# Biomedical-Imaging-Group/MolecularDiffusion_MiViT

Measured on AMD Instinct MI355X. Metric: training image-sequences/sec, higher is better.
Workload: dtype bf16; 1 GPU; PSFNoise 32-frame 64x64 sequences, MiViT depth=4 dim=128 heads=4 hidden=256, linear frame embedding + regression token; train step = fwd + MSE + bwd + AdamW; per_gpu_batch=16384, global_batch=16384, frames=32, frame=64x64, parallelism=dp1, input_dtype=f32 frames resident in HBM

## Files before the change

### include/mivit_hip.h

```cpp
#ifndef MIVIT_HIP_H
#define MIVIT_HIP_H

#include <stddef.h>
#include <stdint.h>

#ifdef __cplusplus
extern "C" {
#endif

#define MIVIT_ABI_VERSION 1

enum { MIVIT_F32 = 0, MIVIT_BF16 = 1, MIVIT_F16 = 2, MIVIT_F64 = 3 };
enum { MIVIT_ACT_NONE = 0, MIVIT_ACT_RELU = 1, MIVIT_ACT_LEAKY_RELU = 2, MIVIT_ACT_GELU = 3 };
enum { MIVIT_EMBED_LINEAR = 0, MIVIT_EMBED_CNN = 1, MIVIT_EMBED_EXTERNAL = 2 };
enum { MIVIT_FUSION_NONE = 0, MIVIT_FUSION_EARLY = 1, MIVIT_FUSION_LATE = 2 };

int mivit_abi_version(void);
const char *mivit_last_error(void);
int mivit_device_count(void);


int mivit_linear_fwd(int dtype, const void *x, int x_is_f32, int64_t ldx, const float *W, const float *bias,
                     int M, int N, int K, int act, const void *resid, int64_t ldr,
                     void *y, int64_t ldy, void *y_preact, void *stream);

int mivit_linear_dgrad(int dtype, const void *dy, int64_t lddy, const float *W, int M, int N, int K,
                       int act, const void *saved, int64_t lds, const void *dres, int64_t lddr,
                       void *dx, int64_t lddx, void *stream);

size_t mivit_linear_wgrad_workspace_bytes(int M, int N, int K);
int mivit_linear_wgrad(int dtype, const void *dy, int64_t lddy, const void *x, int x_is_f32, int64_t ldx,
                       int M, int N, int K, float *dW, float *db, int accumulate,
                       void *workspace, size_t workspace_bytes, void *stream);

int mivit_embed_fwd_bf16(const float *x, const void *W_bf16, const float *bias, int M, int K, int E, void *y_bf16,
                         void *stream);
int mivit_embed_set_variant(int variant);
size_t mivit_embed_wgrad_bf16_workspace_bytes(int M, int K, int E);
int mivit_embed_wgrad_bf16(const void *dy_bf16, const float *x, int M, int K, int E, float *dW, void *workspace,
                           size_t workspace_bytes, void *stream);

int mivit_embed_small_supported(int M, int K, int E);
int mivit_embed_small_fwd(const float *x, const void *W_bf16, const float *bias, int M, int K, int E, void *y_bf16, void *stream);
size_t mivit_embed_small_wgrad_workspace_bytes(int M, int K, int E);
int mivit_embed_small_wgrad(const void *dy_bf16, const float *x, int M, int K, int E, float *dW, float *db, void *workspace,
                            size_t workspace_bytes, void *stream);

int mivit_rowstream_fwd(const void *x, int64_t ldx, const void *W_bf16, const float *bias, int M, int N, int K, int act,
                        const void *resid, int64_t ldr, void *y, int64_t ldy, void *y_preact, const float *ln_gamma,
                        const float *ln_beta, void *ln_out, float *mean, float *rstd, void *stream);
int mivit_rowstream_dgrad(const void *dy, int64_t lddy, const void *W_bf16, int M, int N, int K, int act,
                          const void *saved, int64_t lds, const void *dres, int64_t lddr, void *dx, int64_t lddx,
                          void *stream);
int mivit_wavestream_fwd(const void *x, int64_t ldx, const void *W_bf16, const float *bias, int M, int N, int K, int act,
                         const void *resid, int64_t ldr, void *y, int64_t ldy, void *y_preact, const float *ln_gamma,
                         const float *ln_beta, void *ln_out, float *mean, float *rstd, void *stream);
int mivit_wavestream_dgrad(const void *dy, int64_t lddy, const void *W_bf16, int M, int N, int K, int act,
                           const void *saved, int64_t lds, const void *dres, int64_t lddr, void *dx, int64_t lddx,
                           void *stream);
int mivit_rowstream_set_wavestream(int mode);
int mivit_rowstream_set_wavestream_mask(int mask);

int mivit_gemm_dma_supported(int M, int N, int K, int dgrad);
int mivit_gemm_dma_set_variant(int variant);
int mivit_gemm_dma_fwd(const void *x, int64_t ldx, const void *W_bf16, const float *bias, int M, int N, int K, int act,
                       const void *resid, int64_t ldr, void *y, int64_t ldy, void *y_preact, void *stream);
int mivit_gemm_dma_dgrad(const void *dy, int64_t lddy, const void *W_bf16, int M, int N, int K, int act,
                         const void *saved, int64_t lds, const void *dres, int64_t lddr, void *dx, int64_t lddx,
                         void *stream);
size_t mivit_wgrad_bf16_workspace_bytes(int M, int N, int K);
int mivit_wgrad_bf16(const void *dy, int64_t lddy, const void *x, int64_t ldx, int M, int N, int K, float *dW, float *db,
                     void *workspace, size_t workspace_bytes, void *stream);
int mivit_wgrad_bf16_set_config(int cfg);

int mivit_rowstream_fwd_f16(const void *x, int64_t ldx, const void *W_f16, const float *bias, int M, int N, int K, int act,
                            const void *resid, int64_t ldr, void *y, int64_t ldy, void *y_preact, const float *ln_gamma,
                            const float *ln_beta, void *ln_out, float *mean, float *rstd, void *stream);
int mivit_rowstream_dgrad_f16(const void *dy, int64_t lddy, const void *W_f16, int M, int N, int K, int act,
                              const void *saved, int64_t lds, const void *dres, int64_t lddr, void *dx, int64_t lddx,
                              void *stream);
int mivit_wavestream_fwd_f16(const void *x, int64_t ldx, const void *W_f16, const float *bias, int M, int N, int K, int act,
                             const void *resid, int64_t ldr, void *y, int64_t ldy, void *y_preact, const float *ln_gamma,
                             const float *ln_beta, void *ln_out, float *mean, float *rstd, void *stream);
int mivit_wavestream_dgrad_f16(const void *dy, int64_t lddy, const void *W_f16, int M, int N, int K, int act,
                               const void *saved, int64_t lds, const void *dres, int64_t lddr, void *dx, int64_t lddx,
                               void *stream);
int mivit_rowstream_set_wavestream_f16(int mode);
int mivit_rowstream_set_wavestream_mask_f16(int mask);
size_t mivit_wgrad_bf16_workspace_bytes_f16(int M, int N, int K);
int mivit_wgrad_bf16_f16(const void *dy, int64_t lddy, const void *x, int64_t ldx, int M, int N, int K, float *dW, float *db,
                         void *workspace, size_t workspace_bytes, void *stream);
int mivit_wgrad_bf16_set_config_f16(int cfg);
size_t mivit_wgrad_small_workspace_bytes_f16(int M, int N, int K);
int mivit_wgrad_small_f16(const void *dy, int64_t lddy, const void *x, int64_t ldx, int M, int N, int K, float *dW,
                          float *db, void *workspace, size_t workspace_bytes, void *stream);
int mivit_embed_small_supported_f16(int M, int K, int E);
int mivit_embed_small_fwd_f16(const float *x, const void *W_f16, const float *bias, int M, int K, int E, void *y_f16, void *stream);
size_t mivit_embed_small_wgrad_workspace_bytes_f16(int M, int K, int E);
int mivit_embed_small_wgrad_f16(const void *dy_f16, const float *x, int M, int K, int E, float *dW, float *db, void *workspace,
                                size_t workspace_bytes, void *stream);
int mivit_embed_fwd_bf16_f16(const float *x, const void *W_f16, const float *bias, int M, int K, int E, void *y_f16,
                             void *stream);
int mivit_embed_set_variant_f16(int variant);
size_t mivit_embed_wgrad_bf16_workspace_bytes_f16(int M, int K, int E);
int mivit_embed_wgrad_bf16_f16(const void *dy_f16, const float *x, int M, int K, int E, float *dW, void *workspace,
                               size_t workspace_bytes, void *stream);

int mivit_fused_layer_supported(int dtype, int embed_dim, int hidden_dim, int num_heads, int tokens);
int mivit_attn_block_fwd(const void *n_in, const float *gamma_in, const float *beta_in, const void *Wqkv_bf16,
                         const float *bqkv, const void *Wo_bf16, const float *bo, const float *gamma_out,
                         const float *beta_out, int B, int S, void *ctx, void *n_out, float *rstd, void *x_out,
                         void *z_out, float *mean, void *qkv_out, void *stream);
int mivit_mlp_block_fwd(const void *n_in, const float *gamma_in, const float *beta_in, const void *W1_bf16,
                        const float *b1, const void *W2_bf16, const float *b2, const float *gamma_out,
                        const float *beta_out, int M, int act, void *n_out, float *rstd, void *x_out, void *z_out,
                        float *mean, void *h_out, void *u_out, void *stream);

size_t mivit_mlp_block_bwd_workspace_bytes(int M);
int mivit_mlp_block_bwd_set_waves(int waves);
int mivit_mlp_block_bwd(const void *dy, const void *n2, const float *rstd2, const float *gamma2, const void *n1,
                        const float *gamma1, const float *beta1, const void *W1_bf16, const float *b1, const void *W2_bf16,
                        int M, int act, void *dx1, float *dW1, float *db1, float *dW2, float *db2, float *dgamma2,
                        float *dbeta2, void *workspace, size_t workspace_bytes, void *stream);

int mivit_render_frames(const float *traj_px, int N, int T, int npos, const float *sigmas, int nsig, int P, int up,
                        const float *amp, int center, float *out, void *stream);

int mivit_render_movie(const float *pos, const float *amp, const int *first, const int *last, int Np, int F, int npos,
                       float sigma_hr, int up, int radius, int H, int W, float *movie, void *stream);

size_t mivit_trajectory_features_workspace_bytes(int N, int T, int npos);
int mivit_trajectory_features(const void *traj, int dtype, int N, int T, int npos, double dt, double *feats, void *avg,
                              void *workspace, size_t workspace_bytes, void *stream);

int mivit_rl_tv_deconvolve(const float *frames, int B, int S, int H, int W, const double *psf, int K, const int *snapshots,
                           int n_snap, float tv_weight, float *out, void *stream);

int mivit_gaussian_filter_frames(const float *in, int N, int H, int W, double sigma, double truncate, float *out,
                                 void *stream);

size_t mivit_dog_peaks_workspace_bytes(int F, int H, int W, int cap, int store_dog);
int mivit_dog_peaks(const float *movie, int F, int H, int W, const double *w1, int r1, const double *w2, int r2,
                    float threshold_percentage, int min_distance, int cap, int *count, int *n_candidates, int *coords,
                    float *values, float *dog, void *workspace, size_t workspace_bytes, void *stream);

int mivit_refine_gaussian(const float *patches, int N, int P, double xtol, double *params, float *peak, int *status,
                          void *stream);

int mivit_link_frames(const int *coords, const int *count, const unsigned char *movie_start, int F, int cap,
                      double max_distance, int *link, void *stream);

int mivit_chain_tracks(const int *link, const int *count, const unsigned char *movie_start, int F, int cap, int *ids,
                       int *lengths, int *n_tracks, void *stream);

int mivit_close_gaps(const int *coords, const int *count, const int *link, const unsigned char *movie_start, int F, int cap,
                     int max_gap, double max_distance, int *gap_partner, int *gap_frames, unsigned char *workspace,
                     size_t workspace_bytes, void *stream);

int mivit_chain_tracks_gaps(const int *link, const int *gap_partner, const int *gap_frames, const int *count,
                            const unsigned char *movie_start, int F, int cap, int max_gap, int *ids, int *lengths,
                            int *n_tracks, void *stream);

int mivit_track_msd(const double *pos, int N, const int *offsets, int n_tracks, double dt, int max_lag, int Lmax, double *msd,
                    double *d_lstsq, double *d_weighted, void *stream);

int mivit_track_sequences(const float *movie, int F, int H, int W, const int *frame, const int *y, const int *x, int N,
                          const int *seq_row, int n_seq, int T, int P, float lo, float denom, int normalize, float *seq,
                          void *stream);

int mivit_fgn(const double *z, const double *gamma, const int *gamma_row, int N, int T, int C, int U, double *out, void *stream);

int mivit_map_displacements(const double *disp, const double *s0, const int *geom_of, const double *verts, const double *lengths,
                            const int *vert_offsets, const double *totals, int N, int T, int G, int V, int mode, double *pos,
                            double *arc, int *edge, void *stream);

int mivit_segment_tracks(const double *pos, int N, const int *offsets, int n_tracks, int max_len, int min_len, double penalty,
                         double min_var, int *seg_start, double *cost, void *stream);
int mivit_segment_stats(const double *pos, int N, const int *seg_offsets, const int *seg_track_end, int n_seg, double dt,
                        double R, double *d_cve, double *d_mle, double *sigma2, int *n_increments, void *stream);
int mivit_markov_states(const double *u, const double *p0, const double *M, int N, int T, int K, int *state, void *stream);

size_t mivit_attn_out_bwd_workspace_bytes(int M);
int mivit_attn_out_bwd(const void *dy, const void *n1, const float *rstd1, const float *gamma1, const void *ctx,
                       const void *Wo_bf16, int M, void *dz1, void *dctx, float *dWo, float *dbo, float *dgamma1,
                       float *dbeta1, void *workspace, size_t workspace_bytes, void *stream);

size_t mivit_qkv_bwd_workspace_bytes(int M);
int mivit_qkv_bwd(const void *dqkv, const void *x, const void *Wqkv_bf16, const void *res, int M, void *dx, float *dW, float *db,
                  void *workspace, size_t workspace_bytes, void *stream);
int mivit_qkv_bwd_affine(const void *dqkv, const void *x, const void *Wqkv_bf16, const void *res, int M, void *dx, float *dW,
                         float *db, const float *fix_gamma, const float *fix_beta, void *workspace, size_t workspace_bytes,
                         void *stream);
size_t mivit_qkv_bwd_workspace_bytes_w64(int M);
int mivit_qkv_bwd_w64(const void *dqkv, const void *x, const void *Wqkv_bf16, const void *res, int M, void *dx, float *dW, float *db,
                      void *workspace, size_t workspace_bytes, void *stream);
int mivit_qkv_bwd_affine_w64(const void *dqkv, const void *x, const void *Wqkv_bf16, const void *res, int M, void *dx, float *dW,
                             float *db, const float *fix_gamma, const float *fix_beta, void *workspace, size_t workspace_bytes,
                             void *stream);

int mivit_fused_layer_supported_w64(int dtype, int embed_dim, int hidden_dim, int num_heads, int tokens);
int mivit_attn_block_fwd_w64(const void *n_in, const float *gamma_in, const float *beta_in, const void *Wqkv_bf16,
                             const float *bqkv, const void *Wo_bf16, const float *bo, const float *gamma_out,
                             const float *beta_out, int B, int S, void *ctx, void *n_out, float *rstd, void *x_out,
                             void *z_out, float *mean, void *qkv_out, void *stream);
int mivit_mlp_block_fwd_w64(const void *n_in, const float *gamma_in, const float *beta_in, const void *W1_bf16,
                            const float *b1, const void *W2_bf16, const float *b2, const float *gamma_out,
                            const float *beta_out, int M, int act, void *n_out, float *rstd, void *x_out, void *z_out,
                            float *mean, void *h_out, void *u_out, void *stream);
size_t mivit_mlp_block_bwd_workspace_bytes_w64(int M);
int mivit_mlp_block_bwd_w64(const void *dy, const void *n2, const float *rstd2, const float *gamma2, const void *n1,
                            const float *gamma1, const float *beta1, const void *W1_bf16, const float *b1, const void *W2_bf16,
                            int M, int act, void *dx1, float *dW1, float *db1, float *dW2, float *db2, float *dgamma2,
                            float *dbeta2, void *workspace, size_t workspace_bytes, void *stream);
size_t mivit_attn_out_bwd_workspace_bytes_w64(int M);
int mivit_attn_out_bwd_w64(const void *dy, const void *n1, const float *rstd1, const float *gamma1, const void *ctx,
                           const void *Wo_bf16, int M, void *dz1, void *dctx, float *dWo, float *dbo, float *dgamma1,
                           float *dbeta1, void *workspace, size_t workspace_bytes, void *stream);

int mivit_fused_layer_supported_f16(int dtype, int embed_dim, int hidden_dim, int num_heads, int tokens);
int mivit_attn_block_fwd_f16(const void *n_in, const float *gamma_in, const float *beta_in, const void *Wqkv,
                             const float *bqkv, const void *Wo, const float *bo, const float *gamma_out,
                             const float *beta_out, int B, int S, void *ctx, void *n_out, float *rstd, void *x_out,
                             void *z_out, float *mean, void *qkv_out, void *stream);
int mivit_mlp_block_fwd_f16(const void *n_in, const float *gamma_in, const float *beta_in, const void *W1,
                            const float *b1, const void *W2, const float *b2, const float *gamma_out,
                            const float *beta_out, int M, int act, void *n_out, float *rstd, void *x_out, void *z_out,
                            float *mean, void *h_out, void *u_out, void *stream);
size_t mivit_mlp_block_bwd_workspace_bytes_f16(int M);
int mivit_mlp_block_bwd_f16(const void *dy, const void *n2, const float *rstd2, const float *gamma2, const void *n1,
                            const float *gamma1, const float *beta1, const void *W1, const float *b1, const void *W2,
                            int M, int act, void *dx1, float *dW1, float *db1, float *dW2, float *db2, float *dgamma2,
                            float *dbeta2, void *workspace, size_t workspace_bytes, void *stream);
size_t mivit_attn_out_bwd_workspace_bytes_f16(int M);
int mivit_attn_out_bwd_f16(const void *dy, const void *n1, const float *rstd1, const float *gamma1, const void *ctx,
                           const void *Wo, int M, void *dz1, void *dctx, float *dWo, float *dbo, float *dgamma1,
                           float *dbeta1, void *workspace, size_t workspace_bytes, void *stream);
size_t mivit_qkv_bwd_workspace_bytes_f16(int M);
int mivit_qkv_bwd_f16(const void *dqkv, const void *x, const void *Wqkv, const void *res, int M, void *dx, float *dW, float *db,
                      void *workspace, size_t workspace_bytes, void *stream);
int mivit_qkv_bwd_affine_f16(const void *dqkv, const void *x, const void *Wqkv, const void *res, int M, void *dx, float *dW,
                             float *db, const float *fix_gamma, const float *fix_beta, void *workspace, size_t workspace_bytes,
                             void *stream);
int mivit_mlp_block_bwd_set_waves_f16(int waves);
int mivit_fused_layer_supported_w64_f16(int dtype, int embed_dim, int hidden_dim, int num_heads, int tokens);
int mivit_attn_block_fwd_w64_f16(const void *n_in, const float *gamma_in, const float *beta_in, const void *Wqkv,
                                 const float *bqkv, const void *Wo, const float *bo, const float *gamma_out,
                                 const float *beta_out, int B, int S, void *ctx, void *n_out, float *rstd, void *x_out,
                                 void *z_out, float *mean, void *qkv_out, void *stream);
int mivit_mlp_block_fwd_w64_f16(const void *n_in, const float *gamma_in, const float *beta_in, const void *W1,
                                const float *b1, const void *W2, const float *b2, const float *gamma_out,
                                const float *beta_out, int M, int act, void *n_out, float *rstd, void *x_out, void *z_out,
                                float *mean, void *h_out, void *u_out, void *stream);
size_t mivit_mlp_block_bwd_workspace_bytes_w64_f16(int M);
int mivit_mlp_block_bwd_w64_f16(const void *dy, const void *n2, const float *rstd2, const float *gamma2, const void *n1,
                                const float *gamma1, const float *beta1, const void *W1, const float *b1, const void *W2,
                                int M, int act, void *dx1, float *dW1, float *db1, float *dW2, float *db2, float *dgamma2,
                                float *dbeta2, void *workspace, size_t workspace_bytes, void *stream);
size_t mivit_attn_out_bwd_workspace_bytes_w64_f16(int M);
int mivit_attn_out_bwd_w64_f16(const void *dy, const void *n1, const float *rstd1, const float *gamma1, const void *ctx,
                               const void *Wo, int M, void *dz1, void *dctx, float *dWo, float *dbo, float *dgamma1,
                               float *dbeta1, void *workspace, size_t workspace_bytes, void *stream);
size_t mivit_qkv_bwd_workspace_bytes_w64_f16(int M);
int mivit_qkv_bwd_w64_f16(const void *dqkv, const void *x, const void *Wqkv, const void *res, int M, void *dx, float *dW, float *db,
                          void *workspace, size_t workspace_bytes, void *stream);
int mivit_qkv_bwd_affine_w64_f16(const void *dqkv, const void *x, const void *Wqkv, const void *res, int M, void *dx, float *dW,
                                 float *db, const float *fix_gamma, const float *fix_beta, void *workspace, size_t workspace_bytes,
                                 void *stream);

int mivit_deepresnet_eval_supported(int dtype, int patch_size);
int mivit_deepresnet_eval_fwd(int dtype, const float *x, int N, int P, int E, const float *w0, const float *b0,
                              const void *w11, const void *w12, const void *w1s, const void *w21, const void *w22,
                              const void *w2s, const float *b11, const float *b12, const float *b21, const float *b22,
                              const float *wfc, const float *bfc, float *tokens, void *stream);

typedef struct { const float *weight, *gamma, *beta; float *running_mean, *running_var; } mivit_conv_bn;
typedef struct { mivit_conv_bn conv[7]; const float *fc_weight, *fc_bias; } mivit_deepresnet_params;
typedef struct { float *weight, *gamma, *beta; } mivit_conv_bn_grad;
typedef struct { mivit_conv_bn_grad conv[7]; float *fc_weight, *fc_bias; } mivit_deepresnet_grads;
int mivit_deepresnet_train_supported(int dtype, int patch_size);
size_t mivit_deepresnet_train_workspace_bytes(int dtype, int N, int P, int E);
int mivit_deepresnet_train_fwd(int dtype, const mivit_deepresnet_params *params, const float *x, int N, int P, int E,
                               float momentum, float eps, float *tokens, void *workspace, size_t workspace_bytes,
                               void *stream);
int mivit_deepresnet_infer(int dtype, const mivit_deepresnet_params *params, const float *x, int N, int P, int E,
                           float eps, float *tokens, void *workspace, size_t workspace_bytes, void *stream);
int mivit_deepresnet_train_bwd(int dtype, const mivit_deepresnet_params *params, const float *x, const float *dtokens,
                               int N, int P, int E, float eps, const mivit_deepresnet_grads *grads, void *workspace,
                               size_t workspace_bytes, void *stream);

int mivit_deepresnet_train_workspace_layout(int dtype, int N, int P, int E, size_t *offsets );

#define MIVIT_DEEPRESNET_STAGES 6
#define MIVIT_DEEPRESNET_STATS_DOUBLES (2 * 3 * 128)
int mivit_deepresnet_train_fwd_stage(int dtype, const mivit_deepresnet_params *params, const float *x, int N, int P, int E,
                                     float momentum, float eps, float *tokens, void *workspace, size_t workspace_bytes,
                                     int stage, const double *global_count, double *stats, void *stream);
int mivit_deepresnet_train_bwd_stage(int dtype, const mivit_deepresnet_params *params, const float *x, const float *dtokens,
                                     int N, int P, int E, float eps, const mivit_deepresnet_grads *grads, void *workspace,
                                     size_t workspace_bytes, int stage, const double *global_count, double *stats, void *stream);

size_t mivit_wgrad_small_workspace_bytes(int M, int N, int K);
int mivit_wgrad_small(const void *dy, int64_t lddy, const void *x, int64_t ldx, int M, int N, int K, float *dW,
                      float *db , void *workspace, size_t workspace_bytes, void *stream);

int mivit_layernorm_fwd(int dtype, const void *z, int64_t ldz, const float *gamma, const float *beta,
                        int M, int E, void *y, int64_t ldy, int rows_per_seq, int out_seq_stride, int out_row_off,
                        const float *pos, float *mean, float *rstd, void *stream);

size_t mivit_layernorm_bwd_workspace_bytes(int M, int E);
int mivit_layernorm_bwd(int dtype, const void *dy, int64_t lddy, const void *z, int64_t ldz,
                        const float *gamma, const float *mean, const float *rstd, int M, int E,
                        int rows_per_seq, int in_seq_stride, int in_row_off,
                        void *dz, int64_t lddz, float *dgamma, float *dbeta, int accumulate,
                        void *workspace, size_t workspace_bytes, void *stream);

int mivit_attention_max_seq(int dtype, int Dh);
int mivit_attention_fwd(int dtype, const void *qkv, int B, int S, int H, int Dh, void *ctx, void *stream);
int mivit_attention_bwd(int dtype, const void *qkv, const void *dctx, int B, int S, int H, int Dh,
                        void *dqkv, void *stream);

typedef struct mivit_config {
    int abi_version;
    int dtype;
    int embedding;
    int patch_size;
    int embed_dim;
    int num_heads;
    int hidden_dim;
    int num_layers;
    int activation;
    int use_pos_encoding;
    int use_regression_token;
    int fusion;
    int global_feature_dim;
    int head_hidden;
    int output_dim;
} mivit_config;

typedef struct mivit_plan mivit_plan;

mivit_plan *mivit_plan_create(const mivit_config *cfg);
void mivit_plan_destroy(mivit_plan *plan);

int mivit_plan_num_params(const mivit_plan *plan);
const char *mivit_plan_param_name(const mivit_plan *plan, int i);
int64_t mivit_plan_param_offset(const mivit_plan *plan, int i);
int64_t mivit_plan_param_numel(const mivit_plan *plan, int i);
int64_t mivit_plan_arena_numel(const mivit_plan *plan);
int mivit_plan_num_stages(const mivit_plan *plan);
int mivit_plan_stage_range(const mivit_plan *plan, int stage, int64_t *begin, int64_t *end);

size_t mivit_plan_workspace_bytes(const mivit_plan *plan, int B, int T, int need_backward);

int mivit_forward(const mivit_plan *plan, const float *params, const float *x, const float *features,
                  int B, int T, void *workspace, size_t workspace_bytes, int need_backward,
                  float *out, void *stream);

int mivit_backward(const mivit_plan *plan, const float *params, const float *x, const float *features,
                   int B, int T, void *workspace, size_t workspace_bytes, const float *dout,
                   float *grads, float *dfeatures, float *dx_tokens,
                   int stage_begin, int stage_end, void *stream);

void mivit_graph_stats(uint64_t *replays, uint64_t *captures, int *failures);

enum {
    MIVIT_PROF_EMBED_FWD = 0,
    MIVIT_PROF_EMBED_WGRAD = 1,
    MIVIT_PROF_LINEAR_FWD = 2,
    MIVIT_PROF_LINEAR_DGRAD = 3,
    MIVIT_PROF_LINEAR_WGRAD = 4,
    MIVIT_PROF_ATTN_FWD = 5,
    MIVIT_PROF_ATTN_BWD = 6,
    MIVIT_PROF_LN_FWD = 7,
    MIVIT_PROF_LN_BWD = 8,
    MIVIT_PROF_OP = 9,
    MIVIT_PROF_ATTN_BLOCK_FWD = 10,
    MIVIT_PROF_MLP_BLOCK_FWD = 11,
    MIVIT_PROF_MLP_BLOCK_BWD = 12,
    MIVIT_PROF_ATTN_OUT_BWD = 13,
    MIVIT_PROF_ATTN_CORE_BWD = 14,
    MIVIT_PROF_QKV_WGRAD = 15,
    MIVIT_PROF_QKV_DGRAD = 16,
    MIVIT_PROF_QKV_BWD = 17,
    MIVIT_PROF_NUM_TAGS = 18
};
int mivit_profile_enable(uint64_t tag_mask);
int mivit_profile_collect(int tag, double *total_ms, int *count);
const char *mivit_profile_tag_name(int tag);

#ifdef __cplusplus
}
#endif
#endif
```

### moleculardiffusion_mivit_amd/_native.py

```python
import ctypes
import os
from ctypes import c_char_p, c_float, c_int, c_int64, c_size_t, c_void_p, POINTER, Structure

_PKG = os.path.dirname(os.path.abspath(__file__))
LIB_PATH = os.path.join(_PKG, "libmivit_hip.so")

ABI_VERSION = 1
F32, BF16, F16 = 0, 1, 2
F64 = 3
ACT_NONE, ACT_RELU, ACT_LEAKY_RELU, ACT_GELU = 0, 1, 2, 3
EMBED_LINEAR, EMBED_CNN, EMBED_EXTERNAL = 0, 1, 2
FUSION_NONE, FUSION_EARLY, FUSION_LATE = 0, 1, 2


class MivitConfig(Structure):
    _fields_ = [(n, c_int) for n in (
        "abi_version", "dtype", "embedding", "patch_size", "embed_dim", "num_heads", "hidden_dim", "num_layers",
        "activation", "use_pos_encoding", "use_regression_token", "fusion", "global_feature_dim", "head_hidden",
        "output_dim")]


class ConvBn(Structure):
    _fields_ = [(n, c_void_p) for n in ("weight", "gamma", "beta", "running_mean", "running_var")]


class DeepResNetParams(Structure):
    _fields_ = [("conv", ConvBn * 7), ("fc_weight", c_void_p), ("fc_bias", c_void_p)]


class ConvBnGrad(Structure):
    _fields_ = [(n, c_void_p) for n in ("weight", "gamma", "beta")]


class DeepResNetGrads(Structure):
    _fields_ = [("conv", ConvBnGrad * 7), ("fc_weight", c_void_p), ("fc_bias", c_void_p)]


SYMBOLS = {
    "mivit_abi_version": (c_int, []),
    "mivit_last_error": (c_char_p, []),
    "mivit_device_count": (c_int, []),
    "mivit_linear_fwd": (c_int, [c_int, c_void_p, c_int, c_int64, c_void_p, c_void_p, c_int, c_int, c_int, c_int,
                                 c_void_p, c_int64, c_void_p, c_int64, c_void_p, c_void_p]),
    "mivit_linear_dgrad": (c_int, [c_int, c_void_p, c_int64, c_void_p, c_int, c_int, c_int, c_int, c_void_p, c_int64,
                                   c_void_p, c_int64, c_void_p, c_int64, c_void_p]),
    "mivit_linear_wgrad_workspace_bytes": (c_size_t, [c_int, c_int, c_int]),
    "mivit_linear_wgrad": (c_int, [c_int, c_void_p, c_int64, c_void_p, c_int, c_int64, c_int, c_int, c_int, c_void_p,
                                   c_void_p, c_int, c_void_p, c_size_t, c_void_p]),
    "mivit_embed_fwd_bf16": (c_int, [c_void_p, c_void_p, c_void_p, c_int, c_int, c_int, c_void_p, c_void_p]),
    "mivit_embed_set_variant": (c_int, [c_int]),
    "mivit_embed_wgrad_bf16_workspace_bytes": (c_size_t, [c_int, c_int, c_int]),
    "mivit_embed_wgrad_bf16": (c_int, [c_void_p, c_void_p, c_int, c_int, c_int, c_void_p, c_void_p, c_size_t, c_void_p]),
    "mivit_rowstream_fwd": (c_int, [c_void_p, c_int64, c_void_p, c_void_p, c_int, c_int, c_int, c_int, c_void_p, c_int64,
                                    c_void_p, c_int64, c_void_p, c_void_p, c_void_p, c_void_p, c_void_p, c_void_p, c_void_p]),
    "mivit_rowstream_dgrad": (c_int, [c_void_p, c_int64, c_void_p, c_int, c_int, c_int, c_int, c_void_p, c_int64, c_void_p,
                                      c_int64, c_void_p, c_int64, c_void_p]),
    "mivit_wavestream_fwd": (c_int, [c_void_p, c_int64, c_void_p, c_void_p, c_int, c_int, c_int, c_int, c_void_p, c_int64,
                                     c_void_p, c_int64, c_void_p, c_void_p, c_void_p, c_void_p, c_void_p, c_void_p, c_void_p]),
    "mivit_wavestream_dgrad": (c_int, [c_void_p, c_int64, c_void_p, c_int, c_int, c_int, c_int, c_void_p, c_int64, c_void_p,
                                       c_int64, c_void_p, c_int64, c_void_p]),
    "mivit_gemm_dma_supported": (c_int, [c_int, c_int, c_int, c_int]),
    "mivit_gemm_dma_set_variant": (c_int, [c_int]),
    "mivit_gemm_dma_fwd": (c_int, [c_void_p, c_int64, c_void_p, c_void_p, c_int, c_int, c_int, c_int, c_void_p, c_int64,
                                   c_void_p, c_int64, c_void_p, c_void_p]),
    "mivit_gemm_dma_dgrad": (c_int, [c_void_p, c_int64, c_void_p, c_int, c_int, c_int, c_int, c_void_p, c_int64, c_void_p,
                                     c_int64, c_void_p, c_int64, c_void_p]),
    "mivit_wgrad_bf16_workspace_bytes": (c_size_t, [c_int, c_int, c_int]),
    "mivit_wgrad_bf16": (c_int, [c_void_p, c_int64, c_void_p, c_int64, c_int, c_int, c_int, c_void_p, c_void_p, c_void_p,
                                 c_size_t, c_void_p]),
    "mivit_deepresnet_eval_supported": (c_int, [c_int, c_int]),
    "mivit_deepresnet_eval_fwd": (c_int, [c_int, c_void_p, c_int, c_int, c_int] + [c_void_p] * 16),
    "mivit_deepresnet_train_supported": (c_int, [c_int, c_int]),
    "mivit_deepresnet_train_workspace_bytes": (c_size_t, [c_int, c_int, c_int, c_int]),
    "mivit_deepresnet_train_fwd": (c_int, [c_int, c_void_p, c_void_p, c_int, c_int, c_int, c_float, c_float, c_void_p,
                                           c_void_p, c_size_t, c_void_p]),
    "mivit_deepresnet_infer": (c_int, [c_int, c_void_p, c_void_p, c_int, c_int, c_int, c_float, c_void_p, c_void_p, c_size_t,
                                       c_void_p]),
    "mivit_deepresnet_train_bwd": (c_int, [c_int, c_void_p, c_void_p, c_void_p, c_int, c_int, c_int, c_float, c_void_p,
                                           c_void_p, c_size_t, c_void_p]),
    "mivit_deepresnet_train_workspace_layout": (c_int, [c_int, c_int, c_int, c_int, c_void_p]),
    "mivit_deepresnet_train_fwd_stage": (c_int, [c_int, c_void_p, c_void_p, c_int, c_int, c_int, c_float, c_float, c_void_p,
                                                 c_void_p, c_size_t, c_int, c_void_p, c_void_p, c_void_p]),
    "mivit_deepresnet_train_bwd_stage": (c_int, [c_int, c_void_p, c_void_p, c_void_p, c_int, c_int, c_int, c_float, c_void_p,
                                                 c_void_p, c_size_t, c_int, c_void_p, c_void_p, c_void_p]),
    "mivit_graph_stats": (None, [c_void_p, c_void_p, c_void_p]),
    "mivit_wgrad_small_workspace_bytes": (c_size_t, [c_int, c_int, c_int]),
    "mivit_wgrad_small": (c_int, [c_void_p, c_int64, c_void_p, c_int64, c_int, c_int, c_int, c_void_p, c_void_p, c_void_p,
                                  c_size_t, c_void_p]),
    "mivit_layernorm_fwd": (c_int, [c_int, c_void_p, c_int64, c_void_p, c_void_p, c_int, c_int, c_void_p, c_int64,
                                    c_int, c_int, c_int, c_void_p, c_void_p, c_void_p, c_void_p]),
    "mivit_layernorm_bwd_workspace_bytes": (c_size_t, [c_int, c_int]),
    "mivit_layernorm_bwd": (c_int, [c_int, c_void_p, c_int64, c_void_p, c_int64, c_void_p, c_void_p, c_void_p, c_int,
                                    c_int, c_int, c_int, c_int, c_void_p, c_int64, c_void_p, c_void_p, c_int,
                                    c_void_p, c_size_t, c_void_p]),
    "mivit_attention_max_seq": (c_int, [c_int, c_int]),
    "mivit_attention_fwd": (c_int, [c_int, c_void_p, c_int, c_int, c_int, c_int, c_void_p, c_void_p]),
    "mivit_attention_bwd": (c_int, [c_int, c_void_p, c_void_p, c_int, c_int, c_int, c_int, c_void_p, c_void_p]),
    "mivit_plan_create": (c_void_p, [POINTER(MivitConfig)]),
    "mivit_plan_destroy": (None, [c_void_p]),
    "mivit_plan_num_params": (c_int, [c_void_p]),
    "mivit_plan_param_name": (c_char_p, [c_void_p, c_int]),
    "mivit_plan_param_offset": (c_int64, [c_void_p, c_int]),
    "mivit_plan_param_numel": (c_int64, [c_void_p, c_int]),
    "mivit_plan_arena_numel": (c_int64, [c_void_p]),
    "mivit_plan_num_stages": (c_int, [c_void_p]),
    "mivit_plan_stage_range": (c_int, [c_void_p, c_int, POINTER(c_int64), POINTER(c_int64)]),
    "mivit_plan_workspace_bytes": (c_size_t, [c_void_p, c_int, c_int, c_int]),
    "mivit_forward": (c_int, [c_void_p, c_void_p, c_void_p, c_void_p, c_int, c_int, c_void_p, c_size_t, c_int,
                              c_void_p, c_void_p]),
    "mivit_backward": (c_int, [c_void_p, c_void_p, c_void_p, c_void_p, c_int, c_int, c_void_p, c_size_t, c_void_p,
                               c_void_p, c_void_p, c_void_p, c_int, c_int, c_void_p]),
    "mivit_fused_layer_supported": (c_int, [c_int, c_int, c_int, c_int, c_int]),
    "mivit_attn_block_fwd": (c_int, [c_void_p] * 9 + [c_int, c_int] + [c_void_p] * 8),
    "mivit_mlp_block_fwd": (c_int, [c_void_p] * 9 + [c_int, c_int] + [c_void_p] * 8),
    "mivit_mlp_block_bwd_workspace_bytes": (c_size_t, [c_int]),
    "mivit_mlp_block_bwd_set_waves": (c_int, [c_int]),
    "mivit_mlp_block_bwd": (c_int, [c_void_p] * 10 + [c_int, c_int] + [c_void_p] * 8 + [c_size_t, c_void_p]),
    "mivit_render_frames": (c_int, [c_void_p, c_int, c_int, c_int, c_void_p, c_int, c_int, c_int, c_void_p, c_int, c_void_p, c_void_p]),
    "mivit_render_movie": (c_int, [c_void_p, c_void_p, c_void_p, c_void_p, c_int, c_int, c_int, c_float, c_int, c_int, c_int, c_int,
                                   c_void_p, c_void_p]),
    "mivit_trajectory_features_workspace_bytes": (c_size_t, [c_int, c_int, c_int]),
    "mivit_trajectory_features": (c_int, [c_void_p, c_int, c_int, c_int, c_int, ctypes.c_double, c_void_p, c_void_p, c_void_p,
                                          c_size_t, c_void_p]),
    "mivit_rl_tv_deconvolve": (c_int, [c_void_p, c_int, c_int, c_int, c_int, c_void_p, c_int, c_void_p, c_int, ctypes.c_float,
                                       c_void_p, c_void_p]),
    "mivit_gaussian_filter_frames": (c_int, [c_void_p, c_int, c_int, c_int, ctypes.c_double, ctypes.c_double, c_void_p,
                                             c_void_p]),
    "mivit_dog_peaks_workspace_bytes": (c_size_t, [c_int, c_int, c_int, c_int, c_int]),
    "mivit_dog_peaks": (c_int, [c_void_p, c_int, c_int, c_int, c_void_p, c_int, c_void_p, c_int, c_float, c_int, c_int,
                                c_void_p, c_void_p, c_void_p, c_void_p, c_void_p, c_void_p, c_size_t, c_void_p]),
    "mivit_refine_gaussian": (c_int, [c_void_p, c_int, c_int, ctypes.c_double, c_void_p, c_void_p, c_void_p, c_void_p]),
    "mivit_link_frames": (c_int, [c_void_p, c_void_p, c_void_p, c_int, c_int, ctypes.c_double, c_void_p, c_void_p]),
    "mivit_chain_tracks": (c_int, [c_void_p, c_void_p, c_void_p, c_int, c_int, c_void_p, c_void_p, c_void_p, c_void_p]),
    "mivit_close_gaps": (c_int, [c_void_p, c_void_p, c_void_p, c_void_p, c_int, c_int, c_int, ctypes.c_double, c_void_p, c_void_p,
                                 c_void_p, c_size_t, c_void_p]),
    "mivit_chain_tracks_gaps": (c_int, [c_void_p, c_void_p, c_void_p, c_void_p, c_void_p, c_int, c_int, c_int, c_void_p, c_void_p,
                                        c_void_p, c_void_p]),
    "mivit_track_msd": (c_int, [c_void_p, c_int, c_void_p, c_int, ctypes.c_double, c_int, c_int, c_void_p, c_void_p, c_void_p,
                                c_void_p]),
    "mivit_track_sequences": (c_int, [c_void_p, c_int, c_int, c_int, c_void_p, c_void_p, c_void_p, c_int, c_void_p, c_int, c_int,
                                      c_int, ctypes.c_float, ctypes.c_float, c_int, c_void_p, c_void_p]),
    "mivit_fgn": (c_int, [c_void_p, c_void_p, c_void_p, c_int, c_int, c_int, c_int, c_void_p, c_void_p]),
    "mivit_map_displacements": (c_int, [c_void_p] * 7 + [c_int] * 5 + [c_void_p] * 4),
    "mivit_segment_tracks": (c_int, [c_void_p, c_int, c_void_p, c_int, c_int, c_int, ctypes.c_double, ctypes.c_double, c_void_p,
                                     c_void_p, c_void_p]),
    "mivit_segment_stats": (c_int, [c_void_p, c_int, c_void_p, c_void_p, c_int, ctypes.c_double, ctypes.c_double, c_void_p,
                                    c_void_p, c_void_p, c_void_p, c_void_p]),
    "mivit_markov_states": (c_int, [c_void_p, c_void_p, c_void_p, c_int, c_int, c_int, c_void_p, c_void_p]),
    "mivit_attn_out_bwd_workspace_bytes": (c_size_t, [c_int]),
    "mivit_attn_out_bwd": (c_int, [c_void_p] * 6 + [c_int] + [c_void_p] * 7 + [c_size_t, c_void_p]),
    "mivit_embed_small_supported": (c_int, [c_int, c_int, c_int]),
    "mivit_embed_small_fwd": (c_int, [c_void_p, c_void_p, c_void_p, c_int, c_int, c_int, c_void_p, c_void_p]),
    "mivit_embed_small_wgrad_workspace_bytes": (c_size_t, [c_int, c_int, c_int]),
    "mivit_embed_small_wgrad": (c_int, [c_void_p, c_void_p, c_int, c_int, c_int, c_void_p, c_void_p, c_void_p, c_size_t, c_void_p]),
    "mivit_qkv_bwd_workspace_bytes": (c_size_t, [c_int]),
    "mivit_qkv_bwd": (c_int, [c_void_p] * 4 + [c_int] + [c_void_p] * 4 + [c_size_t, c_void_p]),
    "mivit_qkv_bwd_workspace_bytes_w64": (c_size_t, [c_int]),
    "mivit_qkv_bwd_w64": (c_int, [c_void_p] * 4 + [c_int] + [c_void_p] * 4 + [c_size_t, c_void_p]),
    "mivit_fused_layer_supported_w64": (c_int, [c_int, c_int, c_int, c_int, c_int]),
    "mivit_attn_block_fwd_w64": (c_int, [c_void_p] * 9 + [c_int, c_int] + [c_void_p] * 8),
    "mivit_mlp_block_fwd_w64": (c_int, [c_void_p] * 9 + [c_int, c_int] + [c_void_p] * 8),
    "mivit_mlp_block_bwd_workspace_bytes_w64": (c_size_t, [c_int]),
    "mivit_mlp_block_bwd_w64": (c_int, [c_void_p] * 10 + [c_int, c_int] + [c_void_p] * 8 + [c_size_t, c_void_p]),
    "mivit_attn_out_bwd_workspace_bytes_w64": (c_size_t, [c_int]),
    "mivit_attn_out_bwd_w64": (c_int, [c_void_p] * 6 + [c_int] + [c_void_p] * 7 + [c_size_t, c_void_p]),
    "mivit_qkv_bwd_affine": (c_int, [c_void_p] * 4 + [c_int] + [c_void_p] * 6 + [c_size_t, c_void_p]),
    "mivit_qkv_bwd_affine_w64": (c_int, [c_void_p] * 4 + [c_int] + [c_void_p] * 6 + [c_size_t, c_void_p]),
    "mivit_mlp_block_bwd_set_waves_f16": (c_int, [c_int]),
    "mivit_profile_enable": (c_int, [ctypes.c_uint64]),
    "mivit_profile_collect": (c_int, [c_int, POINTER(ctypes.c_double), POINTER(c_int)]),
    "mivit_profile_tag_name": (c_char_p, [c_int]),
}
for _sfx in ("_f16", "_w64_f16"):
    for _name in ("mivit_fused_layer_supported", "mivit_attn_block_fwd", "mivit_mlp_block_fwd", "mivit_mlp_block_bwd_workspace_bytes",
                  "mivit_mlp_block_bwd", "mivit_attn_out_bwd_workspace_bytes", "mivit_attn_out_bwd", "mivit_qkv_bwd_workspace_bytes",
                  "mivit_qkv_bwd", "mivit_qkv_bwd_affine"):
        SYMBOLS[_name + _sfx] = SYMBOLS[_name]
SYMBOLS["mivit_rowstream_set_wavestream"] = SYMBOLS["mivit_rowstream_set_wavestream_mask"] = (c_int, [c_int])
SYMBOLS["mivit_wgrad_bf16_set_config"] = (c_int, [c_int])
for _name in ("mivit_rowstream_fwd", "mivit_rowstream_dgrad", "mivit_wavestream_fwd", "mivit_wavestream_dgrad",
              "mivit_rowstream_set_wavestream", "mivit_rowstream_set_wavestream_mask", "mivit_wgrad_bf16_workspace_bytes",
              "mivit_wgrad_bf16", "mivit_wgrad_bf16_set_config", "mivit_wgrad_small_workspace_bytes", "mivit_wgrad_small",
              "mivit_embed_small_supported", "mivit_embed_small_fwd", "mivit_embed_small_wgrad_workspace_bytes",
              "mivit_embed_small_wgrad", "mivit_embed_fwd_bf16", "mivit_embed_set_variant",
              "mivit_embed_wgrad_bf16_workspace_bytes", "mivit_embed_wgrad_bf16"):
    SYMBOLS[_name + "_f16"] = SYMBOLS[_name]
PROF_TAGS = ["embed_fwd", "embed_wgrad", "linear_fwd", "linear_dgrad", "linear_wgrad", "attn_fwd", "attn_bwd",
             "ln_fwd", "ln_bwd", "op", "attn_block_fwd", "mlp_block_fwd", "mlp_block_bwd", "attn_out_bwd", "attn_core_bwd",
             "qkv_wgrad", "qkv_dgrad", "qkv_bwd"]


class MivitError(RuntimeError):
    pass


def _load(path=LIB_PATH):
    if not os.path.exists(path):
        raise ImportError(
            f"{path} is missing: the MiViT HIP extension has not been built. Run "
            "`python -m moleculardiffusion_mivit_amd.csrc.build` (needs hipcc, targets gfx950). "
            "There is no CPU / PyTorch fallback for this path.")
    import torch
    lib = ctypes.CDLL(path)
    for name, (res, args) in SYMBOLS.items():
        fn = getattr(lib, name)
        fn.restype = res
        fn.argtypes = args
    if lib.mivit_abi_version() != ABI_VERSION:
        raise ImportError(f"libmivit_hip.so ABI {lib.mivit_abi_version()} != binding ABI {ABI_VERSION}; rebuild")
    return lib


lib = _load()

STRICT_LIB_PATH = os.path.join(_PKG, "libmivit_hip_strict.so")


def load_strict():
    return _load(STRICT_LIB_PATH)


def check(rc, what=""):
    if rc != 0:
        msg = lib.mivit_last_error()
        raise MivitError(f"{what}: {msg.decode() if msg else 'unknown error'}")


def last_error():
    msg = lib.mivit_last_error()
    return msg.decode() if msg else ""
```

### moleculardiffusion_mivit_amd/csrc/attention.hip

```cpp
#include "common.h"

namespace {

template <typename T>
struct Img {
    T *p;
    int rs, ks;
};

template <typename T>
__device__ __forceinline__ f32x4 tile_mma(const Img<T> A, int ar0, const Img<T> B, int br0, int kdim, int lane) {
    f32x4 acc = {0.f, 0.f, 0.f, 0.f};
    for (int kk = 0; kk < kdim; kk += Mma<T>::KS)
        acc = Mma<T>::mma(Mma<T>::load(A.p, A.rs, A.ks, ar0, kk, lane), Mma<T>::load(B.p, B.rs, B.ks, br0, kk, lane), acc);
    return acc;
}

__device__ __forceinline__ void wave_lds_sync() {
    __builtin_amdgcn_fence(__ATOMIC_ACQ_REL, "workgroup");
    __builtin_amdgcn_wave_barrier();
}

__device__ __forceinline__ float group16_max(float v) {
#pragma unroll
    for (int o = 8; o > 0; o >>= 1) v = fmaxf(v, __shfl_xor(v, o, 64));
    return v;
}
__device__ __forceinline__ float group16_sum(float v) {
#pragma unroll
    for (int o = 8; o > 0; o >>= 1) v += __shfl_xor(v, o, 64);
    return v;
}

struct AttnDims {
    int S, Dh, E, H, B;
    int Sp;
    int Skp;
    int Dp;
    int D16;
    int ldq;
    int ldk;
    int per_wave;
    int two_pass;
    int nw;
};

template <typename T>
__host__ __device__ inline int round_up_i(int x, int m) { return (x + m - 1) / m * m; }

template <typename T>
AttnDims make_dims(int B, int S, int H, int Dh, bool backward) {
    constexpr int KS = Mma<T>::KS;
    constexpr bool BF = sizeof(T) == 2;
    AttnDims d;
    d.B = B; d.S = S; d.H = H; d.Dh = Dh; d.E = H * Dh;
    d.Sp = (S + 15) / 16 * 16;
    const int kr = KS > 16 ? KS : 16;
    d.Skp = (S + kr - 1) / kr * kr;
    d.Dp = (Dh + KS - 1) / KS * KS;
    d.D16 = (Dh + 15) / 16 * 16;
    const int rowsq = d.Sp;
    if (BF) {
        d.ldq = d.Dp + 8;
        d.ldk = d.Skp + 8;
    } else {
        d.ldq = (d.Dp > d.D16 ? d.Dp : d.D16) + 1;
        d.ldk = d.Skp + 1;
    }
    const int nat = rowsq * d.ldq;
    const int tr = d.D16 * d.ldk;
    const int ps = (d.Sp > d.Skp ? d.Sp : d.Skp) * d.ldk;
    if (!backward) d.per_wave = 3 * nat + (BF ? tr : 0) + ps;
    else d.per_wave = 4 * nat + (BF ? 3 * tr : 0) + (BF ? 3 : 2) * ps;
    d.two_pass = 0;
    if (backward && !BF && (size_t)d.per_wave * sizeof(T) > (size_t)160 * 1024) { d.two_pass = 1; d.per_wave = 4 * nat + ps; }
    d.per_wave = (d.per_wave + 7) / 8 * 8;
    const size_t bytes = (size_t)d.per_wave * sizeof(T);
    int nw = (int)((size_t)64 * 1024 / bytes);
    d.nw = nw < 1 ? 1 : (nw > 4 ? 4 : nw);
    return d;
}

template <typename T>
__device__ __forceinline__ void stage_head(const T *src, int64_t src_ld, int S, int Dh, T *nat, int ldq, T *tr, int ldk,
                                           int lane) {
    if ((Dh & 3) == 0) {
        const int per_row = Dh >> 2;
        for (int u = lane; u < S * per_row; u += 64) {
            const int r = u / per_row, d = (u % per_row) * 4;
            T v[4];
            if (sizeof(T) == 2) *reinterpret_cast<uint2 *>(v) = *reinterpret_cast<const uint2 *>(src + (int64_t)r * src_ld + d);
            else *reinterpret_cast<float4 *>(v) = *reinterpret_cast<const float4 *>(src + (int64_t)r * src_ld + d);
#pragma unroll
            for (int i = 0; i < 4; ++i) {
                nat[r * ldq + d + i] = v[i];
                if (tr) tr[(d + i) * ldk + r] = v[i];
            }
        }
    } else {
        for (int u = lane; u < S * Dh; u += 64) {
            const int r = u / Dh, d = u % Dh;
            const T v = src[(int64_t)r * src_ld + d];
            nat[r * ldq + d] = v;
            if (tr) tr[d * ldk + r] = v;
        }
    }
}

template <typename T>
__device__ __forceinline__ void zero_lds(T *p, int n, int lane) {
    uint32_t *q = reinterpret_cast<uint32_t *>(p);
    const int words = n * (int)sizeof(T) / 4;
    for (int i = lane; i < words; i += 64) q[i] = 0u;
}

template <typename T, int NT>
__global__ __launch_bounds__(256) void attn_fwd_kernel(const T *qkv, T *ctx, const AttnDims d) {
    extern __shared__ __attribute__((aligned(16))) unsigned char smem_raw[];
    constexpr bool BF = sizeof(T) == 2;
    const int lane = threadIdx.x & 63, wave = threadIdx.x >> 6;
    const int pair = blockIdx.x * d.nw + wave;
    if (pair >= d.B * d.H) return;
    const int b = pair / d.H, h = pair % d.H;
    T *base = reinterpret_cast<T *>(smem_raw) + (size_t)wave * d.per_wave;
    const int nat = d.Sp * d.ldq;
    T *Qn = base, *Kn = Qn + nat, *Vn = Kn + nat;
    T *Vt = BF ? Vn + nat : nullptr;
    T *Ps = (BF ? Vt + d.D16 * d.ldk : Vn + nat);
    zero_lds(base, d.per_wave, lane);
    wave_lds_sync();
    const int64_t ld3 = 3 * (int64_t)d.E;
    const T *src = qkv + (int64_t)b * d.S * ld3 + h * d.Dh;
    stage_head<T>(src, ld3, d.S, d.Dh, Qn, d.ldq, nullptr, 0, lane);
    stage_head<T>(src + d.E, ld3, d.S, d.Dh, Kn, d.ldq, nullptr, 0, lane);
    stage_head<T>(src + 2 * d.E, ld3, d.S, d.Dh, Vn, d.ldq, Vt, d.ldk, lane);
    wave_lds_sync();

    const Img<T> Qi = {Qn, d.ldq, 1}, Ki = {Kn, d.ldq, 1}, Pi = {Ps, d.ldk, 1};
    const Img<T> Vti = BF ? Img<T>{Vt, d.ldk, 1} : Img<T>{Vn, 1, d.ldq};
    const float scale = 1.0f / sqrtf((float)d.Dh);
    const int colq = lane & 15, rowq = (lane >> 4) * 4;

    for (int it = 0; it < NT; ++it) {
        f32x4 sc[NT];
#pragma unroll
        for (int j = 0; j < NT; ++j) sc[j] = tile_mma<T>(Qi, it * 16, Ki, j * 16, d.Dp, lane);
#pragma unroll
        for (int r = 0; r < 4; ++r) {
            float m = -INFINITY;
#pragma unroll
            for (int j = 0; j < NT; ++j) {
                const bool ok = j * 16 + colq < d.S;
                sc[j][r] = ok ? sc[j][r] * scale : -INFINITY;
                m = fmaxf(m, sc[j][r]);
            }
            m = group16_max(m);
            float sum = 0.f;
#pragma unroll
            for (int j = 0; j < NT; ++j) {
                const float e = (j * 16 + colq < d.S) ? __expf(sc[j][r] - m) : 0.f;
                sc[j][r] = e;
                sum += e;
            }
            sum = group16_sum(sum);
            const float inv = 1.f / sum;
#pragma unroll
            for (int j = 0; j < NT; ++j) Ps[(it * 16 + rowq + r) * d.ldk + j * 16 + colq] = from_f32<T>(sc[j][r] * inv);
        }
        wave_lds_sync();
        for (int jd = 0; jd < d.D16 / 16; ++jd) {
            const f32x4 o = tile_mma<T>(Pi, it * 16, Vti, jd * 16, d.Skp, lane);
            const int dcol = jd * 16 + colq;
#pragma unroll
            for (int r = 0; r < 4; ++r) {
                const int row = it * 16 + rowq + r;
                if (row < d.S && dcol < d.Dh)
                    ctx[((int64_t)b * d.S + row) * d.E + h * d.Dh + dcol] = from_f32<T>(o[r]);
            }
        }
    }
}

template <typename T, int NT>
__global__ __launch_bounds__(256) void attn_bwd_kernel(const T *qkv, const T *dctx, T *dqkv, const AttnDims d) {
    extern __shared__ __attribute__((aligned(16))) unsigned char smem_raw[];
    constexpr bool BF = sizeof(T) == 2;
    const int lane = threadIdx.x & 63, wave = threadIdx.x >> 6;
    const int pair = blockIdx.x * d.nw + wave;
    if (pair >= d.B * d.H) return;
    const int b = pair / d.H, h = pair % d.H;
    T *base = reinterpret_cast<T *>(smem_raw) + (size_t)wave * d.per_wave;
    const int nat = d.Sp * d.ldq, tr = d.D16 * d.ldk;
    const int ps = (d.Sp > d.Skp ? d.Sp : d.Skp) * d.ldk;
    T *Qn = base, *Kn = Qn + nat, *Vn = Kn + nat, *On = Vn + nat;
    T *cur = On + nat;
    T *Qt = nullptr, *Kt = nullptr, *Ot = nullptr;
    if (BF) { Qt = cur; Kt = Qt + tr; Ot = Kt + tr; cur = Ot + tr; }
    T *Pa = cur;
    T *dSn = Pa + ps;
    T *dSt = BF ? dSn + ps : nullptr;
    zero_lds(base, d.per_wave, lane);
    wave_lds_sync();
    const int64_t ld3 = 3 * (int64_t)d.E;
    const T *src = qkv + (int64_t)b * d.S * ld3 + h * d.Dh;
    stage_head<T>(src, ld3, d.S, d.Dh, Qn, d.ldq, Qt, d.ldk, lane);
    stage_head<T>(src + d.E, ld3, d.S, d.Dh, Kn, d.ldq, Kt, d.ldk, lane);
    stage_head<T>(src + 2 * d.E, ld3, d.S, d.Dh, Vn, d.ldq, nullptr, 0, lane);
    stage_head<T>(dctx + (int64_t)b * d.S * d.E + h * d.Dh, d.E, d.S, d.Dh, On, d.ldq, Ot, d.ldk, lane);
    wave_lds_sync();

    const Img<T> Qi = {Qn, d.ldq, 1}, Ki = {Kn, d.ldq, 1}, Vi = {Vn, d.ldq, 1}, Oi = {On, d.ldq, 1};
    const float scale = 1.0f / sqrtf((float)d.Dh);
    const int colq = lane & 15, rowq = (lane >> 4) * 4;

    auto score_pass = [&](const int mode) {
        for (int it = 0; it < NT; ++it) {
            f32x4 sc[NT], dp[NT];
#pragma unroll
            for (int j = 0; j < NT; ++j) {
                sc[j] = tile_mma<T>(Qi, it * 16, Ki, j * 16, d.Dp, lane);
                dp[j] = tile_mma<T>(Oi, it * 16, Vi, j * 16, d.Dp, lane);
            }
#pragma unroll
            for (int r = 0; r < 4; ++r) {
                float m = -INFINITY;
#pragma unroll
                for (int j = 0; j < NT; ++j) {
                    const bool ok = j * 16 + colq < d.S;
                    sc[j][r] = ok ? sc[j][r] * scale : -INFINITY;
                    m = fmaxf(m, sc[j][r]);
                }
                m = group16_max(m);
                float sum = 0.f;
#pragma unroll
                for (int j = 0; j < NT; ++j) {
                    const float e = (j * 16 + colq < d.S) ? __expf(sc[j][r] - m) : 0.f;
                    sc[j][r] = e;
                    sum += e;
                }
                sum = group16_sum(sum);
                const float inv = 1.f / sum;
                float delta = 0.f;
#pragma unroll
                for (int j = 0; j < NT; ++j) {
                    sc[j][r] *= inv;
                    delta += sc[j][r] * dp[j][r];
                }
                delta = group16_sum(delta);
                const int row = it * 16 + rowq + r;
#pragma unroll
                for (int j = 0; j < NT; ++j) {
                    const int key = j * 16 + colq;
                    const float p = sc[j][r];
                    const float ds = scale * p * (dp[j][r] - delta);
                    if (mode == 0) {
                        if (BF) {
                            Pa[key * d.ldk + row] = from_f32<T>(p);
                            dSt[key * d.ldk + row] = from_f32<T>(ds);
                        } else {
                            Pa[row * d.ldk + key] = from_f32<T>(p);
                        }
                        dSn[row * d.ldk + key] = from_f32<T>(ds);
                    } else {
                        Pa[row * d.ldk + key] = from_f32<T>(mode == 1 ? p : ds);
                    }
                }
            }
        }
    };
    const bool two_pass = !BF && d.two_pass;
    T *dst = dqkv + (int64_t)b * d.S * ld3 + h * d.Dh;
    if (two_pass) {
        score_pass(1);
        wave_lds_sync();
        const Img<T> PTi1 = {Pa, 1, d.ldk}, Oti1 = {On, 1, d.ldq};
        for (int it = 0; it < NT; ++it)
            for (int jd = 0; jd < d.D16 / 16; ++jd) {
                const f32x4 dv = tile_mma<T>(PTi1, it * 16, Oti1, jd * 16, d.Skp, lane);
                const int dcol = jd * 16 + colq;
#pragma unroll
                for (int r = 0; r < 4; ++r) {
                    const int row = it * 16 + rowq + r;
                    if (row < d.S && dcol < d.Dh) dst[(int64_t)row * ld3 + dcol + 2 * d.E] = from_f32<T>(dv[r]);
                }
            }
        wave_lds_sync();
        score_pass(2);
        wave_lds_sync();
        const Img<T> dSi2 = {Pa, d.ldk, 1}, dSTi2 = {Pa, 1, d.ldk}, Qti2 = {Qn, 1, d.ldq}, Kti2 = {Kn, 1, d.ldq};
        for (int it = 0; it < NT; ++it)
            for (int jd = 0; jd < d.D16 / 16; ++jd) {
                const f32x4 dq = tile_mma<T>(dSi2, it * 16, Kti2, jd * 16, d.Skp, lane);
                const f32x4 dk = tile_mma<T>(dSTi2, it * 16, Qti2, jd * 16, d.Skp, lane);
                const int dcol = jd * 16 + colq;
#pragma unroll
                for (int r = 0; r < 4; ++r) {
                    const int row = it * 16 + rowq + r;
                    if (row < d.S && dcol < d.Dh) {
                        T *o = dst + (int64_t)row * ld3 + dcol;
                        o[0] = from_f32<T>(dq[r]);
                        o[d.E] = from_f32<T>(dk[r]);
                    }
                }
            }
        return;
    }
    score_pass(0);
    wave_lds_sync();

    const Img<T> PTi = BF ? Img<T>{Pa, d.ldk, 1} : Img<T>{Pa, 1, d.ldk};
    const Img<T> dSTi = BF ? Img<T>{dSt, d.ldk, 1} : Img<T>{dSn, 1, d.ldk};
    const Img<T> dSi = {dSn, d.ldk, 1};
    const Img<T> Oti = BF ? Img<T>{Ot, d.ldk, 1} : Img<T>{On, 1, d.ldq};
    const Img<T> Qti = BF ? Img<T>{Qt, d.ldk, 1} : Img<T>{Qn, 1, d.ldq};
    const Img<T> Kti = BF ? Img<T>{Kt, d.ldk, 1} : Img<T>{Kn, 1, d.ldq};
    for (int it = 0; it < NT; ++it) {
        for (int jd = 0; jd < d.D16 / 16; ++jd) {
            const f32x4 dq = tile_mma<T>(dSi, it * 16, Kti, jd * 16, d.Skp, lane);
            const f32x4 dk = tile_mma<T>(dSTi, it * 16, Qti, jd * 16, d.Skp, lane);
            const f32x4 dv = tile_mma<T>(PTi, it * 16, Oti, jd * 16, d.Skp, lane);
            const int dcol = jd * 16 + colq;
#pragma unroll
            for (int r = 0; r < 4; ++r) {
                const int row = it * 16 + rowq + r;
                if (row < d.S && dcol < d.Dh) {
                    T *o = dst + (int64_t)row * ld3 + dcol;
                    o[0] = from_f32<T>(dq[r]);
                    o[d.E] = from_f32<T>(dk[r]);
                    o[2 * d.E] = from_f32<T>(dv[r]);
                }
            }
        }
    }
}

constexpr size_t LDS_LIMIT = 160 * 1024;

template <typename T, int NT>
int launch_fwd_nt(const T *qkv, T *ctx, const AttnDims &d, hipStream_t s) {
    const size_t bytes = (size_t)d.per_wave * sizeof(T) * d.nw;
    auto kern = attn_fwd_kernel<T, NT>;
    if (bytes > 48 * 1024)
        MIVIT_HIP(hipFuncSetAttribute(reinterpret_cast<const void *>(kern), hipFuncAttributeMaxDynamicSharedMemorySize, (int)bytes));
    const int blocks = ceil_div(d.B * d.H, d.nw);
    ProfScope prof(s);
    hipLaunchKernelGGL(kern, dim3(blocks), dim3(64 * d.nw), bytes, s, qkv, ctx, d);
    MIVIT_LAUNCH_CHECK();
    return 0;
}
template <typename T, int NT>
int launch_bwd_nt(const T *qkv, const T *dctx, T *dqkv, const AttnDims &d, hipStream_t s) {
    const size_t bytes = (size_t)d.per_wave * sizeof(T) * d.nw;
    auto kern = attn_bwd_kernel<T, NT>;
    if (bytes > 48 * 1024)
        MIVIT_HIP(hipFuncSetAttribute(reinterpret_cast<const void *>(kern), hipFuncAttributeMaxDynamicSharedMemorySize, (int)bytes));
    const int blocks = ceil_div(d.B * d.H, d.nw);
    ProfScope prof(s);
    hipLaunchKernelGGL(kern, dim3(blocks), dim3(64 * d.nw), bytes, s, qkv, dctx, dqkv, d);
    MIVIT_LAUNCH_CHECK();
    return 0;
}

template <typename T>
int attn_fwd_t(const void *qkv, int B, int S, int H, int Dh, void *ctx, hipStream_t s) {
    const AttnDims d = make_dims<T>(B, S, H, Dh, false);
    MIVIT_CHECK((size_t)d.per_wave * sizeof(T) <= LDS_LIMIT, "attention_fwd: S=%d Dh=%d does not fit in LDS", S, Dh);
    const T *q = static_cast<const T *>(qkv);
    T *c = static_cast<T *>(ctx);
    switch (d.Sp / 16) {
        case 1: return launch_fwd_nt<T, 1>(q, c, d, s);
        case 2: return launch_fwd_nt<T, 2>(q, c, d, s);
        case 3: return launch_fwd_nt<T, 3>(q, c, d, s);
        case 4: return launch_fwd_nt<T, 4>(q, c, d, s);
        case 5: return launch_fwd_nt<T, 5>(q, c, d, s);
        case 6: return launch_fwd_nt<T, 6>(q, c, d, s);
        case 7: return launch_fwd_nt<T, 7>(q, c, d, s);
        case 8: return launch_fwd_nt<T, 8>(q, c, d, s);
        default: MIVIT_FAIL("attention_fwd: S=%d > 128 is not supported by the LDS-resident kernel", S);
    }
}
template <typename T>
int attn_bwd_t(const void *qkv, const void *dctx, int B, int S, int H, int Dh, void *dqkv, hipStream_t s) {
    const AttnDims d = make_dims<T>(B, S, H, Dh, true);
    MIVIT_CHECK((size_t)d.per_wave * sizeof(T) <= LDS_LIMIT, "attention_bwd: S=%d Dh=%d does not fit in LDS", S, Dh);
    const T *q = static_cast<const T *>(qkv);
    const T *g = static_cast<const T *>(dctx);
    T *o = static_cast<T *>(dqkv);
    switch (d.Sp / 16) {
        case 1: return launch_bwd_nt<T, 1>(q, g, o, d, s);
        case 2: return launch_bwd_nt<T, 2>(q, g, o, d, s);
        case 3: return launch_bwd_nt<T, 3>(q, g, o, d, s);
        case 4: return launch_bwd_nt<T, 4>(q, g, o, d, s);
        case 5: return launch_bwd_nt<T, 5>(q, g, o, d, s);
        case 6: return launch_bwd_nt<T, 6>(q, g, o, d, s);
        case 7: return launch_bwd_nt<T, 7>(q, g, o, d, s);
        case 8: return launch_bwd_nt<T, 8>(q, g, o, d, s);
        default: MIVIT_FAIL("attention_bwd: S=%d > 128 is not supported by the LDS-resident kernel", S);
    }
}

}

int attention_max_seq(int dtype, int Dh) {
    int best = 0;
    for (int S = 1; S <= 128; ++S) {
        const AttnDims d = dtype == MIVIT_F32 ? make_dims<float>(1, S, 1, Dh, true) : make_dims<bf16>(1, S, 1, Dh, true);
        if ((size_t)d.per_wave * dtype_size(dtype) <= LDS_LIMIT || attention_fast_supported(dtype, S, Dh) ||
            attention_fast_supported_f16(dtype, S, Dh)) best = S;
    }
    return best;
}

int launch_attention_fwd(int dtype, const void *qkv, int B, int S, int H, int Dh, void *ctx, hipStream_t s) {
    MIVIT_CHECK(B > 0 && S > 0 && H > 0 && Dh > 0, "attention_fwd: empty problem");
    if (attention_fast_supported(dtype, S, Dh)) return launch_attention_fwd_fast(qkv, B, S, H, Dh, ctx, s);
    if (attention_fast_supported_f16(dtype, S, Dh)) return launch_attention_fwd_fast_f16(qkv, B, S, H, Dh, ctx, s);
    return dtype == MIVIT_F32 ? attn_fwd_t<float>(qkv, B, S, H, Dh, ctx, s)
         : dtype == MIVIT_BF16 ? attn_fwd_t<bf16>(qkv, B, S, H, Dh, ctx, s) : attn_fwd_t<f16>(qkv, B, S, H, Dh, ctx, s);
}
int launch_attention_bwd(int dtype, const void *qkv, const void *dctx, int B, int S, int H, int Dh, void *dqkv,
                         hipStream_t s) {
    MIVIT_CHECK(B > 0 && S > 0 && H > 0 && Dh > 0, "attention_bwd: empty problem");
    if (attention_fast_supported(dtype, S, Dh)) return launch_attention_bwd_fast(qkv, dctx, B, S, H, Dh, dqkv, s);
    if (attention_fast_supported_f16(dtype, S, Dh)) return launch_attention_bwd_fast_f16(qkv, dctx, B, S, H, Dh, dqkv, s);
    return dtype == MIVIT_F32 ? attn_bwd_t<float>(qkv, dctx, B, S, H, Dh, dqkv, s)
         : dtype == MIVIT_BF16 ? attn_bwd_t<bf16>(qkv, dctx, B, S, H, Dh, dqkv, s) : attn_bwd_t<f16>(qkv, dctx, B, S, H, Dh, dqkv, s);
}

extern "C" int mivit_attention_max_seq(int dtype, int Dh) { return attention_max_seq(dtype, Dh); }
extern "C" int mivit_attention_fwd(int dtype, const void *qkv, int B, int S, int H, int Dh, void *ctx, void *stream) {
    MIVIT_CHECK(dtype == MIVIT_F32 || dtype == MIVIT_BF16 || dtype == MIVIT_F16, "bad dtype %d", dtype);
    MIVIT_CHECK(qkv && ctx, "attention_fwd: null pointer");
    return launch_attention_fwd(dtype, qkv, B, S, H, Dh, ctx, static_cast<hipStream_t>(stream));
}
extern "C" int mivit_attention_bwd(int dtype, const void *qkv, const void *dctx, int B, int S, int H, int Dh,
                                   void *dqkv, void *stream) {
    MIVIT_CHECK(dtype == MIVIT_F32 || dtype == MIVIT_BF16 || dtype == MIVIT_F16, "bad dtype %d", dtype);
    MIVIT_CHECK(qkv && dctx && dqkv, "attention_bwd: null pointer");
    return launch_attention_bwd(dtype, qkv, dctx, B, S, H, Dh, dqkv, static_cast<hipStream_t>(stream));
}
```

### moleculardiffusion_mivit_amd/csrc/attention_fast.hip

```cpp
#include "common.h"
#include <stdlib.h>
#include "stream_prims.h"
#include "elem.h"

namespace {


struct U128 {
    uint32_t w[4];
};

__device__ __forceinline__ bf16x8 as_frag(const U128 &u) { return __builtin_bit_cast(bf16x8, u); }

__device__ __forceinline__ bf16x8 gfrag(const bf16 *base, int64_t ld, int row0, int S, int d0, int Dh, int lane) {
    const int r = row0 + (lane & 15), d = d0 + 8 * (lane >> 4);
    U128 u = {{0u, 0u, 0u, 0u}};
    if (r < S && d + 8 <= Dh) {
        const uint4 v = *reinterpret_cast<const uint4 *>(base + (int64_t)r * ld + d);
        u.w[0] = v.x; u.w[1] = v.y; u.w[2] = v.z; u.w[3] = v.w;
    }
    return as_frag(u);
}

__device__ __forceinline__ bf16x8 tr_frag(const bf16 *img, int ld, int ta, int tb, int col0, int lane) {
    const int i = lane & 15, q = i >> 2, p = i & 3;
    typedef __attribute__((address_space(3))) s16x4 lds_v4;
    const s16x4 lo = __builtin_amdgcn_ds_read_tr16_b64_v4i16((lds_v4 *)(img + (ta + q) * ld + col0 + 4 * p));
    const s16x4 hi = __builtin_amdgcn_ds_read_tr16_b64_v4i16((lds_v4 *)(img + (tb + q) * ld + col0 + 4 * p));
    struct { s16x4 a, b; } pr = {lo, hi};
    return __builtin_bit_cast(bf16x8, pr);
}

__device__ __forceinline__ bf16x8 pack_frag(const f32x4 a, const f32x4 b) {
    bf16x8 f;
    f[0] = (__bf16)a[0]; f[1] = (__bf16)a[1]; f[2] = (__bf16)a[2]; f[3] = (__bf16)a[3];
    f[4] = (__bf16)b[0]; f[5] = (__bf16)b[1]; f[6] = (__bf16)b[2]; f[7] = (__bf16)b[3];
    return f;
}


__device__ __forceinline__ float g16_max(float v) { return row16_max(v); }
__device__ __forceinline__ float g16_sum(float v) { return row16_sum(v); }
__device__ __forceinline__ float x4_max(float v) { return rows4_max(v); }
__device__ __forceinline__ float x4_sum(float v) { return rows4_sum(v); }

__device__ __forceinline__ void lds_sync() {
    __builtin_amdgcn_fence(__ATOMIC_ACQ_REL, "workgroup");
    __builtin_amdgcn_wave_barrier();
}

template <bool SWZ = false>
__device__ __forceinline__ void stage_nat(bf16 *img, int ld, const bf16 *src, int64_t src_ld, int S, int rows, int Dh,
                                          int lane) {
    const int cpr = Dh >> 3, n = rows * cpr;
    for (int u0 = lane; u0 < n; u0 += 4 * 64) {
        uint4 v[4];
#pragma unroll
        for (int i = 0; i < 4; ++i) {
            const int u = u0 + 64 * i, r = u / cpr, d = (u % cpr) * 8;
            v[i] = make_uint4(0u, 0u, 0u, 0u);
            if (u < n && r < S) v[i] = *reinterpret_cast<const uint4 *>(src + (int64_t)r * src_ld + d);
        }
#pragma unroll
        for (int i = 0; i < 4; ++i) {
            const int u = u0 + 64 * i, r = u / cpr, d = (u % cpr) * 8;
            if (u < n) *reinterpret_cast<uint4 *>(img + r * ld + (SWZ ? (d ^ (((r >> 2) & 1) << 4)) : d)) = v[i];
        }
    }
}

struct FastDims {
    int B, S, H, Dh, E;
    int ld;
    int img;
};

template <int NT, int ND>
__global__ __launch_bounds__(256) void attn_fwd_fast(const bf16 *qkv, bf16 *ctx, const FastDims d) {
    extern __shared__ __attribute__((aligned(16))) unsigned char smem_raw[];
    constexpr int KD = (ND + 1) / 2;
    constexpr int NP = (NT + 1) / 2;
    const int lane = threadIdx.x & 63, wave = threadIdx.x >> 6;
    const int pair = blockIdx.x * (blockDim.x >> 6) + wave;
    if (pair >= d.B * d.H) return;
    const int b = pair / d.H, h = pair % d.H;
    const int g = lane >> 4, cq = lane & 15;
    bf16 *Vimg = reinterpret_cast<bf16 *>(smem_raw) + (size_t)wave * d.img;
    const int64_t ld3 = 3 * (int64_t)d.E;
    const bf16 *q = qkv + (int64_t)b * d.S * ld3 + h * d.Dh, *k = q + d.E, *v = q + 2 * d.E;
    stage_nat(Vimg, d.ld, v, ld3, d.S, NP * 32, d.Dh, lane);
    bf16x8 kf[NT][KD];
#pragma unroll
    for (int j = 0; j < NT; ++j)
#pragma unroll
        for (int kd = 0; kd < KD; ++kd) kf[j][kd] = gfrag(k, ld3, j * 16, d.S, kd * 32, d.Dh, lane);
    lds_sync();
    const float scale = 1.0f / sqrtf((float)d.Dh);

    for (int it = 0; it < NT; ++it) {
        bf16x8 qf[KD];
#pragma unroll
        for (int kd = 0; kd < KD; ++kd) qf[kd] = gfrag(q, ld3, it * 16, d.S, kd * 32, d.Dh, lane);
        f32x4 st[NT];
        float m = -INFINITY;
#pragma unroll
        for (int j = 0; j < NT; ++j) {
            st[j] = f32x4{0.f, 0.f, 0.f, 0.f};
#pragma unroll
            for (int kd = 0; kd < KD; ++kd) st[j] = mma(kf[j][kd], qf[kd], st[j]);
#pragma unroll
            for (int r = 0; r < 4; ++r) {
                const bool ok = j * 16 + 4 * g + r < d.S;
                st[j][r] = ok ? st[j][r] * scale : -INFINITY;
                m = fmaxf(m, st[j][r]);
            }
        }
        m = x4_max(m);
        float sum = 0.f;
#pragma unroll
        for (int j = 0; j < NT; ++j)
#pragma unroll
            for (int r = 0; r < 4; ++r) {
                const float e = (j * 16 + 4 * g + r < d.S) ? __expf(st[j][r] - m) : 0.f;
                st[j][r] = e;
                sum += e;
            }
        const float inv = 1.f / x4_sum(sum);
#pragma unroll
        for (int j = 0; j < NT; ++j) st[j] *= inv;
#pragma unroll
        for (int jd = 0; jd < ND; ++jd) {
            f32x4 o = {0.f, 0.f, 0.f, 0.f};
#pragma unroll
            for (int ks = 0; ks < NP; ++ks) {
                const f32x4 zero = {0.f, 0.f, 0.f, 0.f};
                const bf16x8 a = pack_frag(st[2 * ks], (2 * ks + 1 < NT) ? st[2 * ks + 1] : zero);
                const bf16x8 bb = tr_frag(Vimg, d.ld, 32 * ks + 4 * g, 32 * ks + 16 + 4 * g, jd * 16, lane);
                o = mma(a, bb, o);
            }
#pragma unroll
            for (int r = 0; r < 4; ++r) {
                const int row = it * 16 + 4 * g + r;
                if (row < d.S) ctx[((int64_t)b * d.S + row) * d.E + h * d.Dh + jd * 16 + cq] = from_f32<bf16>(o[r]);
            }
        }
    }
}

template <int NT, int ND>
__global__ __launch_bounds__(256) void attn_bwd_fast(const bf16 *qkv, const bf16 *dctx, bf16 *dqkv, const FastDims d) {
    extern __shared__ __attribute__((aligned(16))) unsigned char smem_raw[];
    constexpr int KD = (ND + 1) / 2;
    constexpr int NP = (NT + 1) / 2;
    const int lane = threadIdx.x & 63, wave = threadIdx.x >> 6;
    const int pair = blockIdx.x * (blockDim.x >> 6) + wave;
    if (pair >= d.B * d.H) return;
    const int b = pair / d.H, h = pair % d.H;
    const int g = lane >> 4, cq = lane & 15;
    bf16 *Qimg = reinterpret_cast<bf16 *>(smem_raw) + (size_t)wave * 3 * d.img;
    bf16 *Kimg = Qimg + d.img, *Oimg = Kimg + d.img;
    const int64_t ld3 = 3 * (int64_t)d.E;
    const bf16 *q = qkv + (int64_t)b * d.S * ld3 + h * d.Dh, *k = q + d.E, *v = q + 2 * d.E;
    const bf16 *dO = dctx + (int64_t)b * d.S * d.E + h * d.Dh;
    stage_nat(Qimg, d.ld, q, ld3, d.S, NP * 32, d.Dh, lane);
    stage_nat(Kimg, d.ld, k, ld3, d.S, NP * 32, d.Dh, lane);
    stage_nat(Oimg, d.ld, dO, d.E, d.S, NP * 32, d.Dh, lane);
    bf16x8 kf[NT][KD], vf[NT][KD], qf[NT][KD], of[NT][KD];
#pragma unroll
    for (int j = 0; j < NT; ++j)
#pragma unroll
        for (int kd = 0; kd < KD; ++kd) {
            kf[j][kd] = gfrag(k, ld3, j * 16, d.S, kd * 32, d.Dh, lane);
            vf[j][kd] = gfrag(v, ld3, j * 16, d.S, kd * 32, d.Dh, lane);
            qf[j][kd] = gfrag(q, ld3, j * 16, d.S, kd * 32, d.Dh, lane);
            of[j][kd] = gfrag(dO, d.E, j * 16, d.S, kd * 32, d.Dh, lane);
        }
    lds_sync();
    const float scale = 1.0f / sqrtf((float)d.Dh);
    const f32x4 zero = {0.f, 0.f, 0.f, 0.f};
    bf16 *dst = dqkv + (int64_t)b * d.S * ld3 + h * d.Dh;

    f32x4 dv[NT][ND], dk[NT][ND];
#pragma unroll
    for (int j = 0; j < NT; ++j)
#pragma unroll
        for (int jd = 0; jd < ND; ++jd) { dv[j][jd] = zero; dk[j][jd] = zero; }

#pragma unroll
    for (int ip = 0; ip < NP; ++ip) {
        f32x4 pU[2][NT], sU[2][NT];
#pragma unroll
        for (int t = 0; t < 2; ++t) {
            const int it = 2 * ip + t;
            if (it >= NT) {
#pragma unroll
                for (int j = 0; j < NT; ++j) { pU[t][j] = zero; sU[t][j] = zero; }
                continue;
            }
            f32x4 sc[NT], dp[NT];
#pragma unroll
            for (int j = 0; j < NT; ++j) {
                sc[j] = zero; dp[j] = zero;
#pragma unroll
                for (int kd = 0; kd < KD; ++kd) {
                    sc[j] = mma(qf[it][kd], kf[j][kd], sc[j]);
                    dp[j] = mma(of[it][kd], vf[j][kd], dp[j]);
                }
            }
#pragma unroll
            for (int r = 0; r < 4; ++r) {
                float m = -INFINITY;
#pragma unroll
                for (int j = 0; j < NT; ++j) {
                    const bool ok = j * 16 + cq < d.S;
                    sc[j][r] = ok ? sc[j][r] * scale : -INFINITY;
                    m = fmaxf(m, sc[j][r]);
                }
                m = g16_max(m);
                float sum = 0.f;
#pragma unroll
                for (int j = 0; j < NT; ++j) {
                    const float e = (j * 16 + cq < d.S) ? __expf(sc[j][r] - m) : 0.f;
                    sc[j][r] = e;
                    sum += e;
                }
                const float inv = 1.f / g16_sum(sum);
                float delta = 0.f;
#pragma unroll
                for (int j = 0; j < NT; ++j) {
                    sc[j][r] *= inv;
                    delta += sc[j][r] * dp[j][r];
                }
                delta = g16_sum(delta);
#pragma unroll
                for (int j = 0; j < NT; ++j) {
                    pU[t][j][r] = sc[j][r];
                    sU[t][j][r] = scale * sc[j][r] * (dp[j][r] - delta);
                }
            }
            f32x4 st[NT], dt[NT];
            float m = -INFINITY;
#pragma unroll
            for (int j = 0; j < NT; ++j) {
                st[j] = zero; dt[j] = zero;
#pragma unroll
                for (int kd = 0; kd < KD; ++kd) {
                    st[j] = mma(kf[j][kd], qf[it][kd], st[j]);
                    dt[j] = mma(vf[j][kd], of[it][kd], dt[j]);
                }
#pragma unroll
                for (int r = 0; r < 4; ++r) {
                    const bool ok = j * 16 + 4 * g + r < d.S;
                    st[j][r] = ok ? st[j][r] * scale : -INFINITY;
                    m = fmaxf(m, st[j][r]);
                }
            }
            m = x4_max(m);
            float sum = 0.f;
#pragma unroll
            for (int j = 0; j < NT; ++j)
#pragma unroll
                for (int r = 0; r < 4; ++r) {
                    const float e = (j * 16 + 4 * g + r < d.S) ? __expf(st[j][r] - m) : 0.f;
                    st[j][r] = e;
                    sum += e;
                }
            const float inv = 1.f / x4_sum(sum);
            float delta = 0.f;
#pragma unroll
            for (int j = 0; j < NT; ++j)
#pragma unroll
                for (int r = 0; r < 4; ++r) {
                    st[j][r] *= inv;
                    delta += st[j][r] * dt[j][r];
                }
            delta = x4_sum(delta);
#pragma unroll
            for (int j = 0; j < NT; ++j)
#pragma unroll
                for (int r = 0; r < 4; ++r) st[j][r] = scale * st[j][r] * (dt[j][r] - delta);
#pragma unroll
            for (int jd = 0; jd < ND; ++jd) {
                f32x4 dq = zero;
#pragma unroll
                for (int ks = 0; ks < NP; ++ks) {
                    const bf16x8 a = pack_frag(st[2 * ks], (2 * ks + 1 < NT) ? st[2 * ks + 1] : zero);
                    const bf16x8 bb = tr_frag(Kimg, d.ld, 32 * ks + 4 * g, 32 * ks + 16 + 4 * g, jd * 16, lane);
                    dq = mma(a, bb, dq);
                }
#pragma unroll
                for (int r = 0; r < 4; ++r) {
                    const int row = it * 16 + 4 * g + r;
                    if (row < d.S) dst[(int64_t)row * ld3 + jd * 16 + cq] = from_f32<bf16>(dq[r]);
                }
            }
        }
#pragma unroll
        for (int jd = 0; jd < ND; ++jd) {
            const bf16x8 bo = tr_frag(Oimg, d.ld, 32 * ip + 4 * g, 32 * ip + 16 + 4 * g, jd * 16, lane);
            const bf16x8 bq = tr_frag(Qimg, d.ld, 32 * ip + 4 * g, 32 * ip + 16 + 4 * g, jd * 16, lane);
#pragma unroll
            for (int j = 0; j < NT; ++j) {
                dv[j][jd] = mma(pack_frag(pU[0][j], pU[1][j]), bo, dv[j][jd]);
                dk[j][jd] = mma(pack_frag(sU[0][j], sU[1][j]), bq, dk[j][jd]);
            }
        }
    }
#pragma unroll
    for (int j = 0; j < NT; ++j)
#pragma unroll
        for (int jd = 0; jd < ND; ++jd)
#pragma unroll
            for (int r = 0; r < 4; ++r) {
                const int key = j * 16 + 4 * g + r;
                if (key < d.S) {
                    bf16 *o = dst + (int64_t)key * ld3 + jd * 16 + cq;
                    o[d.E] = from_f32<bf16>(dk[j][jd][r]);
                    o[2 * d.E] = from_f32<bf16>(dv[j][jd][r]);
                }
            }
}

typedef __attribute__((ext_vector_type(4))) short k16_t;
__device__ __forceinline__ k16_t pack4(const f32x4 a) {
    typedef __attribute__((ext_vector_type(4))) __bf16 bf16x4;
    bf16x4 f;
    f[0] = (__bf16)a[0]; f[1] = (__bf16)a[1]; f[2] = (__bf16)a[2]; f[3] = (__bf16)a[3];
    return __builtin_bit_cast(k16_t, f);
}
template <bool SWZ = false>
__device__ __forceinline__ k16_t tr4(const bf16 *img, int ld, int trow, int col0, int lane) {
    const int i = lane & 15, q = i >> 2, p = i & 3;
    typedef __attribute__((address_space(3))) s16x4 lds_v4;
    const int row = trow + q, col = col0 + 4 * p;
    return __builtin_amdgcn_ds_read_tr16_b64_v4i16((lds_v4 *)(img + row * ld + (SWZ ? (col ^ (((row >> 2) & 1) << 4)) : col)));
}
__device__ __forceinline__ f32x4 mma16(k16_t a, k16_t b, f32x4 c) {
    return ELEM_MFMA_16x16x16(a, b, c);
}

template <int NT, int ND>
__global__ __launch_bounds__(256, (NT * ND <= 6 ? 3 : 1)) void attn_bwd_fast2(const bf16 *qkv, const bf16 *dctx, bf16 *dqkv, const FastDims d) {
    extern __shared__ __attribute__((aligned(16))) unsigned char smem_raw[];
    constexpr int KD = (ND + 1) / 2;
    constexpr bool SWZ = ND == 2;
    const int lane = threadIdx.x & 63, wave = threadIdx.x >> 6;
    const int pair = blockIdx.x * (blockDim.x >> 6) + wave;
    if (pair >= d.B * d.H) return;
    const int b = pair / d.H, h = pair % d.H;
    const int g = lane >> 4, cq = lane & 15;
    bf16 *Qimg = reinterpret_cast<bf16 *>(smem_raw) + (size_t)wave * (3 * d.img + NT * 256);
    bf16 *Kimg = Qimg + d.img, *Oimg = Kimg + d.img, *Simg = Oimg + d.img;
    const int64_t ld3 = 3 * (int64_t)d.E;
    const bf16 *q = qkv + (int64_t)b * d.S * ld3 + h * d.Dh, *k = q + d.E, *v = q + 2 * d.E;
    const bf16 *dO = dctx + (int64_t)b * d.S * d.E + h * d.Dh;
    constexpr int CPR = ND * 2, NCH = NT * 16 * CPR, NIT = (NCH + 63) / 64;
    constexpr bool BATCH = NIT <= 4 && NT <= 4;
    bf16x8 kf[NT][KD], vf[NT][KD];
    if (BATCH) {
        uint4 sq[NIT], sk[NIT], so[NIT];
        auto ld_nat = [&](const bf16 *src, int64_t sld, uint4 (&v)[NIT]) {
#pragma unroll
            for (int i = 0; i < NIT; ++i) {
                const int u = lane + 64 * i, r = u / CPR, dd = (u % CPR) * 8;
                v[i] = make_uint4(0u, 0u, 0u, 0u);
                if (u < NCH && r < d.S && dd + 8 <= d.Dh) v[i] = *reinterpret_cast<const uint4 *>(src + (int64_t)r * sld + dd);
            }
        };
        auto st_nat = [&](bf16 *img, const uint4 (&v)[NIT]) {
#pragma unroll
            for (int i = 0; i < NIT; ++i) {
                const int u = lane + 64 * i, r = u / CPR, dd = (u % CPR) * 8;
                if (u < NCH) *reinterpret_cast<uint4 *>(img + r * d.ld + (SWZ ? (dd ^ (((r >> 2) & 1) << 4)) : dd)) = v[i];
            }
        };
        ld_nat(q, ld3, sq); ld_nat(k, ld3, sk); ld_nat(dO, d.E, so);
#pragma unroll
        for (int j = 0; j < NT; ++j)
#pragma unroll
            for (int kd = 0; kd < KD; ++kd) {
                vf[j][kd] = gfrag(v, ld3, j * 16, d.S, kd * 32, d.Dh, lane);
                if (!SWZ) kf[j][kd] = gfrag(k, ld3, j * 16, d.S, kd * 32, d.Dh, lane);
            }
        st_nat(Qimg, sq); st_nat(Kimg, sk); st_nat(Oimg, so);
    } else {
        stage_nat<SWZ>(Qimg, d.ld, q, ld3, d.S, NT * 16, d.Dh, lane);
        stage_nat<SWZ>(Kimg, d.ld, k, ld3, d.S, NT * 16, d.Dh, lane);
        stage_nat<SWZ>(Oimg, d.ld, dO, d.E, d.S, NT * 16, d.Dh, lane);
#pragma unroll
        for (int j = 0; j < NT; ++j)
#pragma unroll
            for (int kd = 0; kd < KD; ++kd) {
                vf[j][kd] = gfrag(v, ld3, j * 16, d.S, kd * 32, d.Dh, lane);
                if (!SWZ) kf[j][kd] = gfrag(k, ld3, j * 16, d.S, kd * 32, d.Dh, lane);
            }
    }
    lds_sync();
    auto lfrag = [&](const bf16 *img, int row0) {
        const int r = row0 + cq, col = 8 * g;
        return *reinterpret_cast<const bf16x8 *>(img + r * d.ld + (col ^ (((r >> 2) & 1) << 4)));
    };
    if (SWZ) {
#pragma unroll
        for (int j = 0; j < NT; ++j) kf[j][0] = lfrag(Kimg, j * 16);
    }
    const float scale = 1.0f / sqrtf((float)d.Dh);
    const f32x4 zero = {0.f, 0.f, 0.f, 0.f};
    bf16 *dst = dqkv + (int64_t)b * d.S * ld3 + h * d.Dh;

    f32x4 dv[NT][ND], dk[NT][ND];
#pragma unroll
    for (int j = 0; j < NT; ++j)
#pragma unroll
        for (int jd = 0; jd < ND; ++jd) { dv[j][jd] = zero; dk[j][jd] = zero; }

#pragma unroll 1
    for (int it = 0; it < NT; ++it) {
        bf16x8 qf[KD], of[KD];
#pragma unroll
        for (int kd = 0; kd < KD; ++kd) {
            if (SWZ) { qf[kd] = lfrag(Qimg, it * 16); of[kd] = lfrag(Oimg, it * 16); }
            else {
                qf[kd] = gfrag(q, ld3, it * 16, d.S, kd * 32, d.Dh, lane);
                of[kd] = gfrag(dO, d.E, it * 16, d.S, kd * 32, d.Dh, lane);
            }
        }
        f32x4 dS[NT];
        {
            f32x4 sc[NT], dp[NT];
#pragma unroll
            for (int j = 0; j < NT; ++j) {
                sc[j] = zero; dp[j] = zero;
#pragma unroll
                for (int kd = 0; kd < KD; ++kd) {
                    sc[j] = mma(qf[kd], kf[j][kd], sc[j]);
                    dp[j] = mma(of[kd], vf[j][kd], dp[j]);
                }
            }
#pragma unroll
            for (int r = 0; r < 4; ++r) {
                float m = -INFINITY;
#pragma unroll
                for (int j = 0; j < NT; ++j) {
                    const bool ok = j * 16 + cq < d.S;
                    sc[j][r] = ok ? sc[j][r] * scale : -INFINITY;
                    m = fmaxf(m, sc[j][r]);
                }
                m = g16_max(m);
                float sum = 0.f;
#pragma unroll
                for (int j = 0; j < NT; ++j) {
                    const float e = (j * 16 + cq < d.S) ? __expf(sc[j][r] - m) : 0.f;
                    sc[j][r] = e;
                    sum += e;
                }
                const float inv = 1.f / g16_sum(sum);
                float delta = 0.f;
#pragma unroll
                for (int j = 0; j < NT; ++j) {
                    sc[j][r] *= inv;
                    delta += sc[j][r] * dp[j][r];
                }
                delta = g16_sum(delta);
#pragma unroll
                for (int j = 0; j < NT; ++j) dp[j][r] = scale * sc[j][r] * (dp[j][r] - delta);
            }
#pragma unroll
            for (int jd = 0; jd < ND; ++jd) {
                const k16_t bo = tr4<SWZ>(Oimg, d.ld, it * 16 + 4 * g, jd * 16, lane);
                const k16_t bq = tr4<SWZ>(Qimg, d.ld, it * 16 + 4 * g, jd * 16, lane);
#pragma unroll
                for (int j = 0; j < NT; ++j) {
                    dv[j][jd] = mma16(pack4(sc[j]), bo, dv[j][jd]);
                    dk[j][jd] = mma16(pack4(dp[j]), bq, dk[j][jd]);
                }
            }
#pragma unroll
            for (int j = 0; j < NT; ++j) dS[j] = dp[j];
        }
        {
            lds_sync();
#pragma unroll
            for (int j = 0; j < NT; ++j) *reinterpret_cast<k16_t *>(Simg + (j * 16 + cq) * 16 + 4 * g) = pack4(dS[j]);
            lds_sync();
#pragma unroll
            for (int jd = 0; jd < ND; ++jd) {
                f32x4 dq = zero;
#pragma unroll
                for (int j = 0; j < NT; ++j)
                    dq = mma16(tr4(Simg, 16, j * 16 + 4 * g, 0, lane), tr4<SWZ>(Kimg, d.ld, j * 16 + 4 * g, jd * 16, lane), dq);
#pragma unroll
                for (int r = 0; r < 4; ++r) {
                    const int row = it * 16 + 4 * g + r;
                    if (row < d.S) dst[(int64_t)row * ld3 + jd * 16 + cq] = from_f32<bf16>(dq[r]);
                }
            }
        }
    }
#pragma unroll
    for (int j = 0; j < NT; ++j)
#pragma unroll
        for (int jd = 0; jd < ND; ++jd)
#pragma unroll
            for (int r = 0; r < 4; ++r) {
                const int key = j * 16 + 4 * g + r;
                if (key < d.S) {
                    bf16 *o = dst + (int64_t)key * ld3 + jd * 16 + cq;
                    o[d.E] = from_f32<bf16>(dk[j][jd][r]);
                    o[2 * d.E] = from_f32<bf16>(dv[j][jd][r]);
                }
            }
}

FastDims make_fast(int B, int S, int H, int Dh) {
    FastDims d;
    d.B = B; d.S = S; d.H = H; d.Dh = Dh; d.E = H * Dh;
    const int NT = (S + 15) / 16, NP = (NT + 1) / 2;
    d.ld = Dh + 8;
    d.img = NP * 32 * d.ld;
    return d;
}

static int waves_per_block(size_t per_wave_bytes) {
    const int w = (int)((size_t)160 * 1024 / per_wave_bytes);
    return w < 1 ? 1 : (w > 4 ? 4 : w);
}

template <int NT, int ND>
int fwd_launch(const bf16 *qkv, bf16 *ctx, const FastDims &d, hipStream_t s) {
    const size_t per_wave = (size_t)d.img * sizeof(bf16);
    const int wpb = waves_per_block(per_wave);
    auto kern = attn_fwd_fast<NT, ND>;
    if (per_wave * wpb > 64 * 1024)
        MIVIT_HIP(hipFuncSetAttribute(reinterpret_cast<const void *>(kern), hipFuncAttributeMaxDynamicSharedMemorySize, (int)(per_wave * wpb)));
    ProfScope prof(s);
    hipLaunchKernelGGL(kern, dim3(ceil_div(d.B * d.H, wpb)), dim3(64 * wpb), per_wave * wpb, s, qkv, ctx, d);
    MIVIT_LAUNCH_CHECK();
    return 0;
}
template <int NT, int ND>
int bwd_launch(const bf16 *qkv, const bf16 *dctx, bf16 *dqkv, const FastDims &d, hipStream_t s) {
    const size_t per_wave = (size_t)3 * d.img * sizeof(bf16);
    const int wpb = waves_per_block(per_wave);
    static const int version = getenv("MIVIT_ATTN_BWD") ? atoi(getenv("MIVIT_ATTN_BWD")) : 2;
    auto kern = version == 2 ? attn_bwd_fast2<NT, ND> : attn_bwd_fast<NT, ND>;
    if (version == 2) {
        FastDims d2 = d;
        if (ND == 2) d2.ld = 32;
        d2.img = NT * 16 * d2.ld;
        const size_t pw = ((size_t)3 * d2.img + NT * 256) * sizeof(bf16);
        const int w2 = waves_per_block(pw);
        if (pw * w2 > 64 * 1024)
            MIVIT_HIP(hipFuncSetAttribute(reinterpret_cast<const void *>(kern), hipFuncAttributeMaxDynamicSharedMemorySize, (int)(pw * w2)));
        ProfScope prof(s);
        hipLaunchKernelGGL(kern, dim3(ceil_div(d.B * d.H, w2)), dim3(64 * w2), pw * w2, s, qkv, dctx, dqkv, d2);
        MIVIT_LAUNCH_CHECK();
        return 0;
    }
    if (per_wave * wpb > 64 * 1024)
        MIVIT_HIP(hipFuncSetAttribute(reinterpret_cast<const void *>(kern), hipFuncAttributeMaxDynamicSharedMemorySize, (int)(per_wave * wpb)));
    ProfScope prof(s);
    hipLaunchKernelGGL(kern, dim3(ceil_div(d.B * d.H, wpb)), dim3(64 * wpb), per_wave * wpb, s, qkv, dctx, dqkv, d);
    MIVIT_LAUNCH_CHECK();
    return 0;
}

}

bool attention_fast_supported(int dtype, int S, int Dh) {
    if (dtype != MIVIT_ELEM_DTYPE || S < 1) return false;
    const int NT = (S + 15) / 16;
    return (Dh == 16 || Dh == 32 || Dh == 64) && NT <= 8;
}

#define FAST_DISPATCH(FN, ...)                                                 \
    switch (NT * 10 + ND) {                                                    \
        case 11: return FN<1, 1>(__VA_ARGS__);                                 \
        case 21: return FN<2, 1>(__VA_ARGS__);                                 \
        case 31: return FN<3, 1>(__VA_ARGS__);                                 \
        case 41: return FN<4, 1>(__VA_ARGS__);                                 \
        case 12: return FN<1, 2>(__VA_ARGS__);                                 \
        case 22: return FN<2, 2>(__VA_ARGS__);                                 \
        case 32: return FN<3, 2>(__VA_ARGS__);                                 \
        case 42: return FN<4, 2>(__VA_ARGS__);                                 \
        case 14: return FN<1, 4>(__VA_ARGS__);                                 \
        case 24: return FN<2, 4>(__VA_ARGS__);                                 \
        case 34: return FN<3, 4>(__VA_ARGS__);                                 \
        case 44: return FN<4, 4>(__VA_ARGS__);                                 \
        case 51: return FN<5, 1>(__VA_ARGS__);                                 \
        case 52: return FN<5, 2>(__VA_ARGS__);                                 \
        case 54: return FN<5, 4>(__VA_ARGS__);                                 \
        case 61: return FN<6, 1>(__VA_ARGS__);                                 \
        case 62: return FN<6, 2>(__VA_ARGS__);                                 \
        case 71: return FN<7, 1>(__VA_ARGS__);                                 \
        case 72: return FN<7, 2>(__VA_ARGS__);                                 \
        case 81: return FN<8, 1>(__VA_ARGS__);                                 \
        case 82: return FN<8, 2>(__VA_ARGS__);                                 \
        case 64: return FN<6, 4>(__VA_ARGS__);                                 \
        case 74: return FN<7, 4>(__VA_ARGS__);                                 \
        case 84: return FN<8, 4>(__VA_ARGS__);                                 \
        default: MIVIT_FAIL("attention fast path: unsupported tile shape");    \
    }

int launch_attention_fwd_fast(const void *qkv, int B, int S, int H, int Dh, void *ctx, hipStream_t s) {
    const FastDims d = make_fast(B, S, H, Dh);
    const int NT = (S + 15) / 16, ND = Dh / 16;
    FAST_DISPATCH(fwd_launch, static_cast<const bf16 *>(qkv), static_cast<bf16 *>(ctx), d, s)
}

int launch_attention_bwd_fast(const void *qkv, const void *dctx, int B, int S, int H, int Dh, void *dqkv, hipStream_t s) {
    const FastDims d = make_fast(B, S, H, Dh);
    const int NT = (S + 15) / 16, ND = Dh / 16;
    FAST_DISPATCH(bwd_launch, static_cast<const bf16 *>(qkv), static_cast<const bf16 *>(dctx), static_cast<bf16 *>(dqkv), d, s)
}
```

### moleculardiffusion_mivit_amd/csrc/common.h

```cpp
#pragma once
#include <hip/hip_runtime.h>
#include <stdint.h>
#include <stddef.h>
#include <stdio.h>
#include <string>
#include <functional>

#include "../../include/mivit_hip.h"

void mivit_set_error(const char *fmt, ...);
#define MIVIT_FAIL(...)                 \
    do {                                \
        mivit_set_error(__VA_ARGS__);   \
        return 1;                       \
    } while (0)
#define MIVIT_CHECK(cond, ...)          \
    do {                                \
        if (!(cond)) MIVIT_FAIL(__VA_ARGS__); \
    } while (0)
#define MIVIT_HIP(call)                                                                       \
    do {                                                                                      \
        hipError_t e_ = (call);                                                               \
        if (e_ != hipSuccess) MIVIT_FAIL("%s failed: %s (%s:%d)", #call, hipGetErrorString(e_), __FILE__, __LINE__); \
    } while (0)
#define MIVIT_LAUNCH_CHECK()                                                                  \
    do {                                                                                      \
        hipError_t e_ = hipGetLastError();                                                    \
        if (e_ != hipSuccess) MIVIT_FAIL("kernel launch failed: %s (%s:%d)", hipGetErrorString(e_), __FILE__, __LINE__); \
    } while (0)

template <int KIND>
struct h16 {
    uint16_t v;
};
typedef h16<0> bf16;
typedef h16<1> f16;

typedef __attribute__((ext_vector_type(4))) float f32x4;
typedef __attribute__((ext_vector_type(8))) __bf16 bf16x8;
typedef __attribute__((ext_vector_type(8))) _Float16 f16x8;

__device__ __forceinline__ float to_f32(float x) { return x; }
__device__ __forceinline__ float to_f32(bf16 x) { return __uint_as_float(((uint32_t)x.v) << 16); }
__device__ __forceinline__ float to_f32(f16 x) { return (float)__builtin_bit_cast(_Float16, x.v); }

template <typename T>
__device__ __forceinline__ T from_f32(float x);
template <>
__device__ __forceinline__ float from_f32<float>(float x) {
    return x;
}
template <>
__device__ __forceinline__ bf16 from_f32<bf16>(float x) {
    __bf16 b = (__bf16)x;
    bf16 r;
    r.v = __builtin_bit_cast(unsigned short, b);
    return r;
}

static inline size_t dtype_size(int dtype) { return dtype == MIVIT_F32 ? 4 : 2; }

__device__ __forceinline__ float act_fwd(int act, float u) {
    switch (act) {
        case MIVIT_ACT_RELU: return u > 0.f ? u : 0.f;
        case MIVIT_ACT_LEAKY_RELU: return u > 0.f ? u : 0.01f * u;
        case MIVIT_ACT_GELU: return 0.5f * u * (1.f + erff(u * 0.70710678118654752f));
        default: return u;
    }
}
__device__ __forceinline__ float act_bwd(int act, float saved) {
    switch (act) {
        case MIVIT_ACT_RELU: return saved > 0.f ? 1.f : 0.f;
        case MIVIT_ACT_LEAKY_RELU: return saved > 0.f ? 1.f : 0.01f;
        case MIVIT_ACT_GELU: {
            const float u = saved;
            const float cdf = 0.5f * (1.f + erff(u * 0.70710678118654752f));
            const float pdf = 0.3989422804014327f * __expf(-0.5f * u * u);
            return cdf + u * pdf;
        }
        default: return 1.f;
    }
}

template <typename T>
struct Mma;

template <>
struct Mma<float> {
    static constexpr int KS = 4;
    typedef float Frag;
    static __device__ __forceinline__ Frag load(const float *img, int rs, int ks, int r0, int k0, int lane) {
        return img[(r0 + (lane & 15)) * rs + (k0 + (lane >> 4)) * ks];
    }
    static __device__ __forceinline__ f32x4 mma(Frag a, Frag b, f32x4 c) {
        return __builtin_amdgcn_mfma_f32_16x16x4f32(a, b, c, 0, 0, 0);
    }
};

template <>
struct Mma<bf16> {
    static constexpr int KS = 32;
    typedef bf16x8 Frag;
    static __device__ __forceinline__ Frag load(const bf16 *img, int rs, int , int r0, int k0, int lane) {
        return *reinterpret_cast<const bf16x8 *>(img + (r0 + (lane & 15)) * rs + k0 + 8 * (lane >> 4));
    }
    static __device__ __forceinline__ f32x4 mma(Frag a, Frag b, f32x4 c) {
        return __builtin_amdgcn_mfma_f32_16x16x32_bf16(a, b, c, 0, 0, 0);
    }
};

template <>
struct Mma<f16> {
    static constexpr int KS = 32;
    typedef f16x8 Frag;
    static __device__ __forceinline__ Frag load(const f16 *img, int rs, int , int r0, int k0, int lane) {
        return *reinterpret_cast<const f16x8 *>(img + (r0 + (lane & 15)) * rs + k0 + 8 * (lane >> 4));
    }
    static __device__ __forceinline__ f32x4 mma(Frag a, Frag b, f32x4 c) {
        return __builtin_amdgcn_mfma_f32_16x16x32_f16(a, b, c, 0, 0, 0);
    }
};

template <int CTRL>
__device__ __forceinline__ float dpp_mov(float v) {
    return __builtin_bit_cast(float, __builtin_amdgcn_update_dpp(0, __builtin_bit_cast(int, v), CTRL, 0xf, 0xf, false));
}
__device__ __forceinline__ float row16_sum(float v) {
    v += dpp_mov<0x128>(v); v += dpp_mov<0x124>(v); v += dpp_mov<0x122>(v); return v + dpp_mov<0x121>(v);
}
__device__ __forceinline__ float row16_max(float v) {
    v = fmaxf(v, dpp_mov<0x128>(v)); v = fmaxf(v, dpp_mov<0x124>(v)); v = fmaxf(v, dpp_mov<0x122>(v)); return fmaxf(v, dpp_mov<0x121>(v));
}
__device__ __forceinline__ void rows_swap32(float &a, float &b) { asm volatile("s_nop 1\n\tv_permlane32_swap_b32 %0, %1\n\ts_nop 1" : "+v"(a), "+v"(b)); }
__device__ __forceinline__ void rows_swap16(float &a, float &b) { asm volatile("s_nop 1\n\tv_permlane16_swap_b32 %0, %1\n\ts_nop 1" : "+v"(a), "+v"(b)); }
__device__ __forceinline__ float rows4_sum(float v) {
    float a = v, b = v;
    rows_swap32(a, b);
    float t = a + b, c = t;
    rows_swap16(t, c);
    return t + c;
}
__device__ __forceinline__ float rows4_max(float v) {
    float a = v, b = v;
    rows_swap32(a, b);
    float t = fmaxf(a, b), c = t;
    rows_swap16(t, c);
    return fmaxf(t, c);
}

__device__ __forceinline__ float wave_sum(float v) {
#pragma unroll
    for (int o = 32; o > 0; o >>= 1) v += __shfl_xor(v, o, 64);
    return v;
}
__device__ __forceinline__ float wave_max(float v) {
#pragma unroll
    for (int o = 32; o > 0; o >>= 1) v = fmaxf(v, __shfl_xor(v, o, 64));
    return v;
}

template <>
__device__ __forceinline__ f16 from_f32<f16>(float x) {
    f16 r;
    r.v = __builtin_bit_cast(unsigned short, (_Float16)x);
    return r;
}
__device__ __forceinline__ void load16(const float *p, float *out) {
    const float4 v = *reinterpret_cast<const float4 *>(p);
    out[0] = v.x; out[1] = v.y; out[2] = v.z; out[3] = v.w;
}
__device__ __forceinline__ void load16(const bf16 *p, float *out) {
    const uint4 v = *reinterpret_cast<const uint4 *>(p);
    const uint32_t w[4] = {v.x, v.y, v.z, v.w};
#pragma unroll
    for (int i = 0; i < 4; ++i) {
        out[2 * i] = __uint_as_float(w[i] << 16);
        out[2 * i + 1] = __uint_as_float(w[i] & 0xffff0000u);
    }
}
__device__ __forceinline__ void load16(const f16 *p, float *out) {
    const f16x8 v = *reinterpret_cast<const f16x8 *>(p);
#pragma unroll
    for (int i = 0; i < 8; ++i) out[i] = (float)v[i];
}
__device__ __forceinline__ void store16(f16 *p, const float *v) {
    f16x8 o;
#pragma unroll
    for (int i = 0; i < 8; ++i) o[i] = (_Float16)v[i];
    *reinterpret_cast<f16x8 *>(p) = o;
}
__device__ __forceinline__ void store16(float *p, const float *v) {
    *reinterpret_cast<float4 *>(p) = make_float4(v[0], v[1], v[2], v[3]);
}
__device__ __forceinline__ void store16(bf16 *p, const float *v) {
    uint32_t w[4];
#pragma unroll
    for (int i = 0; i < 4; ++i)
        w[i] = (uint32_t)from_f32<bf16>(v[2 * i]).v | ((uint32_t)from_f32<bf16>(v[2 * i + 1]).v << 16);
    *reinterpret_cast<uint4 *>(p) = make_uint4(w[0], w[1], w[2], w[3]);
}

static inline int ceil_div(int a, int b) { return (a + b - 1) / b; }
static inline size_t align_up(size_t x, size_t a) { return (x + a - 1) / a * a; }

struct LinearFwdArgs {
    int dtype;
    const void *x; int x_is_f32; int64_t ldx;
    const void *W; int w_is_bf16;
    const float *bias;
    int M, N, K, act;
    const void *resid; int64_t ldr;
    void *y; int64_t ldy; void *y_preact;
    int map_rows, map_stride, map_off;
    int y_is_f32;
};
int launch_linear_fwd(const LinearFwdArgs &a, hipStream_t s);

struct LinearDgradArgs {
    int dtype;
    const void *dy; int dy_is_f32; int64_t lddy;
    const void *W; int w_is_bf16;
    int M, N, K;
    int act; const void *saved; int64_t lds;
    const void *dres; int64_t lddr;
    void *dx; int64_t lddx; int dx_is_f32;
};
int launch_linear_dgrad(const LinearDgradArgs &a, hipStream_t s);

struct LinearWgradArgs {
    int dtype;
    const void *dy; int dy_is_f32; int64_t lddy;
    const void *x; int x_is_f32; int64_t ldx;
    int M, N, K;
    float *dW; float *db; int accumulate;
    void *ws; size_t ws_bytes;
};
size_t linear_wgrad_ws_bytes(int M, int N, int K);
int launch_linear_wgrad(const LinearWgradArgs &a, hipStream_t s);

struct LayerNormFwdArgs {
    int dtype;
    const void *z; int64_t ldz; const float *gamma; const float *beta;
    int M, E;
    void *y; int64_t ldy; int rows_per_seq, out_seq_stride, out_row_off;
    const float *pos; float *mean; float *rstd;
    int in_rows, in_stride, in_off;
};
int launch_layernorm_fwd(const LayerNormFwdArgs &a, hipStream_t s);

struct LayerNormBwdArgs {
    int dtype;
    const void *dy; int64_t lddy; const void *z; int64_t ldz;
    const float *gamma; const float *mean; const float *rstd;
    int M, E;
    int rows_per_seq, in_seq_stride, in_row_off;
    int z_rows, z_stride, z_off;
    void *dz; int64_t lddz;
    float *dgamma; float *dbeta; int accumulate;
    float *dzsum;
    void *ws; size_t ws_bytes;
};
size_t layernorm_bwd_ws_bytes(int M, int E);
int launch_layernorm_bwd(const LayerNormBwdArgs &a, hipStream_t s);

int launch_attention_fwd(int dtype, const void *qkv, int B, int S, int H, int Dh, void *ctx, hipStream_t s);
int launch_attention_bwd(int dtype, const void *qkv, const void *dctx, int B, int S, int H, int Dh, void *dqkv,
                         hipStream_t s);
int attention_max_seq(int dtype, int Dh);
bool attention_fast_supported(int dtype, int S, int Dh);
int launch_attention_fwd_fast(const void *qkv, int B, int S, int H, int Dh, void *ctx, hipStream_t s);
int launch_attention_bwd_fast(const void *qkv, const void *dctx, int B, int S, int H, int Dh, void *dqkv, hipStream_t s);

bool embed_dma_supported(int dtype, int M, int K, int E);
int launch_embed_fwd_dma(const float *X, const void *W_bf16, const float *bias, void *Y, int M, int K, int E, hipStream_t s);
size_t embed_wgrad_dma_ws_bytes(int M, int K, int E);
int launch_embed_wgrad_dma(const void *dY_bf16, const float *X, float *dW, int M, int K, int E, void *ws, size_t ws_bytes,
                           hipStream_t s);

bool rowstream_supported(int M, int N, int K, bool dgrad, int64_t lda, int64_t ldw, const void *A, const void *W);
int launch_rowstream(bool dgrad, const void *A, int64_t lda, const void *W_bf16, int64_t ldw, int M, int N, int K,
                     const float *bias, int act, const void *dact, int64_t ldd, int dact_kind, const void *resid,
                     int64_t ldr, void *Cout, int64_t ldc, void *C2, const float *gamma, const float *beta, void *Y,
                     int64_t ldy, float *mean, float *rstd, hipStream_t s);

bool wavestream_supported(int M, int N, int K, bool dgrad, int64_t lda, int64_t ldw, const void *A, const void *W);
int launch_wavestream(bool dgrad, const void *A, int64_t lda, const void *W_bf16, int64_t ldw, int M, int N, int K,
                      const float *bias, int act, const void *dact, int64_t ldd, int dact_kind, const void *resid,
                      int64_t ldr, void *Cout, int64_t ldc, void *C2, const float *gamma, const float *beta, void *Y,
                      int64_t ldy, float *mean, float *rstd, hipStream_t s);

bool gemm_dma_supported(int M, int NC, int KC, bool dgrad);
int launch_gemm_dma_fwd(const void *x, int64_t ldx, const void *W_bf16, const float *bias, int M, int N, int K, int act,
                        const void *resid, int64_t ldr, void *y, int64_t ldy, void *y_preact, hipStream_t s);
int launch_gemm_dma_dgrad(const void *dy, int64_t lddy, const void *W_bf16, int M, int N, int K, int act, const void *saved,
                          int64_t lds, const void *dres, int64_t lddr, void *dx, int64_t lddx, hipStream_t s);

bool wgrad_dma_supported(int M, int N, int K, int64_t lddy, int64_t ldx, const void *dy, const void *x);
size_t wgrad_dma_ws_bytes(int M, int N, int K);
int launch_wgrad_dma(const void *dy, int64_t lddy, const void *x, int64_t ldx, int M, int N, int K, float *dW, float *db,
                     void *ws, size_t ws_bytes, hipStream_t s);

bool wgrad_small_supported(int M, int N, int K, int64_t lddy, int64_t ldx, const void *dy, const void *x);
size_t wgrad_small_ws_bytes(int M, int N, int K);
int launch_wgrad_small(const void *dy, int64_t lddy, const void *x, int64_t ldx, int M, int N, int K, float *dW, float *db,
                       void *ws, size_t ws_bytes, hipStream_t s);


bool embed_small_fwd_supported(int M, int K, int E, const void *X, const void *Y);
int launch_embed_small_fwd(const float *X, const void *W_bf16, const float *bias, void *Y, int M, int K, int E, hipStream_t s);
bool embed_small_wgrad_supported(int M, int N, int K, int64_t lddy, const void *dy, const void *x);
size_t embed_small_wgrad_ws_bytes(int M, int N, int K);
int launch_embed_small_wgrad(const void *dy, int64_t lddy, const float *x, int M, int N, int K, float *dW, float *db, void *ws,
                             size_t ws_bytes, hipStream_t s);

bool embed_small_fwd_supported_f16(int M, int K, int E, const void *X, const void *Y);
int launch_embed_small_fwd_f16(const float *X, const void *W_bf16, const float *bias, void *Y, int M, int K, int E, hipStream_t s);
bool embed_small_wgrad_supported_f16(int M, int N, int K, int64_t lddy, const void *dy, const void *x);
size_t embed_small_wgrad_ws_bytes_f16(int M, int N, int K);
int launch_embed_small_wgrad_f16(const void *dy, int64_t lddy, const float *x, int M, int N, int K, float *dW, float *db, void *ws,
                             size_t ws_bytes, hipStream_t s);

bool attention_fast_supported_f16(int dtype, int S, int Dh);
int launch_attention_fwd_fast_f16(const void *qkv, int B, int S, int H, int Dh, void *ctx, hipStream_t s);
int launch_attention_bwd_fast_f16(const void *qkv, const void *dctx, int B, int S, int H, int Dh, void *dqkv, hipStream_t s);
bool embed_dma_supported_f16(int dtype, int M, int K, int E);
int launch_embed_fwd_dma_f16(const float *X, const void *W_bf16, const float *bias, void *Y, int M, int K, int E, hipStream_t s);
size_t embed_wgrad_dma_ws_bytes_f16(int M, int K, int E);
int launch_embed_wgrad_dma_f16(const void *dY_bf16, const float *X, float *dW, int M, int K, int E, void *ws, size_t ws_bytes,
                           hipStream_t s);
bool rowstream_supported_f16(int M, int N, int K, bool dgrad, int64_t lda, int64_t ldw, const void *A, const void *W);
int launch_rowstream_f16(bool dgrad, const void *A, int64_t lda, const void *W_bf16, int64_t ldw, int M, int N, int K,
                     const float *bias, int act, const void *dact, int64_t ldd, int dact_kind, const void *resid,
                     int64_t ldr, void *Cout, int64_t ldc, void *C2, const float *gamma, const float *beta, void *Y,
                     int64_t ldy, float *mean, float *rstd, hipStream_t s);
bool wavestream_supported_f16(int M, int N, int K, bool dgrad, int64_t lda, int64_t ldw, const void *A, const void *W);
int launch_wavestream_f16(bool dgrad, const void *A, int64_t lda, const void *W_bf16, int64_t ldw, int M, int N, int K,
                      const float *bias, int act, const void *dact, int64_t ldd, int dact_kind, const void *resid,
                      int64_t ldr, void *Cout, int64_t ldc, void *C2, const float *gamma, const float *beta, void *Y,
                      int64_t ldy, float *mean, float *rstd, hipStream_t s);
bool wgrad_dma_supported_f16(int M, int N, int K, int64_t lddy, int64_t ldx, const void *dy, const void *x);
size_t wgrad_dma_ws_bytes_f16(int M, int N, int K);
int launch_wgrad_dma_f16(const void *dy, int64_t lddy, const void *x, int64_t ldx, int M, int N, int K, float *dW, float *db,
                     void *ws, size_t ws_bytes, hipStream_t s);
bool wgrad_small_supported_f16(int M, int N, int K, int64_t lddy, int64_t ldx, const void *dy, const void *x);
size_t wgrad_small_ws_bytes_f16(int M, int N, int K);
int launch_wgrad_small_f16(const void *dy, int64_t lddy, const void *x, int64_t ldx, int M, int N, int K, float *dW, float *db,
                       void *ws, size_t ws_bytes, hipStream_t s);

int launch_slab_reduce(const float *part, int nparts, int64_t n, float *out, int accumulate, hipStream_t s);
int launch_slab_reduce_strided(const float *part, int nparts, int64_t stride, int64_t n, float *out, hipStream_t s);
int launch_slab_reduce3(const float *p0, float *o0, const float *p1, float *o1, const float *p2, float *o2, int nparts,
                        int n, int accumulate, hipStream_t s);
int launch_reg_token_fill(int dtype, void *tokens, int B, int S, int E, const float *reg, const void *add,
                          const float *pos, hipStream_t s);
int launch_mean_pool_fwd(int dtype, const void *x, int B, int S, int E, void *out, hipStream_t s);
int launch_mean_pool_bwd(int dtype, const void *dout, int B, int S, int E, void *dx, hipStream_t s);
size_t batch_colsum_ws_bytes(int B, int rows, int E);
int launch_batch_colsum(int dtype, const void *x, int B, int S, int E, int s0, int rows, float *out, void *ws,
                        size_t ws_bytes, hipStream_t s);
int launch_convert(int src_is_f32, const void *src, int64_t lds_, int dst_dtype_is_f32, void *dst, int64_t ldd,
                   int rows, int cols, int accumulate, hipStream_t s, int dtype16 = MIVIT_BF16);
int launch_fill_zero(void *p, size_t bytes, hipStream_t s);
int launch_affine_fixup(float *dW, const float *db, const float *gamma, const float *beta, int N, int K, hipStream_t s);

void prof_set_tag(int tag);
void prof_pin_tag(int tag);
bool prof_begin(hipStream_t s);
void prof_end(hipStream_t s);
struct ProfScope {
    hipStream_t s; bool on;
    explicit ProfScope(hipStream_t st) : s(st), on(prof_begin(st)) {}
    ~ProfScope() { if (on) prof_end(s); }
};
struct ProfPin {
    explicit ProfPin(int tag) { prof_pin_tag(tag); }
    ~ProfPin() { prof_pin_tag(-1); }
    void set(int tag) { prof_pin_tag(tag); }
};

int graph_run(const uint64_t *key, int nkey, hipStream_t s, const std::function<int(hipStream_t)> &body);
```

### moleculardiffusion_mivit_amd/csrc/elem.h

```cpp
#pragma once
#ifdef MIVIT_ELEM_F16
#define MIVIT_ELEM_DTYPE MIVIT_F16
#define bf16 f16
#define bf16x8 f16x8
#define __bf16 _Float16
#define tr_pair tr_pair_f16
#define rowstream_supported rowstream_supported_f16
#define launch_rowstream launch_rowstream_f16
#define wavestream_supported wavestream_supported_f16
#define launch_wavestream launch_wavestream_f16
#define wgrad_dma_supported wgrad_dma_supported_f16
#define wgrad_dma_ws_bytes wgrad_dma_ws_bytes_f16
#define launch_wgrad_dma launch_wgrad_dma_f16
#define embed_small_fwd_supported embed_small_fwd_supported_f16
#define launch_embed_small_fwd launch_embed_small_fwd_f16
#define embed_small_wgrad_supported embed_small_wgrad_supported_f16
#define embed_small_wgrad_ws_bytes embed_small_wgrad_ws_bytes_f16
#define launch_embed_small_wgrad launch_embed_small_wgrad_f16
#define wgrad_small_supported wgrad_small_supported_f16
#define wgrad_small_ws_bytes wgrad_small_ws_bytes_f16
#define launch_wgrad_small launch_wgrad_small_f16
#define attention_fast_supported attention_fast_supported_f16
#define launch_attention_fwd_fast launch_attention_fwd_fast_f16
#define launch_attention_bwd_fast launch_attention_bwd_fast_f16
#define embed_dma_supported embed_dma_supported_f16
#define launch_embed_fwd_dma launch_embed_fwd_dma_f16
#define embed_wgrad_dma_ws_bytes embed_wgrad_dma_ws_bytes_f16
#define launch_embed_wgrad_dma launch_embed_wgrad_dma_f16
#define mivit_rowstream_fwd mivit_rowstream_fwd_f16
#define mivit_rowstream_dgrad mivit_rowstream_dgrad_f16
#define mivit_rowstream_set_wavestream mivit_rowstream_set_wavestream_f16
#define mivit_rowstream_set_wavestream_mask mivit_rowstream_set_wavestream_mask_f16
#define mivit_wavestream_fwd mivit_wavestream_fwd_f16
#define mivit_wavestream_dgrad mivit_wavestream_dgrad_f16
#define mivit_wgrad_bf16_workspace_bytes mivit_wgrad_bf16_workspace_bytes_f16
#define mivit_wgrad_bf16 mivit_wgrad_bf16_f16
#define mivit_wgrad_bf16_set_config mivit_wgrad_bf16_set_config_f16
#define mivit_wgrad_small_workspace_bytes mivit_wgrad_small_workspace_bytes_f16
#define mivit_wgrad_small mivit_wgrad_small_f16
#define mivit_embed_small_supported mivit_embed_small_supported_f16
#define mivit_embed_small_fwd mivit_embed_small_fwd_f16
#define mivit_embed_small_wgrad_workspace_bytes mivit_embed_small_wgrad_workspace_bytes_f16
#define mivit_embed_small_wgrad mivit_embed_small_wgrad_f16
#define mivit_embed_set_variant mivit_embed_set_variant_f16
#define mivit_embed_fwd_bf16 mivit_embed_fwd_bf16_f16
#define mivit_embed_wgrad_bf16_workspace_bytes mivit_embed_wgrad_bf16_workspace_bytes_f16
#define mivit_embed_wgrad_bf16 mivit_embed_wgrad_bf16_f16
#define ELEM_MFMA_16x16x16(a, b, c)                                                                                       \
    __builtin_amdgcn_mfma_f32_16x16x16f16(__builtin_bit_cast(__attribute__((ext_vector_type(4))) _Float16, a),            \
                                          __builtin_bit_cast(__attribute__((ext_vector_type(4))) _Float16, b), c, 0, 0, 0)
__device__ __forceinline__ float elem_lo(uint32_t w) { return (float)__builtin_bit_cast(_Float16, (uint16_t)(w & 0xffffu)); }
__device__ __forceinline__ float elem_hi(uint32_t w) { return (float)__builtin_bit_cast(_Float16, (uint16_t)(w >> 16)); }
#else
#define MIVIT_ELEM_DTYPE MIVIT_BF16
#define ELEM_MFMA_16x16x16(a, b, c) __builtin_amdgcn_mfma_f32_16x16x16bf16_1k(a, b, c, 0, 0, 0)
__device__ __forceinline__ float elem_lo(uint32_t w) { return __uint_as_float(w << 16); }
__device__ __forceinline__ float elem_hi(uint32_t w) { return __uint_as_float(w & 0xffff0000u); }
#endif

#if defined(MIVIT_WIDTH64) && defined(MIVIT_ELEM_F16)
#define MIVIT_FUSED_NAME(x) x##_w64_f16
#elif defined(MIVIT_WIDTH64)
#define MIVIT_FUSED_NAME(x) x##_w64
#elif defined(MIVIT_ELEM_F16)
#define MIVIT_FUSED_NAME(x) x##_f16
#endif
#ifdef MIVIT_FUSED_NAME
#define fused_layer_supported MIVIT_FUSED_NAME(fused_layer_supported)
#define launch_attn_block_fwd MIVIT_FUSED_NAME(launch_attn_block_fwd)
#define launch_mlp_block_fwd MIVIT_FUSED_NAME(launch_mlp_block_fwd)
#define mlp_block_bwd_ws_bytes MIVIT_FUSED_NAME(mlp_block_bwd_ws_bytes)
#define launch_mlp_block_bwd MIVIT_FUSED_NAME(launch_mlp_block_bwd)
#define attn_out_bwd_ws_bytes MIVIT_FUSED_NAME(attn_out_bwd_ws_bytes)
#define launch_attn_out_bwd MIVIT_FUSED_NAME(launch_attn_out_bwd)
#define qkv_bwd_ws_bytes MIVIT_FUSED_NAME(qkv_bwd_ws_bytes)
#define launch_qkv_bwd MIVIT_FUSED_NAME(launch_qkv_bwd)
#define mivit_fused_layer_supported MIVIT_FUSED_NAME(mivit_fused_layer_supported)
#define mivit_mlp_block_fwd MIVIT_FUSED_NAME(mivit_mlp_block_fwd)
#define mivit_attn_block_fwd MIVIT_FUSED_NAME(mivit_attn_block_fwd)
#define mivit_mlp_block_bwd_workspace_bytes MIVIT_FUSED_NAME(mivit_mlp_block_bwd_workspace_bytes)
#define mivit_mlp_block_bwd_set_waves MIVIT_FUSED_NAME(mivit_mlp_block_bwd_set_waves)
#define mivit_mlp_block_bwd MIVIT_FUSED_NAME(mivit_mlp_block_bwd)
#define mivit_attn_out_bwd_workspace_bytes MIVIT_FUSED_NAME(mivit_attn_out_bwd_workspace_bytes)
#define mivit_attn_out_bwd MIVIT_FUSED_NAME(mivit_attn_out_bwd)
#define mivit_qkv_bwd_workspace_bytes MIVIT_FUSED_NAME(mivit_qkv_bwd_workspace_bytes)
#define mivit_qkv_bwd MIVIT_FUSED_NAME(mivit_qkv_bwd)
#define mivit_qkv_bwd_affine MIVIT_FUSED_NAME(mivit_qkv_bwd_affine)
#endif
```

### moleculardiffusion_mivit_amd/csrc/engine.hip

```cpp
#include "common.h"
#include "slab_defer.h"
#include <atomic>
#include <algorithm>

#include <string>
#include <vector>

#define MIVIT_FUSED_DECLS(SFX)                                                                                                     \
    bool fused_layer_supported##SFX(int dtype, int E, int F, int H, int S);                                                        \
    int launch_attn_block_fwd##SFX(const void *nin, const float *gin, const float *bin, const void *Wqkv, const float *bqkv,       \
                                   const void *Wo, const float *bo, const float *gout, const float *bout, int B, int S, void *ctx, \
                                   void *nout, float *rstd, void *xout, void *zout, float *mean, void *qkvout, hipStream_t s);     \
    int launch_mlp_block_fwd##SFX(const void *nin, const float *gin, const float *bin, const void *W1, const float *b1,            \
                                  const void *W2, const float *b2, const float *gout, const float *bout, int M, int act,           \
                                  void *nout, float *rstd, void *xout, void *zout, float *mean, void *hout, void *uout,            \
                                  hipStream_t s);                                                                                  \
    size_t mlp_block_bwd_ws_bytes##SFX(int M);                                                                                     \
    size_t attn_out_bwd_ws_bytes##SFX(int M);                                                                                      \
    int launch_attn_out_bwd##SFX(const void *dy, const void *n1, const float *rstd1, const float *gamma1, const void *ctx,         \
                                 const void *Wo, int M, void *dz1, void *dctx, float *dWo, float *dbo, float *dgamma1,             \
                                 float *dbeta1, void *ws, size_t ws_bytes, hipStream_t s);                                         \
    int launch_mlp_block_bwd##SFX(const void *dy, const void *n2, const float *rstd2, const float *gamma2, const void *n1,         \
                                  const float *gamma1, const float *beta1, const void *W1, const float *b1, const void *W2, int M, \
                                  int act, void *dx1, float *dW1, float *db1, float *dW2, float *db2, float *dgamma2,              \
                                  float *dbeta2, void *ws, size_t ws_bytes, hipStream_t s);                                        \
    size_t qkv_bwd_ws_bytes##SFX(int M);                                                                                           \
    int launch_qkv_bwd##SFX(const void *dqkv, const void *x, const void *Wqkv, const void *res, int M, void *dx, float *dW,        \
                            float *db, const float *fix_gamma, const float *fix_beta, void *ws, size_t ws_bytes, hipStream_t s);
MIVIT_FUSED_DECLS()
MIVIT_FUSED_DECLS(_f16)
MIVIT_FUSED_DECLS(_w64)
MIVIT_FUSED_DECLS(_w64_f16)
#undef MIVIT_FUSED_DECLS

struct FusedOps {
    decltype(&fused_layer_supported) ok;
    decltype(&launch_attn_block_fwd) attn_fwd;
    decltype(&launch_mlp_block_fwd) mlp_fwd;
    decltype(&launch_mlp_block_bwd) mlp_bwd;
    decltype(&launch_attn_out_bwd) attn_out_bwd;
    decltype(&mlp_block_bwd_ws_bytes) mlp_bwd_ws;
    decltype(&attn_out_bwd_ws_bytes) attn_out_bwd_ws;
    decltype(&launch_qkv_bwd) qkv_bwd;
    decltype(&qkv_bwd_ws_bytes) qkv_bwd_ws;
};
#define MIVIT_FUSED_TABLE(SFX)                                                                                                \
    {fused_layer_supported##SFX, launch_attn_block_fwd##SFX, launch_mlp_block_fwd##SFX, launch_mlp_block_bwd##SFX,            \
     launch_attn_out_bwd##SFX, mlp_block_bwd_ws_bytes##SFX, attn_out_bwd_ws_bytes##SFX, launch_qkv_bwd##SFX, qkv_bwd_ws_bytes##SFX}
static const FusedOps kFusedBf16 = MIVIT_FUSED_TABLE(), kFusedF16 = MIVIT_FUSED_TABLE(_f16), kFusedBf16W64 = MIVIT_FUSED_TABLE(_w64),
                      kFusedF16W64 = MIVIT_FUSED_TABLE(_w64_f16);
#undef MIVIT_FUSED_TABLE
static const FusedOps *fused_ops(int dtype, int E) {
    static const bool f16_off = getenv("MIVIT_NO_F16_STREAM") != nullptr, w64_off = getenv("MIVIT_NO_FUSED_W64") != nullptr;
    if (E == 64 && w64_off) return nullptr;
    if (dtype == MIVIT_BF16) return E == 64 ? &kFusedBf16W64 : &kFusedBf16;
    if (dtype == MIVIT_F16 && !f16_off) return E == 64 ? &kFusedF16W64 : &kFusedF16;
    return nullptr;
}
static bool fused_ok(int dtype, int E, int F, int H, int S) {
    const FusedOps *f = fused_ops(dtype, E);
    return f && f->ok(dtype, E, F, H, S);
}

struct ParamInfo {
    std::string name;
    int64_t offset, numel;
};

struct LayerParams {
    int64_t qkv_w, qkv_b, out_w, out_b, n1_w, n1_b, fc1_w, fc1_b, fc2_w, fc2_b, n2_w, n2_b;
};

struct mivit_plan {
    mivit_config c;
    std::vector<ParamInfo> params;
    std::vector<std::pair<int64_t, int64_t>> stages;
    int64_t arena;
    int64_t tn_w, tn_b, fp0_w, fp0_b, fp2_w, fp2_b, h0_w, h0_b, h3_w, h3_b;
    std::vector<LayerParams> layers;
    int64_t reg, pos, n0_w, n0_b, emb_w, emb_b;
    int head_in;
    uint64_t uid;
};

namespace {

constexpr int MAX_TOKENS = 128;

int64_t add_param(mivit_plan *p, const std::string &name, int64_t numel, bool align = true) {
    if (align) p->arena = (p->arena + 7) / 8 * 8;
    const int64_t off = p->arena;
    p->params.push_back({name, off, numel});
    p->arena += numel;
    return off;
}

void add_feature_projector(mivit_plan *p) {
    const int E = p->c.embed_dim, G = p->c.global_feature_dim;
    p->fp0_w = add_param(p, "feature_projector.0.weight", (int64_t)E * G);
    p->fp0_b = add_param(p, "feature_projector.0.bias", E);
    p->fp2_w = add_param(p, "feature_projector.2.weight", (int64_t)E * E);
    p->fp2_b = add_param(p, "feature_projector.2.bias", E);
}

struct Ws {
    size_t total;
    size_t wsh;
    size_t emb, mean0, rstd0, x0;
    struct L { size_t qkv, ctx, z1, x1, h, u, z2, x2, mean1, rstd1, mean2, rstd2; };
    std::vector<L> layer;
    size_t xF, meanF, rstdF, pooled, fp_h, fp_out, head_in, hh;
    size_t xL;
    size_t dout_t, d_hh, d_head_in, d_pool_c, d_fp_h, dxa, dxb, dF, dctx, dqkv, wgrad, ln, colsum;
    size_t wgrad_bytes, ln_bytes, colsum_bytes;
};

Ws make_ws(const mivit_plan *p, int B, int T, bool bwd) {
    const mivit_config &c = p->c;
    const size_t ts = dtype_size(c.dtype);
    const int E = c.embed_dim, F = c.hidden_dim, L = c.num_layers;
    const int S = T + (c.use_regression_token ? 1 : 0);
    const size_t M = (size_t)B * S, Mt = (size_t)B * T;
    Ws w = {};
    size_t off = 0;
    auto take = [&](size_t bytes) { size_t o = off; off += align_up(bytes, 256); return o; };
    w.wsh = c.dtype != MIVIT_F32 ? take((size_t)p->arena * 2) : 0;
    w.emb = take(Mt * E * ts); w.mean0 = take(Mt * 4); w.rstd0 = take(Mt * 4);
    w.x0 = take(M * E * ts);
    const int nsets = bwd ? L : 1;
    const bool fused = L > 0 && fused_ok(c.dtype, E, F, c.num_heads, S);
    for (int l = 0; l < nsets; ++l) {
        Ws::L s;
        if (fused) {
            s.qkv = bwd ? take(M * 3 * E * ts) : 0; s.ctx = take(M * E * ts); s.z1 = take(M * E * ts); s.x1 = 0;
            s.h = 0; s.u = 0;
            s.z2 = take(M * E * ts); s.x2 = 0;
            s.mean1 = s.mean2 = 0; s.rstd1 = take(M * 4); s.rstd2 = take(M * 4);
        } else {
            s.qkv = take(M * 3 * E * ts); s.ctx = take(M * E * ts); s.z1 = take(M * E * ts); s.x1 = take(M * E * ts);
            s.h = take(M * F * ts); s.u = c.activation == MIVIT_ACT_GELU ? take(M * F * ts) : 0;
            s.z2 = take(M * E * ts); s.x2 = take(M * E * ts);
            s.mean1 = take(M * 4); s.rstd1 = take(M * 4); s.mean2 = take(M * 4); s.rstd2 = take(M * 4);
        }
        w.layer.push_back(s);
    }
    for (int l = nsets; l < L; ++l) w.layer.push_back(w.layer[0]);
    w.xL = fused ? take(M * E * ts) : 0;
    w.xF = c.use_regression_token ? 0 : take(M * E * ts);
    w.meanF = take(M * 4); w.rstdF = take(M * 4);
    w.pooled = take((size_t)B * E * ts);
    w.fp_h = take((size_t)B * E * ts); w.fp_out = take((size_t)B * E * ts);
    w.head_in = take((size_t)B * 2 * E * ts);
    w.hh = take((size_t)B * c.head_hidden * ts);
    if (bwd) {
        w.dout_t = take((size_t)B * c.output_dim * ts);
        w.d_hh = take((size_t)B * c.head_hidden * ts);
        w.d_head_in = take((size_t)B * 2 * E * ts);
        w.d_pool_c = take((size_t)B * E * ts);
        w.d_fp_h = take((size_t)B * E * ts);
        w.dxa = take(M * E * ts); w.dxb = take(M * E * ts);
        w.dF = take(M * F * ts); w.dctx = take(M * E * ts); w.dqkv = take(M * 3 * E * ts);
        size_t wg = 0;
        auto mx = [&](int m, int n, int k) {
            size_t b = linear_wgrad_ws_bytes(m, n, k);
            if (c.dtype != MIVIT_F32 && n % 128 == 0 && k % 128 == 0 && m >= 256) b += wgrad_dma_ws_bytes(m, n, k);
            if (c.dtype != MIVIT_F32 && m >= 256) b = std::max(b, wgrad_small_ws_bytes(m, n, k));
            if (c.dtype != MIVIT_F32 && m >= 256) b = std::max(b, embed_small_wgrad_ws_bytes(m, n, k));
            if (b > wg) wg = b;
        };
        mx((int)M, 3 * E, E); mx((int)M, E, E); mx((int)M, F, E); mx((int)M, E, F);
        if (fused) {
            const FusedOps *fo = fused_ops(c.dtype, E);
            wg = std::max(wg, fo->mlp_bwd_ws((int)M) + fo->attn_out_bwd_ws((int)M) + fo->qkv_bwd_ws((int)M));
        }
        if (c.embedding != MIVIT_EMBED_EXTERNAL) {
            mx((int)Mt, E, c.patch_size * c.patch_size);
            if ((c.dtype == MIVIT_F16 ? embed_dma_supported_f16 : embed_dma_supported)(c.dtype, (int)Mt, c.patch_size * c.patch_size, E)) {
                const size_t b = embed_wgrad_dma_ws_bytes((int)Mt, c.patch_size * c.patch_size, E);
                if (b > wg) wg = b;
            }
        }
        mx(B, c.head_hidden, p->head_in); mx(B, c.output_dim, c.head_hidden);
        if (c.fusion != MIVIT_FUSION_NONE) { mx(B, E, E); mx(B, E, c.global_feature_dim); }
        w.wgrad_bytes = wg; w.wgrad = take(wg);
        w.ln_bytes = layernorm_bwd_ws_bytes((int)M, E); w.ln = take(w.ln_bytes);
        w.colsum_bytes = batch_colsum_ws_bytes(B, S, E); w.colsum = take(w.colsum_bytes);
    }
    w.total = off;
    return w;
}

inline void *at(void *base, size_t off) { return static_cast<char *>(base) + off; }
inline const void *at(const void *base, size_t off) { return static_cast<const char *>(base) + off; }
inline void *col_ptr(void *p, size_t cols, int dtype) { return static_cast<char *>(p) + cols * dtype_size(dtype); }

#define RC(call) do { int rc_ = (call); if (rc_) return rc_; } while (0)

struct StreamOps {
    decltype(&rowstream_supported) rowstream_ok;
    decltype(&wavestream_supported) wavestream_ok;
    decltype(&launch_rowstream) rowstream;
    decltype(&wgrad_dma_supported) wgrad_dma_ok;
    decltype(&wgrad_dma_ws_bytes) wgrad_dma_ws;
    decltype(&launch_wgrad_dma) wgrad_dma;
    decltype(&wgrad_small_supported) wgrad_small_ok;
    decltype(&wgrad_small_ws_bytes) wgrad_small_ws;
    decltype(&launch_wgrad_small) wgrad_small;
    decltype(&embed_dma_supported) embed_ok;
    decltype(&launch_embed_fwd_dma) embed_fwd;
    decltype(&embed_wgrad_dma_ws_bytes) embed_wgrad_ws;
    decltype(&launch_embed_wgrad_dma) embed_wgrad;
    decltype(&embed_small_fwd_supported) embed_small_fwd_ok;
    decltype(&launch_embed_small_fwd) embed_small_fwd;
    decltype(&embed_small_wgrad_supported) embed_small_wgrad_ok;
    decltype(&embed_small_wgrad_ws_bytes) embed_small_wgrad_ws;
    decltype(&launch_embed_small_wgrad) embed_small_wgrad;
};
static const StreamOps kStreamBf16 = {rowstream_supported, wavestream_supported, launch_rowstream, wgrad_dma_supported, wgrad_dma_ws_bytes,
                                      launch_wgrad_dma, wgrad_small_supported, wgrad_small_ws_bytes, launch_wgrad_small,
                                      embed_dma_supported, launch_embed_fwd_dma, embed_wgrad_dma_ws_bytes, launch_embed_wgrad_dma,
                                      embed_small_fwd_supported, launch_embed_small_fwd, embed_small_wgrad_supported,
                                      embed_small_wgrad_ws_bytes, launch_embed_small_wgrad};
static const StreamOps kStreamF16 = {rowstream_supported_f16, wavestream_supported_f16, launch_rowstream_f16, wgrad_dma_supported_f16,
                                     wgrad_dma_ws_bytes_f16, launch_wgrad_dma_f16, wgrad_small_supported_f16, wgrad_small_ws_bytes_f16,
                                     launch_wgrad_small_f16, embed_dma_supported_f16, launch_embed_fwd_dma_f16,
                                     embed_wgrad_dma_ws_bytes_f16, launch_embed_wgrad_dma_f16, embed_small_fwd_supported_f16,
                                     launch_embed_small_fwd_f16, embed_small_wgrad_supported_f16, embed_small_wgrad_ws_bytes_f16,
                                     launch_embed_small_wgrad_f16};
static const StreamOps *stream_ops(int dtype) {
    static const bool f16_off = getenv("MIVIT_NO_F16_STREAM") != nullptr;
    return dtype == MIVIT_BF16 ? &kStreamBf16 : (dtype == MIVIT_F16 && !f16_off ? &kStreamF16 : nullptr);
}
static bool stream_gemm_supported(const StreamOps *so, int M, int N, int K, bool dgrad, int64_t lda, int64_t ldw, const void *A, const void *W) {
    return so && (so->rowstream_ok(M, N, K, dgrad, lda, ldw, A, W) || so->wavestream_ok(M, N, K, dgrad, lda, ldw, A, W));
}

int lin_fwd(int dtype, const void *x, int x_f32, int64_t ldx, const void *W, const float *b, int M, int N, int K,
            int act, const void *resid, int64_t ldr, void *y, int64_t ldy, void *pre, int y_f32, hipStream_t s) {
    const StreamOps *so = stream_ops(dtype);
    if (!x_f32 && !y_f32 && stream_gemm_supported(so, M, N, K, false, ldx, K, x, W) &&
        (!resid || ldr % 8 == 0) && ldy % 8 == 0) {
        prof_set_tag(MIVIT_PROF_LINEAR_FWD);
        return so->rowstream(false, x, ldx, W, K, M, N, K, b, act, nullptr, 0, 0, resid, ldr, y, ldy, pre, nullptr,
                                nullptr, nullptr, 0, nullptr, nullptr, s);
    }
    if (dtype == MIVIT_BF16 && !x_f32 && !y_f32 && gemm_dma_supported(M, N, K, false) && ldx % 8 == 0 && ldy % 8 == 0 &&
        (!resid || ldr % 8 == 0) && ((reinterpret_cast<uintptr_t>(x) | reinterpret_cast<uintptr_t>(W) | reinterpret_cast<uintptr_t>(y) |
                                      reinterpret_cast<uintptr_t>(resid) | reinterpret_cast<uintptr_t>(pre)) & 15) == 0) {
        prof_set_tag(MIVIT_PROF_LINEAR_FWD);
        return launch_gemm_dma_fwd(x, ldx, W, b, M, N, K, act, resid, ldr, y, ldy, pre, s);
    }
    if (so && x_f32 && !y_f32 && ldx == K && ldy == N && act == MIVIT_ACT_NONE && !resid && !pre &&
        so->embed_small_fwd_ok(M, K, N, x, y)) {
        prof_set_tag(MIVIT_PROF_EMBED_FWD);
        return so->embed_small_fwd(static_cast<const float *>(x), W, b, y, M, K, N, s);
    }
    LinearFwdArgs a = {};
    a.dtype = dtype; a.x = x; a.x_is_f32 = x_f32 || dtype == MIVIT_F32; a.ldx = ldx; a.W = W;
    a.w_is_bf16 = dtype != MIVIT_F32; a.bias = b;
    a.M = M; a.N = N; a.K = K; a.act = act; a.resid = resid; a.ldr = ldr; a.y = y; a.ldy = ldy; a.y_preact = pre;
    a.y_is_f32 = y_f32;
    prof_set_tag(x_f32 && K > 1024 ? MIVIT_PROF_EMBED_FWD : MIVIT_PROF_LINEAR_FWD);
    return launch_linear_fwd(a, s);
}
int lin_dgrad(int dtype, const void *dy, int64_t lddy, const void *W, int M, int N, int K, int act, const void *saved,
              int64_t lds, const void *dres, int64_t lddr, void *dx, int64_t lddx, int dx_f32, hipStream_t s) {
    const StreamOps *so = stream_ops(dtype);
    if (!dx_f32 && stream_gemm_supported(so, M, K, N, true, lddy, K, dy, W) && lddx % 8 == 0 &&
        (!dres || lddr % 8 == 0) && (act == MIVIT_ACT_NONE || lds % 8 == 0)) {
        prof_set_tag(MIVIT_PROF_LINEAR_DGRAD);
        return so->rowstream(true, dy, lddy, W, K, M, K, N, nullptr, MIVIT_ACT_NONE, act != MIVIT_ACT_NONE ? saved : nullptr,
                                lds, act, dres, lddr, dx, lddx, nullptr, nullptr, nullptr, nullptr, 0, nullptr, nullptr, s);
    }
    if (dtype == MIVIT_BF16 && !dx_f32 && gemm_dma_supported(M, K, N, true) && lddy % 8 == 0 && lddx % 8 == 0 &&
        (!dres || lddr % 8 == 0) && (act == MIVIT_ACT_NONE || lds % 8 == 0) &&
        ((reinterpret_cast<uintptr_t>(dy) | reinterpret_cast<uintptr_t>(W) | reinterpret_cast<uintptr_t>(dx) |
          reinterpret_cast<uintptr_t>(dres) | reinterpret_cast<uintptr_t>(act != MIVIT_ACT_NONE ? saved : nullptr)) & 15) == 0) {
        prof_set_tag(MIVIT_PROF_LINEAR_DGRAD);
        return launch_gemm_dma_dgrad(dy, lddy, W, M, N, K, act, saved, lds, dres, lddr, dx, lddx, s);
    }
    LinearDgradArgs a = {};
    a.dtype = dtype; a.dy = dy; a.dy_is_f32 = dtype == MIVIT_F32; a.lddy = lddy; a.W = W;
    a.w_is_bf16 = dtype != MIVIT_F32; a.M = M; a.N = N; a.K = K;
    a.act = act; a.saved = saved; a.lds = lds; a.dres = dres; a.lddr = lddr; a.dx = dx; a.lddx = lddx; a.dx_is_f32 = dx_f32;
    prof_set_tag(MIVIT_PROF_LINEAR_DGRAD);
    return launch_linear_dgrad(a, s);
}
int lin_wgrad(int dtype, const void *dy, int64_t lddy, const void *x, int x_f32, int64_t ldx, int M, int N, int K,
              float *dW, float *db, void *ws, size_t wsb, hipStream_t s) {
    const StreamOps *so = stream_ops(dtype);
    if (so && !x_f32 && dW && so->wgrad_dma_ok(M, N, K, lddy, ldx, dy, x) &&
        wsb >= so->wgrad_dma_ws(M, N, K) + linear_wgrad_ws_bytes(M, N, K)) {
        prof_set_tag(MIVIT_PROF_LINEAR_WGRAD);
        return so->wgrad_dma(dy, lddy, x, ldx, M, N, K, dW, db, ws, wsb, s);
    }
    if (so && !x_f32 && dW && so->wgrad_small_ok(M, N, K, lddy, ldx, dy, x) &&
        wsb >= so->wgrad_small_ws(M, N, K) && wsb >= linear_wgrad_ws_bytes(M, N, K)) {
        prof_set_tag(MIVIT_PROF_LINEAR_WGRAD);
        return so->wgrad_small(dy, lddy, x, ldx, M, N, K, dW, db, ws, wsb, s);
    }
    if (so && x_f32 && dW && ldx == K && so->embed_small_wgrad_ok(M, N, K, lddy, dy, x) && wsb >= so->embed_small_wgrad_ws(M, N, K)) {
        prof_set_tag(MIVIT_PROF_EMBED_WGRAD);
        return so->embed_small_wgrad(dy, lddy, static_cast<const float *>(x), M, N, K, dW, db, ws, wsb, s);
    }
    LinearWgradArgs a = {};
    a.dtype = dtype; a.dy = dy; a.dy_is_f32 = dtype == MIVIT_F32; a.lddy = lddy; a.x = x;
    a.x_is_f32 = x_f32 || dtype == MIVIT_F32; a.ldx = ldx; a.M = M; a.N = N; a.K = K; a.dW = dW; a.db = db;
    a.ws = ws; a.ws_bytes = wsb;
    prof_set_tag(x_f32 && K > 1024 ? MIVIT_PROF_EMBED_WGRAD : MIVIT_PROF_LINEAR_WGRAD);
    return launch_linear_wgrad(a, s);
}

int lin_res_ln(int dtype, const void *x, int64_t ldx, const void *W, const float *b, int M, int N, int K, const void *resid,
               void *z, const float *gamma, const float *beta, void *y, float *mean, float *rstd, hipStream_t s) {
    const StreamOps *so = stream_ops(dtype);
    if ((N == 128 || N == 64) && stream_gemm_supported(so, M, N, K, false, ldx, K, x, W)) {
        prof_set_tag(MIVIT_PROF_LINEAR_FWD);
        return so->rowstream(false, x, ldx, W, K, M, N, K, b, MIVIT_ACT_NONE, nullptr, 0, 0, resid, N, z, N, nullptr, gamma,
                                beta, y, N, mean, rstd, s);
    }
    RC(lin_fwd(dtype, x, 0, ldx, W, b, M, N, K, MIVIT_ACT_NONE, resid, N, z, N, nullptr, 0, s));
    LayerNormFwdArgs n = {};
    n.dtype = dtype; n.z = z; n.ldz = N; n.gamma = gamma; n.beta = beta; n.M = M; n.E = N; n.y = y; n.ldy = N;
    n.mean = mean; n.rstd = rstd;
    prof_set_tag(MIVIT_PROF_LN_FWD);
    return launch_layernorm_fwd(n, s);
}

int ln_bwd_bias(LayerNormBwdArgs &a, float *db, bool *need_colsum, hipStream_t s) {
    a.dzsum = db;
    prof_set_tag(MIVIT_PROF_LN_BWD);
    const int rc = launch_layernorm_bwd(a, s);
    *need_colsum = (rc == 2);
    return rc == 2 ? 0 : rc;
}

int check_call(const mivit_plan *plan, int B, int T, size_t ws_bytes, bool bwd, const char *who) {
    MIVIT_CHECK(plan, "%s: null plan", who);
    MIVIT_CHECK(B > 0 && T > 0, "%s: empty batch (B=%d, T=%d)", who, B, T);
    const int S = T + (plan->c.use_regression_token ? 1 : 0);
    MIVIT_CHECK(!plan->c.use_pos_encoding || S <= MAX_TOKENS, "%s: %d tokens exceed the %d-entry positional table",
                who, S, MAX_TOKENS);
    const int Dh = plan->c.embed_dim / plan->c.num_heads;
    MIVIT_CHECK(S <= attention_max_seq(plan->c.dtype, Dh),
                "%s: sequence of %d tokens (head dim %d) does not fit the LDS-resident attention kernel (max %d)", who, S,
                Dh, attention_max_seq(plan->c.dtype, Dh));
    MIVIT_CHECK((int64_t)B * S * 3 * plan->c.embed_dim < (1ll << 31) && (int64_t)B * S * plan->c.hidden_dim < (1ll << 31),
                "%s: batch too large for 32-bit row indexing", who);
    const Ws w = make_ws(plan, B, T, bwd);
    MIVIT_CHECK(ws_bytes >= w.total, "%s: workspace too small (%zu < %zu bytes)", who, ws_bytes, w.total);
    return 0;
}

}

extern "C" mivit_plan *mivit_plan_create(const mivit_config *cfg) {
    if (!cfg) { mivit_set_error("plan_create: null config"); return nullptr; }
    const mivit_config &c = *cfg;
#define PLAN_CHECK(cond, ...) do { if (!(cond)) { mivit_set_error(__VA_ARGS__); return nullptr; } } while (0)
    PLAN_CHECK(c.abi_version == MIVIT_ABI_VERSION, "plan_create: ABI version %d != %d", c.abi_version, MIVIT_ABI_VERSION);
    PLAN_CHECK(c.dtype == MIVIT_F32 || c.dtype == MIVIT_BF16 || c.dtype == MIVIT_F16, "plan_create: bad dtype %d", c.dtype);
    PLAN_CHECK(c.embedding >= MIVIT_EMBED_LINEAR && c.embedding <= MIVIT_EMBED_EXTERNAL, "plan_create: bad embedding %d", c.embedding);
    PLAN_CHECK(c.embed_dim > 0 && c.num_heads > 0 && c.hidden_dim > 0 && c.num_layers >= 0, "plan_create: bad model dims");
    PLAN_CHECK(c.embed_dim % c.num_heads == 0, "embed_dim must be divisible by num_heads");
    PLAN_CHECK(c.embed_dim <= 1024, "plan_create: embed_dim %d > 1024 is not supported", c.embed_dim);
    PLAN_CHECK(c.embedding == MIVIT_EMBED_EXTERNAL || c.patch_size > 0, "plan_create: bad patch_size");
    PLAN_CHECK(c.activation >= MIVIT_ACT_RELU && c.activation <= MIVIT_ACT_GELU, "plan_create: unsupported activation %d", c.activation);
    PLAN_CHECK(c.fusion >= MIVIT_FUSION_NONE && c.fusion <= MIVIT_FUSION_LATE, "plan_create: bad fusion %d", c.fusion);
    PLAN_CHECK(c.fusion == MIVIT_FUSION_NONE || c.global_feature_dim > 0, "Must provide global_feature_dim if using global features");
    PLAN_CHECK(c.fusion != MIVIT_FUSION_EARLY || c.use_regression_token, "plan_create: early fusion needs the regression token");
    PLAN_CHECK(c.head_hidden > 0 && c.output_dim > 0, "plan_create: bad head dims");
#undef PLAN_CHECK
    mivit_plan *p = new mivit_plan();
    static std::atomic<uint64_t> next_uid{1};
    p->uid = next_uid.fetch_add(1);
    p->c = c;
    p->arena = 0;
    const int E = c.embed_dim, F = c.hidden_dim;
    p->head_in = c.fusion == MIVIT_FUSION_LATE ? 2 * E : E;
    int64_t b0 = p->arena;
    p->tn_w = add_param(p, "transformer.norm.weight", E);
    p->tn_b = add_param(p, "transformer.norm.bias", E);
    if (c.fusion == MIVIT_FUSION_LATE) add_feature_projector(p);
    p->h0_w = add_param(p, "mlp_head.mlp.0.weight", (int64_t)c.head_hidden * p->head_in);
    p->h0_b = add_param(p, "mlp_head.mlp.0.bias", c.head_hidden);
    p->h3_w = add_param(p, "mlp_head.mlp.3.weight", (int64_t)c.output_dim * c.head_hidden);
    p->h3_b = add_param(p, "mlp_head.mlp.3.bias", c.output_dim);
    p->arena = (p->arena + 7) / 8 * 8;
    p->stages.push_back({b0, p->arena});
    p->layers.resize(c.num_layers);
    for (int l = c.num_layers - 1; l >= 0; --l) {
        b0 = p->arena;
        const std::string pre = "transformer.encoder_layers." + std::to_string(l) + ".";
        LayerParams &lp = p->layers[l];
        lp.qkv_w = add_param(p, pre + "self_attn.q_proj.weight", (int64_t)E * E);
        add_param(p, pre + "self_attn.k_proj.weight", (int64_t)E * E, false);
        add_param(p, pre + "self_attn.v_proj.weight", (int64_t)E * E, false);
        lp.qkv_b = add_param(p, pre + "self_attn.q_proj.bias", E);
        add_param(p, pre + "self_attn.k_proj.bias", E, false);
        add_param(p, pre + "self_attn.v_proj.bias", E, false);
        lp.out_w = add_param(p, pre + "self_attn.out_proj.weight", (int64_t)E * E);
        lp.out_b = add_param(p, pre + "self_attn.out_proj.bias", E);
        lp.n1_w = add_param(p, pre + "norm1.weight", E);
        lp.n1_b = add_param(p, pre + "norm1.bias", E);
        lp.fc1_w = add_param(p, pre + "feed_forward.fc1.weight", (int64_t)F * E);
        lp.fc1_b = add_param(p, pre + "feed_forward.fc1.bias", F);
        lp.fc2_w = add_param(p, pre + "feed_forward.fc2.weight", (int64_t)E * F);
        lp.fc2_b = add_param(p, pre + "feed_forward.fc2.bias", E);
        lp.n2_w = add_param(p, pre + "norm2.weight", E);
        lp.n2_b = add_param(p, pre + "norm2.bias", E);
        p->arena = (p->arena + 7) / 8 * 8;
        p->stages.push_back({b0, p->arena});
    }
    b0 = p->arena;
    p->reg = c.use_regression_token ? add_param(p, "reg_token", E) : -1;
    p->pos = c.use_pos_encoding ? add_param(p, "transformer.pos_embedding", (int64_t)MAX_TOKENS * E) : -1;
    p->n0_w = add_param(p, "norm.weight", E);
    p->n0_b = add_param(p, "norm.bias", E);
    if (c.fusion == MIVIT_FUSION_EARLY) add_feature_projector(p);
    p->emb_w = p->emb_b = -1;
    if (c.embedding == MIVIT_EMBED_LINEAR) {
        p->emb_w = add_param(p, "embedding.proj.weight", (int64_t)E * c.patch_size * c.patch_size);
        p->emb_b = add_param(p, "embedding.proj.bias", E);
    } else if (c.embedding == MIVIT_EMBED_CNN) {
        p->emb_w = add_param(p, "embedding.conv.weight", (int64_t)E * c.patch_size * c.patch_size);
        p->emb_b = add_param(p, "embedding.conv.bias", E);
    }
    p->arena = (p->arena + 7) / 8 * 8;
    p->stages.push_back({b0, p->arena});
    if ((int64_t)E * E % 4 != 0 || E % 4 != 0) {
        mivit_set_error("plan_create: embed_dim must be a multiple of 4 (got %d)", E);
        delete p;
        return nullptr;
    }
    return p;
}

extern "C" void mivit_plan_destroy(mivit_plan *plan) { delete plan; }
extern "C" int mivit_plan_num_params(const mivit_plan *plan) { return plan ? (int)plan->params.size() : 0; }
extern "C" const char *mivit_plan_param_name(const mivit_plan *plan, int i) {
    return (plan && i >= 0 && i < (int)plan->params.size()) ? plan->params[i].name.c_str() : nullptr;
}
extern "C" int64_t mivit_plan_param_offset(const mivit_plan *plan, int i) {
    return (plan && i >= 0 && i < (int)plan->params.size()) ? plan->params[i].offset : -1;
}
extern "C" int64_t mivit_plan_param_numel(const mivit_plan *plan, int i) {
    return (plan && i >= 0 && i < (int)plan->params.size()) ? plan->params[i].numel : -1;
}
extern "C" int64_t mivit_plan_arena_numel(const mivit_plan *plan) { return plan ? plan->arena : 0; }
extern "C" int mivit_plan_num_stages(const mivit_plan *plan) { return plan ? (int)plan->stages.size() : 0; }
extern "C" int mivit_plan_stage_range(const mivit_plan *plan, int stage, int64_t *begin, int64_t *end) {
    MIVIT_CHECK(plan && stage >= 0 && stage < (int)plan->stages.size(), "stage_range: bad stage %d", stage);
    if (begin) *begin = plan->stages[stage].first;
    if (end) *end = plan->stages[stage].second;
    return 0;
}
extern "C" size_t mivit_plan_workspace_bytes(const mivit_plan *plan, int B, int T, int need_backward) {
    if (!plan || B <= 0 || T <= 0) return 0;
    return make_ws(plan, B, T, need_backward != 0).total;
}

namespace {

struct Call {
    const mivit_plan *plan; const mivit_config &cfg;
    const int dt, E, F, H, Dh, L, B, T, off, S, M, Mt, f32;
    const bool bwd;
    const bool fused;
    const FusedOps *fo;
    const Ws w;
    void *ws; const float *P; float *G; hipStream_t s;
    Call(const mivit_plan *p, int B_, int T_, bool bwd_, void *workspace, const float *params, float *grads, void *stream)
        : plan(p), cfg(p->c), dt(cfg.dtype), E(cfg.embed_dim), F(cfg.hidden_dim), H(cfg.num_heads), Dh(E / H), L(cfg.num_layers),
          B(B_), T(T_), off(cfg.use_regression_token ? 1 : 0), S(T + off), M(B * S), Mt(B * T), f32(dt == MIVIT_F32), bwd(bwd_),
          fused(L > 0 && fused_ok(dt, E, F, H, S)), fo(fused ? fused_ops(dt, E) : nullptr), w(make_ws(p, B, T, bwd)),
          ws(workspace), P(params), G(grads), s(static_cast<hipStream_t>(stream)) {}
    void *buf(size_t o) const { return at(ws, o); }
    float *fbuf(size_t o) const { return static_cast<float *>(at(ws, o)); }
    const float *p(int64_t o) const { return P + o; }
    float *g(int64_t o) const { return G + o; }
    const void *W(int64_t o) const { return f32 ? (const void *)(P + o) : (const void *)(static_cast<const bf16 *>(buf(w.wsh)) + o); }
    const void *trunk_out() const { return L == 0 ? buf(w.x0) : (fused ? buf(w.xL) : buf(w.layer[L - 1].x2)); }
};

int embed_fwd(const Call &c, const float *x) {
    const mivit_plan *p = c.plan;
    if (c.cfg.embedding == MIVIT_EMBED_EXTERNAL) return launch_convert(1, x, c.E, c.f32, c.buf(c.w.emb), c.E, c.Mt, c.E, 0, c.s, c.dt);
    const int K = c.cfg.patch_size * c.cfg.patch_size; const StreamOps *so = stream_ops(c.dt);
    if (so && so->embed_ok(c.dt, c.Mt, K, c.E)) {
        prof_set_tag(MIVIT_PROF_EMBED_FWD);
        return so->embed_fwd(x, c.W(p->emb_w), c.p(p->emb_b), c.buf(c.w.emb), c.Mt, K, c.E, c.s);
    }
    return lin_fwd(c.dt, x, 1, K, c.W(p->emb_w), c.p(p->emb_b), c.Mt, c.E, K, MIVIT_ACT_NONE, nullptr, 0, c.buf(c.w.emb), c.E, nullptr, 0, c.s);
}

int tokens_fwd(const Call &c, const float *features) {
    const mivit_plan *p = c.plan; const mivit_config &cfg = c.cfg; const Ws &w = c.w;
    const int dt = c.dt, E = c.E, B = c.B;
    LayerNormFwdArgs a = {};
    a.dtype = dt; a.z = c.buf(w.emb); a.ldz = E; a.gamma = c.p(p->n0_w); a.beta = c.p(p->n0_b); a.M = c.Mt; a.E = E;
    a.y = c.buf(w.x0); a.ldy = E; a.rows_per_seq = c.T; a.out_seq_stride = c.S; a.out_row_off = c.off;
    a.pos = cfg.use_pos_encoding ? c.p(p->pos) : nullptr; a.mean = c.fbuf(w.mean0); a.rstd = c.fbuf(w.rstd0);
    prof_set_tag(MIVIT_PROF_LN_FWD); RC(launch_layernorm_fwd(a, c.s));
    if (cfg.fusion != MIVIT_FUSION_NONE) {
        const int Fg = cfg.global_feature_dim;
        RC(lin_fwd(dt, features, 1, Fg, c.W(p->fp0_w), c.p(p->fp0_b), B, E, Fg, MIVIT_ACT_RELU, nullptr, 0, c.buf(w.fp_h), E, nullptr, 0, c.s));
        RC(lin_fwd(dt, c.buf(w.fp_h), 0, E, c.W(p->fp2_w), c.p(p->fp2_b), B, E, E, MIVIT_ACT_NONE, nullptr, 0, c.buf(w.fp_out), E, nullptr, 0, c.s));
    }
    if (cfg.use_regression_token)
        RC(launch_reg_token_fill(dt, c.buf(w.x0), B, c.S, E, c.p(p->reg), cfg.fusion == MIVIT_FUSION_EARLY ? c.buf(w.fp_out) : nullptr, a.pos, c.s));
    return 0;
}

int layers_fwd_fused(const Call &c) {
    const float *gin = nullptr, *bin = nullptr;
    const void *nin = c.buf(c.w.x0);
    for (int l = 0; l < c.L; ++l) {
        const LayerParams &lp = c.plan->layers[l]; const Ws::L &b = c.w.layer[l];
        prof_set_tag(MIVIT_PROF_ATTN_BLOCK_FWD);
        RC(c.fo->attn_fwd(nin, gin, bin, c.W(lp.qkv_w), c.p(lp.qkv_b), c.W(lp.out_w), c.p(lp.out_b), c.p(lp.n1_w), c.p(lp.n1_b), c.B, c.S,
                          c.buf(b.ctx), c.buf(b.z1), c.fbuf(b.rstd1), nullptr, nullptr, nullptr, c.bwd ? c.buf(b.qkv) : nullptr, c.s));
        prof_set_tag(MIVIT_PROF_MLP_BLOCK_FWD);
        RC(c.fo->mlp_fwd(c.buf(b.z1), c.p(lp.n1_w), c.p(lp.n1_b), c.W(lp.fc1_w), c.p(lp.fc1_b), c.W(lp.fc2_w), c.p(lp.fc2_b), c.p(lp.n2_w),
                         c.p(lp.n2_b), c.M, c.cfg.activation, c.buf(b.z2), c.fbuf(b.rstd2), l + 1 == c.L ? c.buf(c.w.xL) : nullptr,
                         nullptr, nullptr, nullptr, nullptr, c.s));
        nin = c.buf(b.z2); gin = c.p(lp.n2_w); bin = c.p(lp.n2_b);
    }
    return 0;
}

int layers_fwd_general(const Call &c) {
    const int dt = c.dt, E = c.E, F = c.F, M = c.M, act = c.cfg.activation;
    const void *xin = c.buf(c.w.x0);
    for (int l = 0; l < c.L; ++l) {
        const LayerParams &lp = c.plan->layers[l]; const Ws::L &b = c.w.layer[l];
        RC(lin_fwd(dt, xin, 0, E, c.W(lp.qkv_w), c.p(lp.qkv_b), M, 3 * E, E, MIVIT_ACT_NONE, nullptr, 0, c.buf(b.qkv), 3 * E, nullptr, 0, c.s));
        prof_set_tag(MIVIT_PROF_ATTN_FWD); RC(launch_attention_fwd(dt, c.buf(b.qkv), c.B, c.S, c.H, c.Dh, c.buf(b.ctx), c.s));
        RC(lin_res_ln(dt, c.buf(b.ctx), E, c.W(lp.out_w), c.p(lp.out_b), M, E, E, xin, c.buf(b.z1), c.p(lp.n1_w), c.p(lp.n1_b),
                      c.buf(b.x1), c.fbuf(b.mean1), c.fbuf(b.rstd1), c.s));
        RC(lin_fwd(dt, c.buf(b.x1), 0, E, c.W(lp.fc1_w), c.p(lp.fc1_b), M, F, E, act, nullptr, 0, c.buf(b.h), F,
                   act == MIVIT_ACT_GELU ? c.buf(b.u) : nullptr, 0, c.s));
        RC(lin_res_ln(dt, c.buf(b.h), F, c.W(lp.fc2_w), c.p(lp.fc2_b), M, E, F, c.buf(b.x1), c.buf(b.z2), c.p(lp.n2_w), c.p(lp.n2_b),
                      c.buf(b.x2), c.fbuf(b.mean2), c.fbuf(b.rstd2), c.s));
        xin = c.buf(b.x2);
    }
    return 0;
}

int readout_fwd(const Call &c) {
    const Ws &w = c.w; LayerNormFwdArgs a = {};
    a.dtype = c.dt; a.z = c.trunk_out(); a.ldz = c.E; a.gamma = c.p(c.plan->tn_w); a.beta = c.p(c.plan->tn_b); a.E = c.E; a.ldy = c.E;
    a.mean = c.fbuf(w.meanF); a.rstd = c.fbuf(w.rstdF);
    prof_set_tag(MIVIT_PROF_LN_FWD);
    if (c.cfg.use_regression_token) {
        a.M = c.B; a.y = c.buf(w.pooled); a.in_rows = 1; a.in_stride = c.S; a.in_off = 0;
        return launch_layernorm_fwd(a, c.s);
    }
    a.M = c.M; a.y = c.buf(w.xF); RC(launch_layernorm_fwd(a, c.s));
    return launch_mean_pool_fwd(c.dt, c.buf(w.xF), c.B, c.S, c.E, c.buf(w.pooled), c.s);
}

int head_fwd(const Call &c, float *out) {
    const mivit_plan *p = c.plan; const Ws &w = c.w;
    const int dt = c.dt, E = c.E, B = c.B, Hh = c.cfg.head_hidden, Hin = p->head_in, O = c.cfg.output_dim;
    const void *head_in = c.buf(w.pooled);
    if (c.cfg.fusion == MIVIT_FUSION_LATE) {
        RC(launch_convert(c.f32, c.buf(w.pooled), E, c.f32, c.buf(w.head_in), 2 * E, B, E, 0, c.s, dt));
        RC(launch_convert(c.f32, c.buf(w.fp_out), E, c.f32, col_ptr(c.buf(w.head_in), E, dt), 2 * E, B, E, 0, c.s, dt));
        head_in = c.buf(w.head_in);
    }
    RC(lin_fwd(dt, head_in, 0, Hin, c.W(p->h0_w), c.p(p->h0_b), B, Hh, Hin, MIVIT_ACT_RELU, nullptr, 0, c.buf(w.hh), Hh, nullptr, 0, c.s));
    return lin_fwd(dt, c.buf(w.hh), 0, Hh, c.W(p->h3_w), c.p(p->h3_b), B, O, Hh, MIVIT_ACT_NONE, nullptr, 0, out, O, nullptr, 1, c.s);
}

int forward_impl(const mivit_plan *plan, const float *params, const float *x, const float *features, int B, int T,
                        void *workspace, size_t workspace_bytes, int need_backward, float *out, void *stream) {
    RC(check_call(plan, B, T, workspace_bytes, need_backward != 0, "mivit_forward"));
    MIVIT_CHECK(params && x && workspace && out, "mivit_forward: null pointer");
    MIVIT_CHECK(plan->c.fusion == MIVIT_FUSION_NONE || features, "Global features required for %s fusion",
                plan->c.fusion == MIVIT_FUSION_EARLY ? "early" : "late");
    const Call c(plan, B, T, need_backward != 0, workspace, params, nullptr, stream);
    if (!c.f32) RC(launch_convert(1, c.P, plan->arena, 0, c.buf(c.w.wsh), plan->arena, 1, (int)plan->arena, 0, c.s, c.dt));
    RC(embed_fwd(c, x));
    RC(tokens_fwd(c, features));
    RC(c.fused ? layers_fwd_fused(c) : layers_fwd_general(c));
    RC(readout_fwd(c));
    return head_fwd(c, out);
}

int feature_projector_bwd(const Call &c, const float *features, const void *dy, int64_t lddy, float *dfeatures) {
    const mivit_plan *p = c.plan; const Ws &w = c.w;
    const int dt = c.dt, E = c.E, B = c.B, Fg = c.cfg.global_feature_dim;
    RC(lin_wgrad(dt, dy, lddy, c.buf(w.fp_h), 0, E, B, E, E, c.g(p->fp2_w), c.g(p->fp2_b), c.buf(w.wgrad), w.wgrad_bytes, c.s));
    RC(lin_dgrad(dt, dy, lddy, c.W(p->fp2_w), B, E, E, MIVIT_ACT_RELU, c.buf(w.fp_h), E, nullptr, 0, c.buf(w.d_fp_h), E, 0, c.s));
    RC(lin_wgrad(dt, c.buf(w.d_fp_h), E, features, 1, Fg, B, E, Fg, c.g(p->fp0_w), c.g(p->fp0_b), c.buf(w.wgrad), w.wgrad_bytes, c.s));
    if (dfeatures) RC(lin_dgrad(dt, c.buf(w.d_fp_h), E, c.W(p->fp0_w), B, E, Fg, MIVIT_ACT_NONE, nullptr, 0, nullptr, 0, dfeatures, Fg, 1, c.s));
    return 0;
}

int head_bwd(const Call &c, const float *dout, const float *features, float *dfeatures) {
    const mivit_plan *p = c.plan; const Ws &w = c.w;
    const int dt = c.dt, E = c.E, B = c.B, Hh = c.cfg.head_hidden, Hin = p->head_in, O = c.cfg.output_dim;
    void *wg = c.buf(w.wgrad); const size_t wgb = w.wgrad_bytes;
    const void *head_in = c.cfg.fusion == MIVIT_FUSION_LATE ? c.buf(w.head_in) : c.buf(w.pooled), *dy = dout;
    if (!c.f32) { RC(launch_convert(1, dout, O, 0, c.buf(w.dout_t), O, B, O, 0, c.s, dt)); dy = c.buf(w.dout_t); }
    RC(lin_wgrad(dt, dy, O, c.buf(w.hh), 0, Hh, B, O, Hh, c.g(p->h3_w), c.g(p->h3_b), wg, wgb, c.s));
    RC(lin_dgrad(dt, dy, O, c.W(p->h3_w), B, O, Hh, MIVIT_ACT_RELU, c.buf(w.hh), Hh, nullptr, 0, c.buf(w.d_hh), Hh, 0, c.s));
    RC(lin_wgrad(dt, c.buf(w.d_hh), Hh, head_in, 0, Hin, B, Hh, Hin, c.g(p->h0_w), c.g(p->h0_b), wg, wgb, c.s));
    RC(lin_dgrad(dt, c.buf(w.d_hh), Hh, c.W(p->h0_w), B, Hh, Hin, MIVIT_ACT_NONE, nullptr, 0, nullptr, 0, c.buf(w.d_head_in), Hin, 0, c.s));
    if (c.cfg.fusion == MIVIT_FUSION_LATE) RC(feature_projector_bwd(c, features, col_ptr(c.buf(w.d_head_in), E, dt), Hin, dfeatures));
    LayerNormBwdArgs a = {};
    a.dtype = dt; a.z = c.trunk_out(); a.ldz = E; a.gamma = c.p(p->tn_w); a.mean = c.fbuf(w.meanF); a.rstd = c.fbuf(w.rstdF);
    a.E = E; a.dz = c.buf(w.dxa); a.lddz = E; a.dgamma = c.g(p->tn_w); a.dbeta = c.g(p->tn_b); a.ws = c.buf(w.ln); a.ws_bytes = w.ln_bytes;
    if (c.cfg.use_regression_token) {
        RC(launch_fill_zero(c.buf(w.dxa), (size_t)c.M * E * dtype_size(dt), c.s));
        a.dy = c.buf(w.d_head_in); a.lddy = Hin; a.M = B; a.z_rows = 1; a.z_stride = c.S; a.z_off = 0;
    } else {
        const void *dp = c.buf(w.d_head_in);
        if (Hin != E) {
            RC(launch_convert(c.f32, c.buf(w.d_head_in), Hin, c.f32, c.buf(w.d_pool_c), E, B, E, 0, c.s, dt));
            dp = c.buf(w.d_pool_c);
        }
        RC(launch_mean_pool_bwd(dt, dp, B, c.S, E, c.buf(w.dxb), c.s));
        a.dy = c.buf(w.dxb); a.lddy = E; a.M = c.M;
    }
    prof_set_tag(MIVIT_PROF_LN_BWD);
    return launch_layernorm_bwd(a, c.s);
}

struct FusedBwdWs { bool defer; struct Region { void *ptr; size_t bytes; } mlp, attn_out, qkv; };
FusedBwdWs fused_bwd_ws(const Call &c, bool want_defer) {
    uint8_t *wg = static_cast<uint8_t *>(c.buf(c.w.wgrad));
    const size_t wgb = c.w.wgrad_bytes, n_mlp = c.fo->mlp_bwd_ws(c.M), n_ao = c.fo->attn_out_bwd_ws(c.M);
    if (!want_defer || wgb < n_mlp + n_ao + c.fo->qkv_bwd_ws(c.M)) return {false, {wg, wgb}, {wg, wgb}, {wg, wgb}};
    return {true, {wg, wgb}, {wg + n_mlp, wgb - n_mlp}, {wg + n_mlp + n_ao, wgb - n_mlp - n_ao}};
}

int layer_bwd_fused(const Call &c, int l) {
    static const bool qkv_split = getenv("MIVIT_NO_QKV_BWD") != nullptr;
    static const bool no_defer = getenv("MIVIT_NO_SLAB_DEFER") != nullptr || qkv_split;
    const Ws &w = c.w; const Ws::L &b = w.layer[l]; const LayerParams &lp = c.plan->layers[l];
    const int dt = c.dt, E = c.E, M = c.M;
    const void *xin = l > 0 ? c.buf(w.layer[l - 1].z2) : c.buf(w.x0);
    const float *gin = l > 0 ? c.p(c.plan->layers[l - 1].n2_w) : nullptr, *bin = l > 0 ? c.p(c.plan->layers[l - 1].n2_b) : nullptr;
    void *dx1 = c.buf(w.dxb), *dz1 = c.buf(w.dF);
    const FusedBwdWs r = fused_bwd_ws(c, !no_defer);
    SlabDefer slabs(r.defer);
    prof_set_tag(MIVIT_PROF_MLP_BLOCK_BWD);
    RC(c.fo->mlp_bwd(c.buf(w.dxa), c.buf(b.z2), c.fbuf(b.rstd2), c.p(lp.n2_w), c.buf(b.z1), c.p(lp.n1_w), c.p(lp.n1_b), c.W(lp.fc1_w),
                     c.p(lp.fc1_b), c.W(lp.fc2_w), M, c.cfg.activation, dx1, c.g(lp.fc1_w), c.g(lp.fc1_b), c.g(lp.fc2_w), c.g(lp.fc2_b),
                     c.g(lp.n2_w), c.g(lp.n2_b), r.mlp.ptr, r.mlp.bytes, c.s));
    prof_set_tag(MIVIT_PROF_ATTN_OUT_BWD);
    RC(c.fo->attn_out_bwd(dx1, c.buf(b.z1), c.fbuf(b.rstd1), c.p(lp.n1_w), c.buf(b.ctx), c.W(lp.out_w), M, dz1, c.buf(w.dctx),
                          c.g(lp.out_w), c.g(lp.out_b), c.g(lp.n1_w), c.g(lp.n1_b), r.attn_out.ptr, r.attn_out.bytes, c.s));
    prof_set_tag(MIVIT_PROF_ATTN_CORE_BWD);
    RC(launch_attention_bwd(dt, c.buf(b.qkv), c.buf(w.dctx), c.B, c.S, c.H, c.Dh, c.buf(w.dqkv), c.s));
    if (!qkv_split) {
        ProfPin pin(MIVIT_PROF_QKV_BWD);
        RC(c.fo->qkv_bwd(c.buf(w.dqkv), xin, c.W(lp.qkv_w), dz1, M, c.buf(w.dxa), c.g(lp.qkv_w), c.g(lp.qkv_b), gin, bin, r.qkv.ptr, r.qkv.bytes, c.s));
        return slabs.flush(c.s);
    }
    ProfPin pin(MIVIT_PROF_QKV_WGRAD);
    RC(lin_wgrad(dt, c.buf(w.dqkv), 3 * E, xin, 0, E, M, 3 * E, E, c.g(lp.qkv_w), c.g(lp.qkv_b), r.qkv.ptr, r.qkv.bytes, c.s));
    if (l > 0) RC(launch_affine_fixup(c.g(lp.qkv_w), c.g(lp.qkv_b), gin, bin, 3 * E, E, c.s));
    pin.set(MIVIT_PROF_QKV_DGRAD);
    return lin_dgrad(dt, c.buf(w.dqkv), 3 * E, c.W(lp.qkv_w), M, 3 * E, E, MIVIT_ACT_NONE, nullptr, 0, dz1, E, c.buf(w.dxa), E, 0, c.s);
}

int layer_bwd_general(const Call &c, int l) {
    const Ws &w = c.w; const Ws::L &b = w.layer[l]; const LayerParams &lp = c.plan->layers[l];
    const int dt = c.dt, E = c.E, F = c.F, M = c.M, act = c.cfg.activation;
    const void *xin = l > 0 ? c.buf(w.layer[l - 1].x2) : c.buf(w.x0);
    void *wg = c.buf(w.wgrad), *dxa = c.buf(w.dxa), *dxb = c.buf(w.dxb); const size_t wgb = w.wgrad_bytes;
    bool cs = false; LayerNormBwdArgs n2 = {};
    n2.dtype = dt; n2.dy = dxa; n2.lddy = E; n2.z = c.buf(b.z2); n2.ldz = E; n2.gamma = c.p(lp.n2_w); n2.mean = c.fbuf(b.mean2);
    n2.rstd = c.fbuf(b.rstd2); n2.M = M; n2.E = E; n2.dz = dxb; n2.lddz = E; n2.dgamma = c.g(lp.n2_w); n2.dbeta = c.g(lp.n2_b);
    n2.ws = c.buf(w.ln); n2.ws_bytes = w.ln_bytes;
    RC(ln_bwd_bias(n2, c.g(lp.fc2_b), &cs, c.s));
    RC(lin_wgrad(dt, dxb, E, c.buf(b.h), 0, F, M, E, F, c.g(lp.fc2_w), cs ? c.g(lp.fc2_b) : nullptr, wg, wgb, c.s));
    RC(lin_dgrad(dt, dxb, E, c.W(lp.fc2_w), M, E, F, act, act == MIVIT_ACT_GELU ? c.buf(b.u) : c.buf(b.h), F, nullptr, 0, c.buf(w.dF), F, 0, c.s));
    RC(lin_wgrad(dt, c.buf(w.dF), F, c.buf(b.x1), 0, E, M, F, E, c.g(lp.fc1_w), c.g(lp.fc1_b), wg, wgb, c.s));
    RC(lin_dgrad(dt, c.buf(w.dF), F, c.W(lp.fc1_w), M, F, E, MIVIT_ACT_NONE, nullptr, 0, dxb, E, dxa, E, 0, c.s));
    LayerNormBwdArgs n1 = n2;
    n1.dy = dxa; n1.z = c.buf(b.z1); n1.gamma = c.p(lp.n1_w); n1.mean = c.fbuf(b.mean1); n1.rstd = c.fbuf(b.rstd1);
    n1.dz = dxb; n1.dgamma = c.g(lp.n1_w); n1.dbeta = c.g(lp.n1_b);
    RC(ln_bwd_bias(n1, c.g(lp.out_b), &cs, c.s));
    RC(lin_wgrad(dt, dxb, E, c.buf(b.ctx), 0, E, M, E, E, c.g(lp.out_w), cs ? c.g(lp.out_b) : nullptr, wg, wgb, c.s));
    RC(lin_dgrad(dt, dxb, E, c.W(lp.out_w), M, E, E, MIVIT_ACT_NONE, nullptr, 0, nullptr, 0, c.buf(w.dctx), E, 0, c.s));
    prof_set_tag(MIVIT_PROF_ATTN_BWD);
    RC(launch_attention_bwd(dt, c.buf(b.qkv), c.buf(w.dctx), c.B, c.S, c.H, c.Dh, c.buf(w.dqkv), c.s));
    RC(lin_wgrad(dt, c.buf(w.dqkv), 3 * E, xin, 0, E, M, 3 * E, E, c.g(lp.qkv_w), c.g(lp.qkv_b), wg, wgb, c.s));
    return lin_dgrad(dt, c.buf(w.dqkv), 3 * E, c.W(lp.qkv_w), M, 3 * E, E, MIVIT_ACT_NONE, nullptr, 0, dxb, E, dxa, E, 0, c.s);
}

int embed_bwd(const Call &c, const float *x, const float *features, float *dfeatures, float *dx_tokens) {
    const mivit_plan *p = c.plan; const mivit_config &cfg = c.cfg; const Ws &w = c.w;
    const int dt = c.dt, E = c.E, B = c.B, S = c.S, Mt = c.Mt;
    void *wg = c.buf(w.wgrad); const size_t wgb = w.wgrad_bytes;
    if (cfg.use_pos_encoding) {
        RC(launch_fill_zero(c.g(p->pos), (size_t)MAX_TOKENS * E * sizeof(float), c.s));
        RC(launch_batch_colsum(dt, c.buf(w.dxa), B, S, E, 0, S, c.g(p->pos), c.buf(w.colsum), w.colsum_bytes, c.s));
    }
    if (cfg.use_regression_token) RC(launch_batch_colsum(dt, c.buf(w.dxa), B, S, E, 0, 1, c.g(p->reg), c.buf(w.colsum), w.colsum_bytes, c.s));
    if (cfg.fusion == MIVIT_FUSION_EARLY) RC(feature_projector_bwd(c, features, c.buf(w.dxa), (int64_t)S * E, dfeatures));
    LayerNormBwdArgs a = {};
    a.dtype = dt; a.dy = c.buf(w.dxa); a.lddy = E; a.z = c.buf(w.emb); a.ldz = E; a.gamma = c.p(p->n0_w); a.mean = c.fbuf(w.mean0);
    a.rstd = c.fbuf(w.rstd0); a.M = Mt; a.E = E; a.rows_per_seq = c.T; a.in_seq_stride = S; a.in_row_off = c.off;
    a.dz = c.buf(w.dxb); a.lddz = E; a.dgamma = c.g(p->n0_w); a.dbeta = c.g(p->n0_b); a.ws = c.buf(w.ln); a.ws_bytes = w.ln_bytes;
    if (cfg.embedding == MIVIT_EMBED_EXTERNAL) {
        prof_set_tag(MIVIT_PROF_LN_BWD); RC(launch_layernorm_bwd(a, c.s));
        if (dx_tokens) RC(launch_convert(c.f32, c.buf(w.dxb), E, 1, dx_tokens, E, Mt, E, 0, c.s, dt));
        return 0;
    }
    bool cs = false;
    RC(ln_bwd_bias(a, c.g(p->emb_b), &cs, c.s));
    const int K = cfg.patch_size * cfg.patch_size; const StreamOps *so = stream_ops(dt);
    if (so && so->embed_ok(dt, Mt, K, E)) {
        prof_set_tag(MIVIT_PROF_EMBED_WGRAD);
        RC(so->embed_wgrad(c.buf(w.dxb), x, c.g(p->emb_w), Mt, K, E, wg, wgb, c.s));
        if (cs) RC(lin_wgrad(dt, c.buf(w.dxb), E, x, 1, K, Mt, E, K, nullptr, c.g(p->emb_b), wg, wgb, c.s));
        return 0;
    }
    return lin_wgrad(dt, c.buf(w.dxb), E, x, 1, K, Mt, E, K, c.g(p->emb_w), cs ? c.g(p->emb_b) : nullptr, wg, wgb, c.s);
}

int backward_impl(const mivit_plan *plan, const float *params, const float *x, const float *features, int B, int T,
                         void *workspace, size_t workspace_bytes, const float *dout, float *grads, float *dfeatures,
                         float *dx_tokens, int stage_begin, int stage_end, void *stream) {
    RC(check_call(plan, B, T, workspace_bytes, true, "mivit_backward"));
    MIVIT_CHECK(params && x && workspace && dout && grads, "mivit_backward: null pointer");
    MIVIT_CHECK(stage_begin >= 0 && stage_begin <= stage_end && stage_end <= (int)plan->stages.size(),
                "mivit_backward: bad stage range [%d,%d)", stage_begin, stage_end);
    MIVIT_CHECK(plan->c.fusion == MIVIT_FUSION_NONE || features, "mivit_backward: features required");
    const Call c(plan, B, T, true, workspace, params, grads, stream);
    for (int st = stage_begin; st < stage_end; ++st) {
        if (st == 0) RC(head_bwd(c, dout, features, dfeatures));
        else if (st <= c.L) RC(c.fused ? layer_bwd_fused(c, c.L - st) : layer_bwd_general(c, c.L - st));
        else RC(embed_bwd(c, x, features, dfeatures, dx_tokens));
    }
    return 0;
}

}

static bool graph_sized(const mivit_plan *plan, int B, int T) {
    return plan && (int64_t)B * (T + 1) * plan->c.embed_dim <= 65536LL * 128;
}

extern "C" int mivit_forward(const mivit_plan *plan, const float *params, const float *x, const float *features, int B, int T,
                             void *workspace, size_t workspace_bytes, int need_backward, float *out, void *stream) {
    const auto body = [&](hipStream_t cs) {
        return forward_impl(plan, params, x, features, B, T, workspace, workspace_bytes, need_backward, out, cs);
    };
    hipStream_t s = static_cast<hipStream_t>(stream);
    if (!graph_sized(plan, B, T)) return body(s);
    const uint64_t key[] = {1, plan->uid, (uint64_t)params, (uint64_t)x, (uint64_t)features, (uint64_t)B, (uint64_t)T,
                            (uint64_t)workspace, (uint64_t)workspace_bytes, (uint64_t)need_backward, (uint64_t)out};
    return graph_run(key, (int)(sizeof(key) / sizeof(key[0])), s, body);
}

extern "C" int mivit_backward(const mivit_plan *plan, const float *params, const float *x, const float *features, int B,
                              int T, void *workspace, size_t workspace_bytes, const float *dout, float *grads,
                              float *dfeatures, float *dx_tokens, int stage_begin, int stage_end, void *stream) {
    const auto body = [&](hipStream_t cs) {
        return backward_impl(plan, params, x, features, B, T, workspace, workspace_bytes, dout, grads, dfeatures, dx_tokens,
                             stage_begin, stage_end, cs);
    };
    hipStream_t s = static_cast<hipStream_t>(stream);
    if (!graph_sized(plan, B, T)) return body(s);
    const uint64_t key[] = {2, plan->uid, (uint64_t)params, (uint64_t)x, (uint64_t)features, (uint64_t)B, (uint64_t)T,
                            (uint64_t)workspace, (uint64_t)workspace_bytes, (uint64_t)dout, (uint64_t)grads,
                            (uint64_t)dfeatures, (uint64_t)dx_tokens, (uint64_t)stage_begin, (uint64_t)stage_end};
    return graph_run(key, (int)(sizeof(key) / sizeof(key[0])), s, body);
}
```

Before: 1.943 million sequences/s.

## Compute last layer MLP and attention backward only for regression-token rows

With a regression token, only row 0 of the final layer's output reaches the head. The last layer's MLP forward now runs only on the B readout rows, which are gathered into compact buffers and scattered back into the full layout. The attention backward gets a row-limited variant that processes only the query tiles containing row 0 and zeroes dQ for the rest. The intent is to skip the final-layer MLP and attention-backward work on the other 32 rows. The cost is extra convert, fill and scatter kernels and new workspace buffers.

```diff
diff --git a/include/mivit_hip.h b/include/mivit_hip.h
--- a/include/mivit_hip.h
+++ b/include/mivit_hip.h
@@ -318,6 +318,8 @@
 int mivit_attention_fwd(int dtype, const void *qkv, int B, int S, int H, int Dh, void *ctx, void *stream);
 int mivit_attention_bwd(int dtype, const void *qkv, const void *dctx, int B, int S, int H, int Dh,
                         void *dqkv, void *stream);
+int mivit_attention_bwd_rows(int dtype, const void *qkv, const void *dctx, int64_t dctx_seq_stride, int q_rows, int B, int S,
+                             int H, int Dh, void *dqkv, void *stream);
 
 typedef struct mivit_config {
     int abi_version;
@@ -362,6 +364,8 @@
                    int stage_begin, int stage_end, void *stream);
 
 void mivit_graph_stats(uint64_t *replays, uint64_t *captures, int *failures);
+
+int mivit_set_readout_rows(int mode);
 
 enum {
     MIVIT_PROF_EMBED_FWD = 0,
diff --git a/moleculardiffusion_mivit_amd/_native.py b/moleculardiffusion_mivit_amd/_native.py
--- a/moleculardiffusion_mivit_amd/_native.py
+++ b/moleculardiffusion_mivit_amd/_native.py
@@ -96,6 +96,8 @@
     "mivit_attention_max_seq": (c_int, [c_int, c_int]),
     "mivit_attention_fwd": (c_int, [c_int, c_void_p, c_int, c_int, c_int, c_int, c_void_p, c_void_p]),
     "mivit_attention_bwd": (c_int, [c_int, c_void_p, c_void_p, c_int, c_int, c_int, c_int, c_void_p, c_void_p]),
+    "mivit_attention_bwd_rows": (c_int, [c_int, c_void_p, c_void_p, c_int64, c_int, c_int, c_int, c_int, c_int, c_void_p, c_void_p]),
+    "mivit_set_readout_rows": (c_int, [c_int]),
     "mivit_plan_create": (c_void_p, [POINTER(MivitConfig)]),
     "mivit_plan_destroy": (None, [c_void_p]),
     "mivit_plan_num_params": (c_int, [c_void_p]),
diff --git a/moleculardiffusion_mivit_amd/csrc/attention.hip b/moleculardiffusion_mivit_amd/csrc/attention.hip
--- a/moleculardiffusion_mivit_amd/csrc/attention.hip
+++ b/moleculardiffusion_mivit_amd/csrc/attention.hip
@@ -427,6 +427,19 @@
          : dtype == MIVIT_BF16 ? attn_bwd_t<bf16>(qkv, dctx, B, S, H, Dh, dqkv, s) : attn_bwd_t<f16>(qkv, dctx, B, S, H, Dh, dqkv, s);
 }
 
+bool attention_bwd_rows_ok(int dtype, int S, int Dh) {
+    return attention_bwd_rows_supported(dtype, S, Dh) || attention_bwd_rows_supported_f16(dtype, S, Dh);
+}
+int launch_attention_bwd_q_rows(int dtype, const void *qkv, const void *dctx, int64_t dctx_seq_stride, int q_rows, int B, int S, int H,
+                                int Dh, void *dqkv, hipStream_t s) {
+    MIVIT_CHECK(B > 0 && S > 0 && H > 0 && Dh > 0, "attention_bwd_rows: empty problem");
+    if (attention_bwd_rows_supported(dtype, S, Dh)) return launch_attention_bwd_rows(qkv, dctx, dctx_seq_stride, q_rows, B, S, H, Dh, dqkv, s);
+    if (attention_bwd_rows_supported_f16(dtype, S, Dh))
+        return launch_attention_bwd_rows_f16(qkv, dctx, dctx_seq_stride, q_rows, B, S, H, Dh, dqkv, s);
+    MIVIT_FAIL("attention_bwd_rows: no kernel for dtype %d, S = %d, head dim %d (16-bit, S <= 128, head dim 16 / 32 / 64, MIVIT_ATTN_BWD unset or 2)",
+               dtype, S, Dh);
+}
+
 extern "C" int mivit_attention_max_seq(int dtype, int Dh) { return attention_max_seq(dtype, Dh); }
 extern "C" int mivit_attention_fwd(int dtype, const void *qkv, int B, int S, int H, int Dh, void *ctx, void *stream) {
     MIVIT_CHECK(dtype == MIVIT_F32 || dtype == MIVIT_BF16 || dtype == MIVIT_F16, "bad dtype %d", dtype);
@@ -439,3 +452,9 @@
     MIVIT_CHECK(qkv && dctx && dqkv, "attention_bwd: null pointer");
     return launch_attention_bwd(dtype, qkv, dctx, B, S, H, Dh, dqkv, static_cast<hipStream_t>(stream));
 }
+extern "C" int mivit_attention_bwd_rows(int dtype, const void *qkv, const void *dctx, int64_t dctx_seq_stride, int q_rows, int B, int S,
+                                        int H, int Dh, void *dqkv, void *stream) {
+    MIVIT_CHECK(dtype == MIVIT_F32 || dtype == MIVIT_BF16 || dtype == MIVIT_F16, "bad dtype %d", dtype);
+    MIVIT_CHECK(qkv && dctx && dqkv, "attention_bwd_rows: null pointer");
+    return launch_attention_bwd_q_rows(dtype, qkv, dctx, dctx_seq_stride, q_rows, B, S, H, Dh, dqkv, static_cast<hipStream_t>(stream));
+}
diff --git a/moleculardiffusion_mivit_amd/csrc/attention_fast.hip b/moleculardiffusion_mivit_amd/csrc/attention_fast.hip
--- a/moleculardiffusion_mivit_amd/csrc/attention_fast.hip
+++ b/moleculardiffusion_mivit_amd/csrc/attention_fast.hip
@@ -73,6 +73,8 @@
     int B, S, H, Dh, E;
     int ld;
     int img;
+    int q_rows;
+    int64_t do_stride;
 };
 
 template <int NT, int ND>
@@ -339,7 +341,7 @@
     return ELEM_MFMA_16x16x16(a, b, c);
 }
 
-template <int NT, int ND>
+template <int NT, int ND, bool ROWS>
 __global__ __launch_bounds__(256, (NT * ND <= 6 ? 3 : 1)) void attn_bwd_fast2(const bf16 *qkv, const bf16 *dctx, bf16 *dqkv, const FastDims d) {
     extern __shared__ __attribute__((aligned(16))) unsigned char smem_raw[];
     constexpr int KD = (ND + 1) / 2;
@@ -353,18 +355,25 @@
     bf16 *Kimg = Qimg + d.img, *Oimg = Kimg + d.img, *Simg = Oimg + d.img;
     const int64_t ld3 = 3 * (int64_t)d.E;
     const bf16 *q = qkv + (int64_t)b * d.S * ld3 + h * d.Dh, *k = q + d.E, *v = q + 2 * d.E;
-    const bf16 *dO = dctx + (int64_t)b * d.S * d.E + h * d.Dh;
+    const int q_rows = ROWS ? d.q_rows : d.S;
+    const bf16 *dO = dctx + (ROWS ? (int64_t)b * d.do_stride : (int64_t)b * d.S * d.E) + h * d.Dh;
+    const int nit = ROWS ? min(NT, (q_rows + 15) >> 4) : NT;
+    if (ROWS) {
+        bf16 *dq0 = dqkv + ((int64_t)b * d.S + nit * 16) * ld3 + h * d.Dh;
+        for (int u = lane; u < (d.S - nit * 16) * (ND * 2); u += 64)
+            *reinterpret_cast<uint4 *>(dq0 + (int64_t)(u / (ND * 2)) * ld3 + (u % (ND * 2)) * 8) = make_uint4(0u, 0u, 0u, 0u);
+    }
     constexpr int CPR = ND * 2, NCH = NT * 16 * CPR, NIT = (NCH + 63) / 64;
     constexpr bool BATCH = NIT <= 4 && NT <= 4;
     bf16x8 kf[NT][KD], vf[NT][KD];
     if (BATCH) {
         uint4 sq[NIT], sk[NIT], so[NIT];
-        auto ld_nat = [&](const bf16 *src, int64_t sld, uint4 (&v)[NIT]) {
+        auto ld_nat = [&](const bf16 *src, int64_t sld, int rows, uint4 (&v)[NIT]) {
 #pragma unroll
             for (int i = 0; i < NIT; ++i) {
                 const int u = lane + 64 * i, r = u / CPR, dd = (u % CPR) * 8;
                 v[i] = make_uint4(0u, 0u, 0u, 0u);
-                if (u < NCH && r < d.S && dd + 8 <= d.Dh) v[i] = *reinterpret_cast<const uint4 *>(src + (int64_t)r * sld + dd);
+                if (u < NCH && r < rows && dd + 8 <= d.Dh) v[i] = *reinterpret_cast<const uint4 *>(src + (int64_t)r * sld + dd);
             }
         };
         auto st_nat = [&](bf16 *img, const uint4 (&v)[NIT]) {
@@ -374,7 +383,7 @@
                 if (u < NCH) *reinterpret_cast<uint4 *>(img + r * d.ld + (SWZ ? (dd ^ (((r >> 2) & 1) << 4)) : dd)) = v[i];
             }
         };
-        ld_nat(q, ld3, sq); ld_nat(k, ld3, sk); ld_nat(dO, d.E, so);
+        ld_nat(q, ld3, d.S, sq); ld_nat(k, ld3, d.S, sk); ld_nat(dO, d.E, q_rows, so);
 #pragma unroll
         for (int j = 0; j < NT; ++j)
 #pragma unroll
@@ -386,7 +395,7 @@
     } else {
         stage_nat<SWZ>(Qimg, d.ld, q, ld3, d.S, NT * 16, d.Dh, lane);
         stage_nat<SWZ>(Kimg, d.ld, k, ld3, d.S, NT * 16, d.Dh, lane);
-        stage_nat<SWZ>(Oimg, d.ld, dO, d.E, d.S, NT * 16, d.Dh, lane);
+        stage_nat<SWZ>(Oimg, d.ld, dO, d.E, q_rows, NT * 16, d.Dh, lane);
 #pragma unroll
         for (int j = 0; j < NT; ++j)
 #pragma unroll
@@ -415,14 +424,14 @@
         for (int jd = 0; jd < ND; ++jd) { dv[j][jd] = zero; dk[j][jd] = zero; }
 
 #pragma unroll 1
-    for (int it = 0; it < NT; ++it) {
+    for (int it = 0; it < nit; ++it) {
         bf16x8 qf[KD], of[KD];
 #pragma unroll
         for (int kd = 0; kd < KD; ++kd) {
             if (SWZ) { qf[kd] = lfrag(Qimg, it * 16); of[kd] = lfrag(Oimg, it * 16); }
             else {
                 qf[kd] = gfrag(q, ld3, it * 16, d.S, kd * 32, d.Dh, lane);
-                of[kd] = gfrag(dO, d.E, it * 16, d.S, kd * 32, d.Dh, lane);
+                of[kd] = gfrag(dO, d.E, it * 16, q_rows, kd * 32, d.Dh, lane);
             }
         }
         f32x4 dS[NT];
@@ -518,6 +527,7 @@
     const int NT = (S + 15) / 16, NP = (NT + 1) / 2;
     d.ld = Dh + 8;
     d.img = NP * 32 * d.ld;
+    d.q_rows = 0; d.do_stride = 0;
     return d;
 }
 
@@ -538,12 +548,16 @@
     MIVIT_LAUNCH_CHECK();
     return 0;
 }
+static int bwd_version() {
+    static const int version = getenv("MIVIT_ATTN_BWD") ? atoi(getenv("MIVIT_ATTN_BWD")) : 2;
+    return version;
+}
 template <int NT, int ND>
 int bwd_launch(const bf16 *qkv, const bf16 *dctx, bf16 *dqkv, const FastDims &d, hipStream_t s) {
     const size_t per_wave = (size_t)3 * d.img * sizeof(bf16);
     const int wpb = waves_per_block(per_wave);
-    static const int version = getenv("MIVIT_ATTN_BWD") ? atoi(getenv("MIVIT_ATTN_BWD")) : 2;
-    auto kern = version == 2 ? attn_bwd_fast2<NT, ND> : attn_bwd_fast<NT, ND>;
+    const int version = bwd_version();
+    auto kern = version != 2 ? attn_bwd_fast<NT, ND> : (d.q_rows > 0 ? attn_bwd_fast2<NT, ND, true> : attn_bwd_fast2<NT, ND, false>);
     if (version == 2) {
         FastDims d2 = d;
         if (ND == 2) d2.ld = 32;
@@ -613,3 +627,14 @@
     const int NT = (S + 15) / 16, ND = Dh / 16;
     FAST_DISPATCH(bwd_launch, static_cast<const bf16 *>(qkv), static_cast<const bf16 *>(dctx), static_cast<bf16 *>(dqkv), d, s)
 }
+
+bool attention_bwd_rows_supported(int dtype, int S, int Dh) { return attention_fast_supported(dtype, S, Dh) && bwd_version() == 2; }
+int launch_attention_bwd_rows(const void *qkv, const void *dctx, int64_t dctx_seq_stride, int q_rows, int B, int S, int H, int Dh,
+                              void *dqkv, hipStream_t s) {
+    MIVIT_CHECK(q_rows >= 1 && q_rows <= S && dctx_seq_stride >= (int64_t)q_rows * H * Dh && dctx_seq_stride % 8 == 0,
+                "attention_bwd_rows: %d rows of %d at stride %lld", q_rows, S, (long long)dctx_seq_stride);
+    FastDims d = make_fast(B, S, H, Dh);
+    d.q_rows = q_rows; d.do_stride = dctx_seq_stride;
+    const int NT = (S + 15) / 16, ND = Dh / 16;
+    FAST_DISPATCH(bwd_launch, static_cast<const bf16 *>(qkv), static_cast<const bf16 *>(dctx), static_cast<bf16 *>(dqkv), d, s)
+}
diff --git a/moleculardiffusion_mivit_amd/csrc/common.h b/moleculardiffusion_mivit_amd/csrc/common.h
--- a/moleculardiffusion_mivit_amd/csrc/common.h
+++ b/moleculardiffusion_mivit_amd/csrc/common.h
@@ -266,10 +266,16 @@
 int launch_attention_fwd(int dtype, const void *qkv, int B, int S, int H, int Dh, void *ctx, hipStream_t s);
 int launch_attention_bwd(int dtype, const void *qkv, const void *dctx, int B, int S, int H, int Dh, void *dqkv,
                          hipStream_t s);
+bool attention_bwd_rows_ok(int dtype, int S, int Dh);
+int launch_attention_bwd_q_rows(int dtype, const void *qkv, const void *dctx, int64_t dctx_seq_stride, int q_rows, int B, int S, int H,
+                                int Dh, void *dqkv, hipStream_t s);
 int attention_max_seq(int dtype, int Dh);
 bool attention_fast_supported(int dtype, int S, int Dh);
 int launch_attention_fwd_fast(const void *qkv, int B, int S, int H, int Dh, void *ctx, hipStream_t s);
 int launch_attention_bwd_fast(const void *qkv, const void *dctx, int B, int S, int H, int Dh, void *dqkv, hipStream_t s);
+bool attention_bwd_rows_supported(int dtype, int S, int Dh);
+int launch_attention_bwd_rows(const void *qkv, const void *dctx, int64_t dctx_seq_stride, int q_rows, int B, int S, int H, int Dh,
+                              void *dqkv, hipStream_t s);
 
 bool embed_dma_supported(int dtype, int M, int K, int E);
 int launch_embed_fwd_dma(const float *X, const void *W_bf16, const float *bias, void *Y, int M, int K, int E, hipStream_t s);
@@ -323,6 +329,9 @@
 bool attention_fast_supported_f16(int dtype, int S, int Dh);
 int launch_attention_fwd_fast_f16(const void *qkv, int B, int S, int H, int Dh, void *ctx, hipStream_t s);
 int launch_attention_bwd_fast_f16(const void *qkv, const void *dctx, int B, int S, int H, int Dh, void *dqkv, hipStream_t s);
+bool attention_bwd_rows_supported_f16(int dtype, int S, int Dh);
+int launch_attention_bwd_rows_f16(const void *qkv, const void *dctx, int64_t dctx_seq_stride, int q_rows, int B, int S, int H, int Dh,
+                                  void *dqkv, hipStream_t s);
 bool embed_dma_supported_f16(int dtype, int M, int K, int E);
 int launch_embed_fwd_dma_f16(const float *X, const void *W_bf16, const float *bias, void *Y, int M, int K, int E, hipStream_t s);
 size_t embed_wgrad_dma_ws_bytes_f16(int M, int K, int E);
diff --git a/moleculardiffusion_mivit_amd/csrc/elem.h b/moleculardiffusion_mivit_amd/csrc/elem.h
--- a/moleculardiffusion_mivit_amd/csrc/elem.h
+++ b/moleculardiffusion_mivit_amd/csrc/elem.h
@@ -23,6 +23,8 @@
 #define attention_fast_supported attention_fast_supported_f16
 #define launch_attention_fwd_fast launch_attention_fwd_fast_f16
 #define launch_attention_bwd_fast launch_attention_bwd_fast_f16
+#define attention_bwd_rows_supported attention_bwd_rows_supported_f16
+#define launch_attention_bwd_rows launch_attention_bwd_rows_f16
 #define embed_dma_supported embed_dma_supported_f16
 #define launch_embed_fwd_dma launch_embed_fwd_dma_f16
 #define embed_wgrad_dma_ws_bytes embed_wgrad_dma_ws_bytes_f16
diff --git a/moleculardiffusion_mivit_amd/csrc/engine.hip b/moleculardiffusion_mivit_amd/csrc/engine.hip
--- a/moleculardiffusion_mivit_amd/csrc/engine.hip
+++ b/moleculardiffusion_mivit_amd/csrc/engine.hip
@@ -57,6 +57,9 @@
     if (dtype == MIVIT_F16 && !f16_off) return E == 64 ? &kFusedF16W64 : &kFusedF16;
     return nullptr;
 }
+static int g_readout_rows = getenv("MIVIT_NO_READOUT_ROWS") ? 0 : (getenv("MIVIT_READOUT_ROWS") ? atoi(getenv("MIVIT_READOUT_ROWS")) : 1);
+extern "C" int mivit_set_readout_rows(int on) { const int old = g_readout_rows; g_readout_rows = on; return old; }
+
 static bool fused_ok(int dtype, int E, int F, int H, int S) {
     const FusedOps *f = fused_ops(dtype, E);
     return f && f->ok(dtype, E, F, H, S);
@@ -111,6 +114,8 @@
     std::vector<L> layer;
     size_t xF, meanF, rstdF, pooled, fp_h, fp_out, head_in, hh;
     size_t xL;
+    size_t z1c, rstd1c, ctxc, dz1c, dctxc;
+    size_t z2c, rstd2c, xLc;
     size_t dout_t, d_hh, d_head_in, d_pool_c, d_fp_h, dxa, dxb, dF, dctx, dqkv, wgrad, ln, colsum;
     size_t wgrad_bytes, ln_bytes, colsum_bytes;
 };
@@ -146,6 +151,9 @@
     }
     for (int l = nsets; l < L; ++l) w.layer.push_back(w.layer[0]);
     w.xL = fused ? take(M * E * ts) : 0;
+    const bool rows = fused && c.use_regression_token && S > 1;
+    w.z1c = rows ? take((size_t)B * E * ts) : 0;
+    if (rows) { w.z2c = take((size_t)B * E * ts); w.rstd2c = take((size_t)B * 4); w.xLc = take((size_t)B * E * ts); }
     w.xF = c.use_regression_token ? 0 : take(M * E * ts);
     w.meanF = take(M * 4); w.rstdF = take(M * 4);
     w.pooled = take((size_t)B * E * ts);
@@ -160,6 +168,10 @@
         w.d_fp_h = take((size_t)B * E * ts);
         w.dxa = take(M * E * ts); w.dxb = take(M * E * ts);
         w.dF = take(M * F * ts); w.dctx = take(M * E * ts); w.dqkv = take(M * 3 * E * ts);
+        if (rows) {
+            w.rstd1c = take((size_t)B * 4); w.ctxc = take((size_t)B * E * ts);
+            w.dz1c = take((size_t)B * E * ts); w.dctxc = take((size_t)B * E * ts);
+        }
         size_t wg = 0;
         auto mx = [&](int m, int n, int k) {
             size_t b = linear_wgrad_ws_bytes(m, n, k);
@@ -468,12 +480,16 @@
     const bool bwd;
     const bool fused;
     const FusedOps *fo;
+    const bool rows;
+    const bool rows_exact;
     const Ws w;
     void *ws; const float *P; float *G; hipStream_t s;
     Call(const mivit_plan *p, int B_, int T_, bool bwd_, void *workspace, const float *params, float *grads, void *stream)
         : plan(p), cfg(p->c), dt(cfg.dtype), E(cfg.embed_dim), F(cfg.hidden_dim), H(cfg.num_heads), Dh(E / H), L(cfg.num_layers),
           B(B_), T(T_), off(cfg.use_regression_token ? 1 : 0), S(T + off), M(B * S), Mt(B * T), f32(dt == MIVIT_F32), bwd(bwd_),
-          fused(L > 0 && fused_ok(dt, E, F, H, S)), fo(fused ? fused_ops(dt, E) : nullptr), w(make_ws(p, B, T, bwd)),
+          fused(L > 0 && fused_ok(dt, E, F, H, S)), fo(fused ? fused_ops(dt, E) : nullptr),
+          rows(fused && cfg.use_regression_token && S > 1 && g_readout_rows == 2),
+          rows_exact(fused && cfg.use_regression_token && S > 1 && g_readout_rows != 0 && g_readout_rows != 2), w(make_ws(p, B, T, bwd)),
           ws(workspace), P(params), G(grads), s(static_cast<hipStream_t>(stream)) {}
     void *buf(size_t o) const { return at(ws, o); }
     float *fbuf(size_t o) const { return static_cast<float *>(at(ws, o)); }
@@ -520,6 +536,29 @@
         prof_set_tag(MIVIT_PROF_ATTN_BLOCK_FWD);
         RC(c.fo->attn_fwd(nin, gin, bin, c.W(lp.qkv_w), c.p(lp.qkv_b), c.W(lp.out_w), c.p(lp.out_b), c.p(lp.n1_w), c.p(lp.n1_b), c.B, c.S,
                           c.buf(b.ctx), c.buf(b.z1), c.fbuf(b.rstd1), nullptr, nullptr, nullptr, c.bwd ? c.buf(b.qkv) : nullptr, c.s));
+        if (c.rows_exact && l + 1 == c.L) {
+            const Ws &w = c.w; const size_t ts = dtype_size(c.dt); const int64_t SE = (int64_t)c.S * c.E;
+            RC(launch_convert(0, c.buf(b.z1), SE, 0, c.buf(w.z1c), c.E, c.B, c.E, 0, c.s, c.dt));
+            prof_set_tag(MIVIT_PROF_MLP_BLOCK_FWD);
+            RC(c.fo->mlp_fwd(c.buf(w.z1c), c.p(lp.n1_w), c.p(lp.n1_b), c.W(lp.fc1_w), c.p(lp.fc1_b), c.W(lp.fc2_w), c.p(lp.fc2_b),
+                             c.p(lp.n2_w), c.p(lp.n2_b), c.B, c.cfg.activation, c.buf(w.z2c), c.fbuf(w.rstd2c), c.buf(w.xLc), nullptr,
+                             nullptr, nullptr, nullptr, c.s));
+            RC(launch_convert(0, c.buf(w.xLc), c.E, 0, c.buf(w.xL), SE, c.B, c.E, 0, c.s, c.dt));
+            if (c.bwd) {
+                RC(launch_fill_zero(c.buf(b.z2), (size_t)c.M * c.E * ts, c.s));
+                RC(launch_fill_zero(c.buf(b.rstd2), (size_t)c.M * 4, c.s));
+                RC(launch_convert(0, c.buf(w.z2c), c.E, 0, c.buf(b.z2), SE, c.B, c.E, 0, c.s, c.dt));
+                RC(launch_convert(1, c.fbuf(w.rstd2c), 1, 1, c.fbuf(b.rstd2), c.S, c.B, 1, 0, c.s, c.dt));
+            }
+            return 0;
+        }
+        if (c.rows && l + 1 == c.L) {
+            RC(launch_convert(0, c.buf(b.z1), (int64_t)c.S * c.E, 0, c.buf(c.w.z1c), c.E, c.B, c.E, 0, c.s, c.dt));
+            prof_set_tag(MIVIT_PROF_MLP_BLOCK_FWD);
+            return c.fo->mlp_fwd(c.buf(c.w.z1c), c.p(lp.n1_w), c.p(lp.n1_b), c.W(lp.fc1_w), c.p(lp.fc1_b), c.W(lp.fc2_w), c.p(lp.fc2_b),
+                                 c.p(lp.n2_w), c.p(lp.n2_b), c.B, c.cfg.activation, c.buf(b.z2), c.fbuf(b.rstd2), c.buf(c.w.xL), nullptr,
+                                 nullptr, nullptr, nullptr, c.s);
+        }
         prof_set_tag(MIVIT_PROF_MLP_BLOCK_FWD);
         RC(c.fo->mlp_fwd(c.buf(b.z1), c.p(lp.n1_w), c.p(lp.n1_b), c.W(lp.fc1_w), c.p(lp.fc1_b), c.W(lp.fc2_w), c.p(lp.fc2_b), c.p(lp.n2_w),
                          c.p(lp.n2_b), c.M, c.cfg.activation, c.buf(b.z2), c.fbuf(b.rstd2), l + 1 == c.L ? c.buf(c.w.xL) : nullptr,
@@ -553,7 +592,8 @@
     a.mean = c.fbuf(w.meanF); a.rstd = c.fbuf(w.rstdF);
     prof_set_tag(MIVIT_PROF_LN_FWD);
     if (c.cfg.use_regression_token) {
-        a.M = c.B; a.y = c.buf(w.pooled); a.in_rows = 1; a.in_stride = c.S; a.in_off = 0;
+        a.M = c.B; a.y = c.buf(w.pooled);
+        if (!c.rows) { a.in_rows = 1; a.in_stride = c.S; a.in_off = 0; }
         return launch_layernorm_fwd(a, c.s);
     }
     a.M = c.M; a.y = c.buf(w.xF); RC(launch_layernorm_fwd(a, c.s));
@@ -613,8 +653,11 @@
     a.dtype = dt; a.z = c.trunk_out(); a.ldz = E; a.gamma = c.p(p->tn_w); a.mean = c.fbuf(w.meanF); a.rstd = c.fbuf(w.rstdF);
     a.E = E; a.dz = c.buf(w.dxa); a.lddz = E; a.dgamma = c.g(p->tn_w); a.dbeta = c.g(p->tn_b); a.ws = c.buf(w.ln); a.ws_bytes = w.ln_bytes;
     if (c.cfg.use_regression_token) {
-        RC(launch_fill_zero(c.buf(w.dxa), (size_t)c.M * E * dtype_size(dt), c.s));
-        a.dy = c.buf(w.d_head_in); a.lddy = Hin; a.M = B; a.z_rows = 1; a.z_stride = c.S; a.z_off = 0;
+        a.dy = c.buf(w.d_head_in); a.lddy = Hin; a.M = B;
+        if (!c.rows) {
+            RC(launch_fill_zero(c.buf(w.dxa), (size_t)c.M * E * dtype_size(dt), c.s));
+            a.z_rows = 1; a.z_stride = c.S; a.z_off = 0;
+        }
     } else {
         const void *dp = c.buf(w.d_head_in);
         if (Hin != E) {
@@ -654,7 +697,53 @@
     RC(c.fo->attn_out_bwd(dx1, c.buf(b.z1), c.fbuf(b.rstd1), c.p(lp.n1_w), c.buf(b.ctx), c.W(lp.out_w), M, dz1, c.buf(w.dctx),
                           c.g(lp.out_w), c.g(lp.out_b), c.g(lp.n1_w), c.g(lp.n1_b), r.attn_out.ptr, r.attn_out.bytes, c.s));
     prof_set_tag(MIVIT_PROF_ATTN_CORE_BWD);
-    RC(launch_attention_bwd(dt, c.buf(b.qkv), c.buf(w.dctx), c.B, c.S, c.H, c.Dh, c.buf(w.dqkv), c.s));
+    if (c.rows_exact && l + 1 == c.L && attention_bwd_rows_ok(dt, c.S, c.Dh))
+        RC(launch_attention_bwd_q_rows(dt, c.buf(b.qkv), c.buf(w.dctx), (int64_t)c.S * E, 1, c.B, c.S, c.H, c.Dh, c.buf(w.dqkv), c.s));
+    else
+        RC(launch_attention_bwd(dt, c.buf(b.qkv), c.buf(w.dctx), c.B, c.S, c.H, c.Dh, c.buf(w.dqkv), c.s));
+    if (!qkv_split) {
+        ProfPin pin(MIVIT_PROF_QKV_BWD);
+        RC(c.fo->qkv_bwd(c.buf(w.dqkv), xin, c.W(lp.qkv_w), dz1, M, c.buf(w.dxa), c.g(lp.qkv_w), c.g(lp.qkv_b), gin, bin, r.qkv.ptr, r.qkv.bytes, c.s));
+        return slabs.flush(c.s);
+    }
+    ProfPin pin(MIVIT_PROF_QKV_WGRAD);
+    RC(lin_wgrad(dt, c.buf(w.dqkv), 3 * E, xin, 0, E, M, 3 * E, E, c.g(lp.qkv_w), c.g(lp.qkv_b), r.qkv.ptr, r.qkv.bytes, c.s));
+    if (l > 0) RC(launch_affine_fixup(c.g(lp.qkv_w), c.g(lp.qkv_b), gin, bin, 3 * E, E, c.s));
+    pin.set(MIVIT_PROF_QKV_DGRAD);
+    return lin_dgrad(dt, c.buf(w.dqkv), 3 * E, c.W(lp.qkv_w), M, 3 * E, E, MIVIT_ACT_NONE, nullptr, 0, dz1, E, c.buf(w.dxa), E, 0, c.s);
+}
+
+int last_layer_bwd_rows(const Call &c) {
+    static const bool qkv_split = getenv("MIVIT_NO_QKV_BWD") != nullptr;
+    static const bool no_defer = getenv("MIVIT_NO_SLAB_DEFER") != nullptr || qkv_split;
+    const int l = c.L - 1;
+    const Ws &w = c.w; const Ws::L &b = w.layer[l]; const LayerParams &lp = c.plan->layers[l];
+    const int dt = c.dt, E = c.E, M = c.M, B = c.B; const int64_t SE = (int64_t)c.S * E;
+    const void *xin = l > 0 ? c.buf(w.layer[l - 1].z2) : c.buf(w.x0);
+    const float *gin = l > 0 ? c.p(c.plan->layers[l - 1].n2_w) : nullptr, *bin = l > 0 ? c.p(c.plan->layers[l - 1].n2_b) : nullptr;
+    void *dx1 = c.buf(w.dxb), *dz1 = c.buf(w.dF);
+    const FusedBwdWs r = fused_bwd_ws(c, !no_defer);
+    SlabDefer slabs(r.defer);
+    RC(launch_convert(1, c.fbuf(b.rstd1), c.S, 1, c.fbuf(w.rstd1c), 1, B, 1, 0, c.s, dt));
+    RC(launch_convert(0, c.buf(b.ctx), SE, 0, c.buf(w.ctxc), E, B, E, 0, c.s, dt));
+    prof_set_tag(MIVIT_PROF_MLP_BLOCK_BWD);
+    RC(c.fo->mlp_bwd(c.buf(w.dxa), c.buf(b.z2), c.fbuf(b.rstd2), c.p(lp.n2_w), c.buf(w.z1c), c.p(lp.n1_w), c.p(lp.n1_b), c.W(lp.fc1_w),
+                     c.p(lp.fc1_b), c.W(lp.fc2_w), B, c.cfg.activation, dx1, c.g(lp.fc1_w), c.g(lp.fc1_b), c.g(lp.fc2_w), c.g(lp.fc2_b),
+                     c.g(lp.n2_w), c.g(lp.n2_b), r.mlp.ptr, r.mlp.bytes, c.s));
+    prof_set_tag(MIVIT_PROF_ATTN_OUT_BWD);
+    RC(c.fo->attn_out_bwd(dx1, c.buf(w.z1c), c.fbuf(w.rstd1c), c.p(lp.n1_w), c.buf(w.ctxc), c.W(lp.out_w), B, c.buf(w.dz1c), c.buf(w.dctxc),
+                          c.g(lp.out_w), c.g(lp.out_b), c.g(lp.n1_w), c.g(lp.n1_b), r.attn_out.ptr, r.attn_out.bytes, c.s));
+    if (attention_bwd_rows_ok(dt, c.S, c.Dh)) {
+        prof_set_tag(MIVIT_PROF_ATTN_CORE_BWD);
+        RC(launch_attention_bwd_q_rows(dt, c.buf(b.qkv), c.buf(w.dctxc), E, 1, B, c.S, c.H, c.Dh, c.buf(w.dqkv), c.s));
+    } else {
+        RC(launch_fill_zero(c.buf(w.dctx), (size_t)M * E * dtype_size(dt), c.s));
+        RC(launch_convert(0, c.buf(w.dctxc), E, 0, c.buf(w.dctx), SE, B, E, 0, c.s, dt));
+        prof_set_tag(MIVIT_PROF_ATTN_CORE_BWD);
+        RC(launch_attention_bwd(dt, c.buf(b.qkv), c.buf(w.dctx), B, c.S, c.H, c.Dh, c.buf(w.dqkv), c.s));
+    }
+    RC(launch_fill_zero(dz1, (size_t)M * E * dtype_size(dt), c.s));
+    RC(launch_convert(0, c.buf(w.dz1c), E, 0, dz1, SE, B, E, 0, c.s, dt));
     if (!qkv_split) {
         ProfPin pin(MIVIT_PROF_QKV_BWD);
         RC(c.fo->qkv_bwd(c.buf(w.dqkv), xin, c.W(lp.qkv_w), dz1, M, c.buf(w.dxa), c.g(lp.qkv_w), c.g(lp.qkv_b), gin, bin, r.qkv.ptr, r.qkv.bytes, c.s));
@@ -735,6 +824,7 @@
     const Call c(plan, B, T, true, workspace, params, grads, stream);
     for (int st = stage_begin; st < stage_end; ++st) {
         if (st == 0) RC(head_bwd(c, dout, features, dfeatures));
+        else if (st == 1 && c.rows) RC(last_layer_bwd_rows(c));
         else if (st <= c.L) RC(c.fused ? layer_bwd_fused(c, c.L - st) : layer_bwd_general(c, c.L - st));
         else RC(embed_bwd(c, x, features, dfeatures, dx_tokens));
     }
@@ -755,7 +845,8 @@
     hipStream_t s = static_cast<hipStream_t>(stream);
     if (!graph_sized(plan, B, T)) return body(s);
     const uint64_t key[] = {1, plan->uid, (uint64_t)params, (uint64_t)x, (uint64_t)features, (uint64_t)B, (uint64_t)T,
-                            (uint64_t)workspace, (uint64_t)workspace_bytes, (uint64_t)need_backward, (uint64_t)out};
+                            (uint64_t)workspace, (uint64_t)workspace_bytes, (uint64_t)need_backward, (uint64_t)out,
+                            (uint64_t)g_readout_rows};
     return graph_run(key, (int)(sizeof(key) / sizeof(key[0])), s, body);
 }
 
@@ -770,6 +861,7 @@
     if (!graph_sized(plan, B, T)) return body(s);
     const uint64_t key[] = {2, plan->uid, (uint64_t)params, (uint64_t)x, (uint64_t)features, (uint64_t)B, (uint64_t)T,
                             (uint64_t)workspace, (uint64_t)workspace_bytes, (uint64_t)dout, (uint64_t)grads,
-                            (uint64_t)dfeatures, (uint64_t)dx_tokens, (uint64_t)stage_begin, (uint64_t)stage_end};
+                            (uint64_t)dfeatures, (uint64_t)dx_tokens, (uint64_t)stage_begin, (uint64_t)stage_end,
+                            (uint64_t)g_readout_rows};
     return graph_run(key, (int)(sizeof(key) / sizeof(key[0])), s, body);
 }
```

Result: faster. 1.973 million sequences/s, median of 6 (+1.5%).
